# Druthyn/rtiow

Hardware: AMD Instinct MI355X
Metric: Msamples/sec (pixels×spp) on book-1 final scene; per-pixel RMSE vs CPU (higher is better)
Workload: dtype f64

## Files before the change

__graft_entry__.py:

```python
import os
import subprocess
import sys

ROOT = os.path.dirname(os.path.abspath(__file__))
if ROOT not in sys.path:
    sys.path.insert(0, ROOT)

HIPCC_FLAGS = [
    "-O3", "-std=c++17", "--offload-arch=gfx950",
    "-ffp-contract=off",
    "-fhip-fp32-correctly-rounded-divide-sqrt",
    "-mllvm", "-amdgpu-mfma-vgpr-form",
    "-fPIC", "-shared",
]


def build_hip_library(crosscheck=False):
    out = os.path.join(ROOT, "tools", "librtiow_hip_xcheck.so") if crosscheck else os.path.join(ROOT, "rtiow_amd", "librtiow_hip.so")
    srcs = [os.path.join(ROOT, "rtiow_amd", "csrc", name) for name in ("rt_api.hip", "rt_frames.hip")]
    import bench
    cmd = ["hipcc", *HIPCC_FLAGS, *(["-DRTIOW_CROSSCHECK_MODES"] if crosscheck else []),
           f'-DRT_SOURCE_SHA="{bench.kernel_source_sha()}"',
           "-I", os.path.join(ROOT, "include"), "-I", os.path.join(ROOT, "rtiow_amd", "csrc"), "-o", out, *srcs]
    subprocess.run(cmd, check=True, cwd=ROOT)
    return out


def build_host_cli(sanitize=False):
    out = os.path.join(ROOT, "host", "rtiow_render_san" if sanitize else "rtiow_render")
    rocm = os.environ.get("ROCM_PATH", "/opt/rocm")
    opt = ["-O1", "-g", "-fno-omit-frame-pointer", "-fsanitize=address,undefined", "-fno-sanitize-recover=all"] if sanitize else ["-O2"]
    cmd = ["g++", *opt, "-std=c++17", "-ffp-contract=off", "-Wall", "-Wextra", "-Wno-unused-parameter",
           "-I", os.path.join(ROOT, "include"), "-I", os.path.join(ROOT, "host"), "-isystem", os.path.join(rocm, "include"),
           "-o", out, os.path.join(ROOT, "host", "rtiow_render.cpp"),
           "-L", os.path.join(ROOT, "rtiow_amd"), "-lrtiow_hip", "-L", os.path.join(rocm, "lib"), "-lamdhip64", "-lrccl",
           "-pthread", "-Wl,-rpath,$ORIGIN/../rtiow_amd", "-Wl,-rpath," + os.path.join(rocm, "lib")]
    subprocess.run(cmd, check=True, cwd=ROOT)
    return out


def build() -> None:
    build_hip_library()
    build_hip_library(crosscheck=True)
    build_host_cli()
    subprocess.run(["make", "-s", "-C", os.path.join(ROOT, "oracle"), "liboracle.so"], check=True)
    import rtiow_amd
    from rtiow_amd import _ffi
    lib = _ffi.load()
    assert lib.rt_backend_name() == b"hip-gfx950"
    assert not _ffi.has_crosscheck_modes()
    assert rtiow_amd.SPHERE_DTYPE.itemsize == 72


def smoke() -> None:
    import numpy as np
    import oracle
    import rtiow_amd as rt

    w, h, spp = 96, 54, 4
    flat = rt.random_scene(1).flatten()
    cam = rt.book1_camera(w, h)
    with rt.Renderer(0) as r:
        r.upload_scene(flat)
        sums, fix, st = r.render(cam, rt.make_params(w, h, spp, seed=1))
        rgba = r.resolve_rgba8(fix, spp, flip=True)
    want_fix, want_sum, ost = oracle.render_b(oracle.camera_from_host(cam), flat, oracle.make_params(w, h, spp, seed=1))
    assert np.array_equal(fix, want_fix), "GPU exact sums differ from the CPU oracle"
    assert np.array_equal(sums, want_sum)
    assert st["rays_traced"] == ost["rays_traced"] and st["samples"] == w * h * spp
    assert np.array_equal(rgba, oracle.resolve_b(want_fix, spp, flip=True))
    with rt.Renderer(0) as r:
        r.upload_scene(flat)
        one_call, _ = r.render_rgba8(cam, rt.make_params(w, h, spp, seed=1), flip=True)
    assert np.array_equal(one_call, rgba), "rt_render_rgba8 differs from rt_render + rt_resolve_rgba8"
    print(f"smoke ok: {w}x{h}x{spp} bit-exact vs oracle; {st['rays_traced']} rays, "
          f"kernel {st['kernel_ms']:.3f} ms on {st['grid_blocks']} blocks")


if __name__ == "__main__":
    build()
    if len(sys.argv) > 1 and sys.argv[1] == "smoke":
        smoke()
```

rtiow_amd/csrc/rt_api.hip:

```cpp
#include <hip/hip_runtime.h>

#include <algorithm>
#include <cmath>
#include <cstdarg>
#include <cstdio>
#include <cstdlib>
#include <cstring>
#include <vector>

#include "rt_host.hpp"

namespace {

thread_local char g_err[512] = "";

int env_int(const char *name, int dflt)
{
    const char *v = getenv(name);
    if (!v || !*v) return dflt;
    return atoi(v);
}

}

int rt_host::fail(int code, const char *fmt, ...)
{
    va_list ap;
    va_start(ap, fmt);
    vsnprintf(g_err, sizeof(g_err), fmt, ap);
    va_end(ap);
    return code;
}

using namespace rt_host;

int rt_host::validate_params(const rt_params *p)
{
    if (!p) return fail(RT_ERR_INVALID_ARGUMENT, "params is NULL");
    if (p->width < 2 || p->height < 2)
        return fail(RT_ERR_INVALID_ARGUMENT, "width and height must be >= 2 (u,v divide by W-1,H-1; main.rs:131-132)");
    if (p->width > 65535 || p->height > 65535)
        return fail(RT_ERR_INVALID_ARGUMENT, "width and height must be <= 65535");
    if ((long long)p->width * p->height > 0x7fffffffLL)
        return fail(RT_ERR_INVALID_ARGUMENT, "width*height does not fit the 32-bit Philox pixel counter");
    if (p->spp < 0 || p->sample_begin < 0 || (long long)p->spp + p->sample_begin > 0x7fffffffLL)
        return fail(RT_ERR_INVALID_ARGUMENT, "spp/sample_begin out of range");
    if (p->max_depth < 0) return fail(RT_ERR_INVALID_ARGUMENT, "max_depth must be >= 0");
    if (!(p->t_min > 0.0)) return fail(RT_ERR_INVALID_ARGUMENT, "t_min must be > 0 (reference: 1e-4, main.rs:44)");
    if (p->tile_rows < 1) return fail(RT_ERR_INVALID_ARGUMENT, "tile_rows must be >= 1");
    if (p->shard_count < 1 || p->shard_index < 0 || p->shard_index >= p->shard_count)
        return fail(RT_ERR_INVALID_ARGUMENT, "need 0 <= shard_index < shard_count");
    if (p->flags & ~RT_FLAG_KNOWN)
        return fail(RT_ERR_INVALID_ARGUMENT, "unknown flags 0x%x (this library knows 0x%x)", p->flags & ~RT_FLAG_KNOWN, RT_FLAG_KNOWN);
    return RT_OK;
}

namespace {

int shard_rows(const rt_params *p)
{
    const long long T = p->tile_rows, H = p->height;
    const long long ntiles = (H + T - 1) / T;
    long long rows = 0;
    for (long long t = p->shard_index; t < ntiles; t += p->shard_count) {
        const long long lo = t * T;
        rows += (lo + T <= H) ? T : (H - lo);
    }
    return (int)rows;
}

}

int rt_host::ensure(void **ptr, size_t *have, size_t need)
{
    if (*have >= need && *ptr) return RT_OK;
    if (*ptr) { (void)hipFree(*ptr); *ptr = nullptr; *have = 0; }
    RT_HIP(hipMalloc(ptr, need ? need : 16));
    *have = need;
    return RT_OK;
}

namespace {

float filter_kprime(const rt_sphere &s, double KU)
{
    const double kappa = KU / (1.0 - KU);
    const double r2 = s.radius * s.radius;
    const double c2 = s.center[0] * s.center[0] + s.center[1] * s.center[1] + s.center[2] * s.center[2];
    if (!(r2 > 1e-30) || !(c2 + r2 < 1e30)) return -INFINITY;
    const double exact = c2 * (1.0 - kappa) - r2 * (1.0 + 2.0 * kappa);
    float kp = (float)(exact - std::fabs(exact) * 1e-12);
    if ((double)kp > exact) kp = std::nextafterf(kp, -INFINITY);
    return kp;
}

uint32_t host_bf16_rne(float x)
{
    uint32_t u; memcpy(&u, &x, 4);
    return (u + 0x7FFFu + ((u >> 16) & 1u)) >> 16;
}
void host_split_bf16x3(float x, uint32_t p[3])
{
    auto back = [](uint32_t b) { uint32_t u = b << 16; float f; memcpy(&f, &u, 4); return f; };
    p[0] = host_bf16_rne(x);
    const float r1 = x - back(p[0]);
    p[1] = host_bf16_rne(r1);
    const float r2 = r1 - back(p[1]);
    p[2] = host_bf16_rne(r2);
}

float tube_radius_floor(const rt_sphere *spheres, int n, const char *skip)
{
    std::vector<double> r;
    for (int i = 0; i < n; ++i)
        if (!(skip && skip[i]) && std::fabs(spheres[i].radius) > 1e-15 && std::fabs(spheres[i].radius) < 1e15)
            r.push_back(std::fabs(spheres[i].radius));
    if (r.empty()) return 1.0f;
    std::nth_element(r.begin(), r.begin() + r.size() / 4, r.end());
    return (float)r[r.size() / 4];
}
float tube_bound(const rt_sphere &s, float rho)
{
    const double r = std::fabs(s.radius);
    const double c2 = s.center[0] * s.center[0] + s.center[1] * s.center[1] + s.center[2] * s.center[2];
    if (!(r * r > 1e-30) || !(c2 + r * r < 1e30)) return INFINITY;
    const double R = r * (1.0 + (double)rt::kTubeBasisErr) + (double)rt::kTubeCenterErr * std::sqrt(c2);
    float f = (float)(R * (1.0 + 1e-12));
    if ((double)f < R) f = std::nextafterf(f, INFINITY);
    return f > rho ? f : rho;
}
uint32_t tube_sigma_bits(float bound)
{
    if (!(bound < INFINITY)) return 0u;
    const float f = (float)(2.0 * (1.0 - 1.0 / 64.0) / (double)bound);
    uint32_t u; memcpy(&u, &f, 4);
    return u >> 16;
}
void tube_tile(const rt_sphere *const s[32], float rho, uint4 out_b[64], float out_r[32])
{
    for (int c = 0; c < 32; ++c) {
        uint32_t w[8] = {0, 0, 0, 0, 0, 0, 0, 0};
        out_r[c] = -1.0f;
        if (s[c]) {
            out_r[c] = tube_bound(*s[c], rho);
            const uint32_t sg = tube_sigma_bits(out_r[c]);
            uint32_t sgu = sg << 16; float sigma; memcpy(&sigma, &sgu, 4);
            if (sg != 0u) {
                for (int i = 0; i < 3; ++i) {
                    const double ci = s[c]->center[i] * (double)sigma;
                    const uint32_t y1 = host_bf16_rne((float)ci);
                    uint32_t u1 = y1 << 16; float f1; memcpy(&f1, &u1, 4);
                    const uint32_t y2 = host_bf16_rne((float)(ci - (double)f1));
                    w[2 * i + 0] = y1 | (y2 << 16);
                    w[2 * i + 1] = y1 | (y2 << 16);
                }
            }
            w[6] = sg | (sg << 16);
            w[7] = sg;
        } else {
            w[7] = 0x4080u << 16;
        }
        out_b[c] = make_uint4(w[0], w[1], w[2], w[3]);
        out_b[32 + c] = make_uint4(w[4], w[5], w[6], w[7]);
    }
}

void free_scene(rt_context *ctx)
{
    (void)hipFree(ctx->d_filt); (void)hipFree(ctx->d_geo); (void)hipFree(ctx->d_mat);
    (void)hipFree(ctx->d_btube); (void)hipFree(ctx->d_geo_slot); (void)hipFree(ctx->d_slot_orig);
    ctx->d_filt = nullptr; ctx->d_geo = ctx->d_mat = nullptr; ctx->d_btube = nullptr; ctx->d_geo_slot = nullptr; ctx->d_slot_orig = nullptr;
#ifdef RTIOW_CROSSCHECK_MODES
    ctx->x.release();
#endif
    ctx->n_spheres = -1;
}

template <typename T>
int upload_table(T **dst, const T *src, size_t count)
{
    RT_HIP(hipMalloc((void **)dst, (count ? count : 1) * sizeof(T)));
    if (count) RT_HIP(hipMemcpy(*dst, src, count * sizeof(T), hipMemcpyHostToDevice));
    return RT_OK;
}

}

void rt_host::set_scene_params(const rt_context *ctx, rt::KParams &kp)
{
    kp.filt = ctx->d_filt; kp.geo = ctx->d_geo; kp.mat = ctx->d_mat;
    kp.n_tiles = ctx->n_tiles;
#ifdef RTIOW_CROSSCHECK_MODES
    kp.x.bmat = ctx->x.d_bmat; kp.x.kpt = ctx->x.d_kpt;
    kp.x.bmat16 = ctx->x.d_bmat16; kp.x.kpt16 = ctx->x.d_kpt16; kp.x.bmatL = ctx->x.d_bmatL;
#endif
    kp.btube = ctx->d_btube; kp.tube_rho = ctx->tube_rho;
    kp.geo_slot = ctx->d_geo_slot; kp.slot_orig = ctx->d_slot_orig;
    kp.n_global = ctx->n_global; kp.grid_dim = ctx->grid_dim;
    kp.grid_rows = 0ull;
    for (int k = 0; ctx->grid_dim > 0 && (k + 1) * ctx->grid_dim <= 64; ++k) kp.grid_rows |= 1ull << (k * ctx->grid_dim);
    for (int k = 0; k < 8; ++k) kp.grid[k] = ctx->grid[k];
    kp.scene_scale = ctx->scene_scale;
    kp.n_always = ctx->n_always;
    for (int e = 0; e < 8; ++e) kp.always_idx[e] = ctx->always_idx[e];
}

int rt_host::next_launch_slot(rt_context *ctx, hipStream_t stream, rt::KParams &kp)
{
    ctx->cur = (ctx->cur + 1) % rt_context::kSlots;
    ctx->d_queue = ctx->q_slots[ctx->cur]; ctx->d_stats = ctx->s_slots[ctx->cur];
    ctx->ev0 = ctx->e0_slots[ctx->cur]; ctx->ev1 = ctx->e1_slots[ctx->cur];
    if (ctx->slot_used[ctx->cur]) RT_HIP(hipStreamWaitEvent(stream, ctx->ev1, 0));
    ctx->slot_used[ctx->cur] = true;
    kp.queue = ctx->d_queue; kp.stats = ctx->d_stats;
    return RT_OK;
}

namespace {

int validate_pixel_list(const rt_context *ctx, const rt_camera *cam, const rt_params *p, int64_t n_pixels)
{
    int rc = validate_params(p);
    if (rc) return rc;
    if (p->flags & (RT_FLAG_UNIFORM53 | RT_FLAG_DIAG_STATS | RT_FLAG_NO_FILTER))
        return fail(RT_ERR_INVALID_ARGUMENT, "pixel-list renders run the shipped kernel only: RT_FLAG_UNIFORM53, RT_FLAG_DIAG_STATS and "
                    "RT_FLAG_NO_FILTER are not available on them (flags 0x%x)", p->flags);
    if (p->shard_count != 1)
        return fail(RT_ERR_INVALID_ARGUMENT, "pixel-list renders are not sharded: shard_count must be 1 (is %d)", p->shard_count);
    if (n_pixels < 0 || n_pixels > 0x7fffffffLL)
        return fail(RT_ERR_INVALID_ARGUMENT, "n_pixels %lld out of range [0, 2^31)", (long long)n_pixels);
    if (!ctx || !cam) return fail(RT_ERR_INVALID_ARGUMENT, "ctx/cam is NULL");
    if (ctx->scan_mode != 5)
        return fail(RT_ERR_INVALID_ARGUMENT, "pixel-list renders need the shipped scan mode 5; this context was created under RTIOW_SCAN_MODE=%d", ctx->scan_mode);
    return RT_OK;
}

int validate_adaptive(const rt_adaptive *a)
{
    if (!a) return fail(RT_ERR_INVALID_ARGUMENT, "rt_adaptive is NULL");
    if (a->step < 1) return fail(RT_ERR_INVALID_ARGUMENT, "rt_adaptive.step must be >= 1 (is %d)", a->step);
    if (a->reserved != 0) return fail(RT_ERR_INVALID_ARGUMENT, "rt_adaptive.reserved must be 0");
    if (!(a->threshold >= 0.0)) return fail(RT_ERR_INVALID_ARGUMENT, "rt_adaptive.threshold must be >= 0 (and not a NaN)");
    if (!(a->dark_floor > 0.0) || !(a->dark_floor < INFINITY))
        return fail(RT_ERR_INVALID_ARGUMENT, "rt_adaptive.dark_floor must be > 0 and finite (with a zero floor a black pixel's error is 0/0)");
    return RT_OK;
}

constexpr int kAdaptiveMaxSpp = 32766;

int validate_select(const void *fix, const void *half, const void *count, int32_t width, int32_t height, int32_t n, const rt_adaptive *a,
                    const void *list_out, const void *n_out)
{
    if (!fix || !half || !count || !list_out || !n_out) return fail(RT_ERR_INVALID_ARGUMENT, "rt_select_pixels: a buffer is NULL");
    if (width < 1 || height < 1 || (long long)width * height > 0x7fffffffLL)
        return fail(RT_ERR_INVALID_ARGUMENT, "rt_select_pixels: bad width/height");
    if (n < 2 || n > kAdaptiveMaxSpp || (n & 1))
        return fail(RT_ERR_INVALID_ARGUMENT, "rt_select_pixels: n = %d samples must be even (two halves) and in [2, %d]", n, kAdaptiveMaxSpp);
    return validate_adaptive(a);
}

constexpr size_t kMaxColumns = (size_t)1 << 26;
constexpr int kMaxGridDim = 63;

struct TileLayout {
    int grid_dim = 0, n_global = 0;
    float grid[8] = {};
    float scale = 0.0f;
    std::vector<int> slot_of;
};

std::vector<int> always_exact_list(const rt_sphere *spheres, int n)
{
    std::vector<int> out;
    if (n <= 0) return out;
    std::vector<double> radii(n);
    for (int i = 0; i < n; ++i) radii[i] = std::fabs(spheres[i].radius);
    std::vector<double> sorted = radii;
    std::nth_element(sorted.begin(), sorted.begin() + n / 2, sorted.end());
    const double big = 8.0 * sorted[n / 2];
    std::vector<int> order;
    for (int i = 0; i < n; ++i) if (radii[i] > big) order.push_back(i);
    std::sort(order.begin(), order.end(), [&](int x, int y) { return radii[x] > radii[y]; });
    for (size_t k = 0; k < order.size() && k < 8; ++k) out.push_back(order[k]);
    return out;
}

TileLayout tile_layout(const rt_sphere *spheres, int n, const char *never)
{
    TileLayout L;
    std::vector<int> filtered;
    for (int i = 0; i < n; ++i) if (!never[i]) filtered.push_back(i);
    std::vector<int> &slot_of = L.slot_of;
    L.grid_dim = 0; L.n_global = 0;
    if (filtered.size() > 64 && !env_int("RTIOW_NO_GRID", 0)) {
        std::vector<double> rr;
        for (int i : filtered) rr.push_back(std::fabs(spheres[i].radius));
        std::nth_element(rr.begin(), rr.begin() + rr.size() / 2, rr.end());
        const double med = rr[rr.size() / 2];
        double x0 = INFINITY, x1 = -INFINITY, z0 = INFINITY, z1 = -INFINITY;
        for (int i : filtered) {
            if (std::fabs(spheres[i].radius) > 3.0 * med) continue;
            x0 = std::min(x0, spheres[i].center[0]); x1 = std::max(x1, spheres[i].center[0]);
            z0 = std::min(z0, spheres[i].center[2]); z1 = std::max(z1, spheres[i].center[2]);
        }
        const double extent = std::max(x1 - x0, z1 - z0);
        const bool one_cell = extent == 0.0;
        const bool grid_ok = one_cell || (extent > 0.0 && extent < 1e15);
        if (grid_ok) {
        std::vector<std::vector<int>> cells;
        std::vector<int> global;
        double cell = 1.0;
        auto assign = [&](int G, bool keep) -> int {
            cell = one_cell ? 1.0 : extent / G;
            std::vector<int> count((size_t)G * G, 0);
            if (keep) { cells.assign((size_t)G * G, {}); global.clear(); }
            size_t n_glob = 0;
            for (int i : filtered) {
                const double r = std::fabs(spheres[i].radius);
                bool to_cell = !(r > 3.0 * med || r > 0.25 * cell);
                size_t c = 0;
                if (to_cell) {
                    int ix = (int)std::floor((spheres[i].center[0] - x0) / cell), iz = (int)std::floor((spheres[i].center[2] - z0) / cell);
                    ix = std::max(0, std::min(ix, G - 1)); iz = std::max(0, std::min(iz, G - 1));
                    c = (size_t)iz * G + ix;
                    to_cell = count[c] < 32;
                }
                if (to_cell) { ++count[c]; if (keep) cells[c].push_back(i); }
                else { ++n_glob; if (keep) global.push_back(i); }
            }
            return (int)((n_glob + 31) / 32);
        };
        int G = one_cell ? 1 : env_int("RTIOW_GRID_DIM", 0);
        if (G <= 0) {
            double best = INFINITY;
            for (int g = 1; g <= kMaxGridDim; ++g) {
                if ((double)g * g > (double)filtered.size()) break;
                const int ng = assign(g, false);
                if (ng > 48) continue;
                const double cost = ng + 1.4 * g;
                if (cost < best) { best = cost; G = g; }
            }
        }
        G = std::max(1, std::min(G, kMaxGridDim));
        (void)assign(G, true);
        double ylo = INFINITY, yhi = -INFINITY, pad = 0.0;
        for (const std::vector<int> &c : cells)
            for (int i : c) {
                const double r = std::fabs(spheres[i].radius);
                ylo = std::min(ylo, spheres[i].center[1] - r); yhi = std::max(yhi, spheres[i].center[1] + r);
                pad = std::max(pad, r);
            }
        const int n_global = (int)((global.size() + 31) / 32);
        const float inv_cell = (float)(1.0 / cell);
        if (std::isnormal(inv_cell) && (size_t)(n_global + G * G) * 32 <= (size_t)kMaxColumns && n_global <= 48 && ylo <= yhi) {
            L.grid_dim = G; L.n_global = n_global;
            slot_of.assign((size_t)(n_global + G * G) * 32, -1);
            for (size_t k = 0; k < global.size(); ++k) slot_of[k] = global[k];
            for (size_t c = 0; c < cells.size(); ++c)
                for (size_t k = 0; k < cells[c].size(); ++k) slot_of[((size_t)n_global + c) * 32 + k] = cells[c][k];
            auto down = [](double v) { float f = (float)v; if ((double)f > v) f = std::nextafterf(f, -INFINITY); return f; };
            auto up = [](double v) { float f = (float)v; if ((double)f < v) f = std::nextafterf(f, INFINITY); return f; };
            L.grid[0] = down(x0); L.grid[1] = down(z0);
            L.grid[2] = inv_cell;
            L.grid[3] = up(x0 + G * cell); L.grid[4] = up(z0 + G * cell);
            L.grid[5] = down(ylo); L.grid[6] = up(yhi); L.grid[7] = up(pad);
            const double gs = std::max(std::fabs(x0), std::fabs(x0 + G * cell)) + pad + std::max(std::fabs(ylo), std::fabs(yhi)) +
                              std::max(std::fabs(z0), std::fabs(z0 + G * cell)) + pad;
            L.scale = (float)gs * 1.0001f;
        }
        }
    }
    if (L.grid_dim == 0) {
        slot_of.assign((size_t)((filtered.empty() ? 0 : filtered.back() + 1) + 31) / 32 * 32, -1);
        for (int i : filtered) slot_of[i] = i;
    }
    return L;
}

#ifdef RTIOW_CROSSCHECK_MODES
#include "xcheck/rt_xcheck_host.inc"
#endif

}

extern "C" {

const char *rt_last_error(void) { return g_err; }
const char *rt_backend_name(void) { return "hip-gfx950"; }
int32_t rt_abi_version(void) { return RTIOW_HIP_ABI_VERSION; }
#ifndef RT_SOURCE_SHA
#define RT_SOURCE_SHA "unknown"
#endif
const char *rt_build_source_sha(void) { return RT_SOURCE_SHA; }

int rt_create(int32_t device_id, rt_context **out)
{
    if (!out) return fail(RT_ERR_INVALID_ARGUMENT, "out is NULL");
    *out = nullptr;
    int count = 0;
    hipError_t e = hipGetDeviceCount(&count);
    if (e != hipSuccess || count <= 0)
        return fail(RT_ERR_NO_DEVICE, "no HIP device visible (%s); librtiow_hip has no CPU fallback",
                    e == hipSuccess ? "count = 0" : hipGetErrorString(e));
    if (device_id < 0 || device_id >= count)
        return fail(RT_ERR_INVALID_ARGUMENT, "device_id %d out of range [0,%d)", device_id, count);
    RT_HIP(hipSetDevice(device_id));
    hipDeviceProp_t prop;
    RT_HIP(hipGetDeviceProperties(&prop, device_id));
    if (strncmp(prop.gcnArchName, "gfx950", 6) != 0)
        return fail(RT_ERR_NO_DEVICE, "device %d is %s; this library carries gfx950 (MI355X) code only",
                    device_id, prop.gcnArchName);
    rt_context *ctx = new (std::nothrow) rt_context();
    if (!ctx) return fail(RT_ERR_OUT_OF_MEMORY, "host allocation failed");
    ctx->device = device_id;
    ctx->cu_count = prop.multiProcessorCount;
    ctx->blocks_per_cu = env_int("RTIOW_BLOCKS_PER_CU", 0);
    ctx->ring_min_spp = env_int("RTIOW_RING_MIN_SPP", 0);
    ctx->scan_mode = env_int("RTIOW_SCAN_MODE", 5);
#ifdef RTIOW_CROSSCHECK_MODES
    if (ctx->scan_mode < 1 || ctx->scan_mode > 5) ctx->scan_mode = 5;
#else
    if (ctx->scan_mode != 1 && ctx->scan_mode != 5) {
        const int asked = ctx->scan_mode;
        rt_destroy(ctx);
        return fail(RT_ERR_INVALID_ARGUMENT, "RTIOW_SCAN_MODE=%d: this build carries scan modes 1 and 5 (modes 2-4 need "
                    "a -DRTIOW_CROSSCHECK_MODES build)", asked);
    }
#endif
    hipError_t e1 = hipSuccess, e2 = hipSuccess, e3 = hipSuccess, e4 = hipSuccess;
    for (int k = 0; k < rt_context::kSlots; ++k) {
        hipError_t a = hipMalloc((void **)&ctx->q_slots[k], 64), b = hipMalloc((void **)&ctx->s_slots[k], 1024);
        hipError_t c = hipEventCreate(&ctx->e0_slots[k]), d = hipEventCreate(&ctx->e1_slots[k]);
        if (a != hipSuccess) e1 = a;
        if (b != hipSuccess) e2 = b;
        if (c != hipSuccess) e3 = c;
        if (d != hipSuccess) e4 = d;
    }
    ctx->d_queue = ctx->q_slots[0]; ctx->d_stats = ctx->s_slots[0]; ctx->ev0 = ctx->e0_slots[0]; ctx->ev1 = ctx->e1_slots[0];
    hipError_t e5 = hipStreamCreateWithFlags(&ctx->own_stream, hipStreamNonBlocking);
    if (e1 != hipSuccess || e2 != hipSuccess || e3 != hipSuccess || e4 != hipSuccess || e5 != hipSuccess) {
        rt_destroy(ctx);
        return fail(RT_ERR_HIP, "context setup failed on device %d", device_id);
    }
    *out = ctx;
    return RT_OK;
}

int rt_destroy(rt_context *ctx)
{
    if (!ctx) return RT_OK;
    (void)hipSetDevice(ctx->device);
    if (ctx->own_stream) (void)hipStreamSynchronize(ctx->own_stream);
    free_scene(ctx);
    for (int k = 0; k < rt_context::kSlots; ++k) {
        (void)hipFree(ctx->q_slots[k]); (void)hipFree(ctx->s_slots[k]);
        if (ctx->e0_slots[k]) (void)hipEventDestroy(ctx->e0_slots[k]);
        if (ctx->e1_slots[k]) (void)hipEventDestroy(ctx->e1_slots[k]);
    }
    (void)hipFree(ctx->d_stage_fix); (void)hipFree(ctx->d_stage_sum); (void)hipFree(ctx->d_stage_rgba);
    (void)hipFree(ctx->d_sel); (void)hipFree(ctx->d_adapt); (void)hipFree(ctx->d_stage_list); (void)hipFree(ctx->d_stage_cams);
    if (ctx->own_stream) (void)hipStreamDestroy(ctx->own_stream);
    delete ctx;
    return RT_OK;
}

int rt_upload_scene(rt_context *ctx, const rt_sphere *spheres, int32_t n)
{
    if (!ctx) return fail(RT_ERR_INVALID_ARGUMENT, "ctx is NULL");
    if (n < 0 || (n > 0 && !spheres)) return fail(RT_ERR_INVALID_ARGUMENT, "bad sphere list");
    if (n > RT_MAX_SPHERES) return fail(RT_ERR_INVALID_ARGUMENT, "at most %d spheres (RT_MAX_SPHERES)", RT_MAX_SPHERES);
    if (ctx->scan_mode == 1 && n > 65535) return fail(RT_ERR_INVALID_ARGUMENT, "RTIOW_SCAN_MODE=1 (the cross-check filter) takes at most 65535 spheres");
    for (int i = 0; i < n; ++i) {
        const rt_sphere &s = spheres[i];
        if (s.kind < RT_LAMBERTIAN || s.kind > RT_DIALECTRIC)
            return fail(RT_ERR_INVALID_ARGUMENT, "sphere %d: unknown material kind %d", i, s.kind);
        const double mags[4] = { s.center[0], s.center[1], s.center[2], s.radius };
        for (double v : mags)
            if (!(std::fabs(v) < 1e15))
                return fail(RT_ERR_INVALID_ARGUMENT, "sphere %d: coordinates/radius must be finite and below 1e15", i);
        if (s.radius == 0.0) return fail(RT_ERR_INVALID_ARGUMENT, "sphere %d: radius must not be zero", i);
    }
    RT_HIP(hipSetDevice(ctx->device));
    RT_HIP(hipDeviceSynchronize());
    free_scene(ctx);
    const size_t cnt = (size_t)(n > 0 ? n : 1);
    std::vector<double> geo(cnt * 4, 0.0), mat(cnt * rt::kMatStride, 0.0);
    for (int i = 0; i < n; ++i) {
        const rt_sphere &s = spheres[i];
        const double r2 = s.radius * s.radius;
        geo[4 * i + 0] = s.center[0]; geo[4 * i + 1] = s.center[1]; geo[4 * i + 2] = s.center[2];
        geo[4 * i + 3] = r2;
        double *m = &mat[(size_t)rt::kMatStride * i];
        m[0] = 1.0 / s.radius;
        m[1] = s.param;
        m[2] = s.albedo[0]; m[3] = s.albedo[1]; m[4] = s.albedo[2];
        m[5] = (double)s.kind;
        if (s.kind == RT_DIALECTRIC) {
            m[6] = 1.0 / s.param;
            double r0 = (1.0 - m[6]) / (1.0 + m[6]); m[7] = r0 * r0;
            r0 = (1.0 - s.param) / (1.0 + s.param); m[8] = r0 * r0;
            m[2] = 1.0; m[3] = 1.0; m[4] = 1.0;
        }
    }
    ctx->n_always = 0;
    for (int i : always_exact_list(spheres, n)) ctx->always_idx[ctx->n_always++] = i;
    const int n_tiles = 2 * ((n + 31) / 32);
    ctx->n_tiles = n_tiles;
    int rc = RT_OK;
    if (ctx->scan_mode == 5) {
        std::vector<char> never(n > 0 ? n : 1, 0);
        for (int e = 0; e < ctx->n_always; ++e) never[ctx->always_idx[e]] = 1;
        ctx->tube_rho = tube_radius_floor(spheres, n, never.data());
        const TileLayout L = tile_layout(spheres, n, never.data());
        const std::vector<int> &slot_of = L.slot_of;
        ctx->grid_dim = L.grid_dim; ctx->n_global = L.n_global;
        for (int k = 0; k < 8; ++k) ctx->grid[k] = L.grid[k];
        ctx->scene_scale = L.scale;
        const int n_tiles32 = (int)(slot_of.size() / 32);
        ctx->n_tiles = 2 * n_tiles32;
        const size_t ttc = (size_t)n_tiles32 + 1;
        std::vector<uint4> btube(ttc * 64);
        std::vector<float> rtube(ttc * 32);
        std::vector<double> geo_slot(ttc * 32 * 4, 0.0);
        std::vector<uint32_t> slot_orig(ttc * 32, 0xFFFFFFFFu);
        for (size_t t = 0; t < ttc; ++t) {
            const rt_sphere *col[32];
            for (int c = 0; c < 32; ++c) {
                const size_t slot = 32 * t + c;
                const int i = slot < slot_of.size() ? slot_of[slot] : -1;
                col[c] = i >= 0 ? &spheres[i] : nullptr;
                if (i >= 0) {
                    slot_orig[slot] = (uint32_t)i;
                    for (int k = 0; k < 4; ++k) geo_slot[4 * slot + k] = geo[4 * (size_t)i + k];
                }
            }
            tube_tile(col, ctx->tube_rho, &btube[t * 64], &rtube[t * 32]);
        }
        if (!rc) rc = upload_table(&ctx->d_btube, btube.data(), btube.size());
        if (!rc) rc = upload_table(&ctx->d_geo_slot, geo_slot.data(), geo_slot.size());
        if (!rc) rc = upload_table(&ctx->d_slot_orig, slot_orig.data(), slot_orig.size());
    }
    std::vector<float> filt(cnt * 4, 0.0f);
    if (ctx->scan_mode >= 1 && ctx->scan_mode <= 3) {
        for (int i = 0; i < n; ++i) {
            const rt_sphere &s = spheres[i];
            filt[4 * i + 0] = (float)s.center[0]; filt[4 * i + 1] = (float)s.center[1];
            filt[4 * i + 2] = (float)s.center[2]; filt[4 * i + 3] = filter_kprime(s, (double)rt::kFilterKU);
        }
        if (ctx->scan_mode == 1 && !rc) rc = upload_table(&ctx->d_filt, filt.data(), filt.size());
    }
#ifdef RTIOW_CROSSCHECK_MODES
    if (!rc) rc = xcheck_upload_tables(ctx, spheres, n, n_tiles, filt);
#endif
    if (!rc) rc = upload_table(&ctx->d_geo, geo.data(), geo.size());
    if (!rc) rc = upload_table(&ctx->d_mat, mat.data(), mat.size());
    if (rc) {
        free_scene(ctx);
        return rc;
    }
    ctx->n_spheres = n;
    return RT_OK;
}

int rt_shard_rows(const rt_params *p, int32_t *out_rows)
{
    if (!out_rows) return fail(RT_ERR_INVALID_ARGUMENT, "out_rows is NULL");
    int rc = validate_params(p);
    if (rc) return rc;
    *out_rows = shard_rows(p);
    return RT_OK;
}

int rt_shard_row_index(const rt_params *p, int32_t compact_row, int32_t *out_j)
{
    if (!out_j) return fail(RT_ERR_INVALID_ARGUMENT, "out_j is NULL");
    int rc = validate_params(p);
    if (rc) return rc;
    if (compact_row < 0 || compact_row >= shard_rows(p))
        return fail(RT_ERR_INVALID_ARGUMENT, "compact_row out of range");
    const int lt = compact_row / p->tile_rows;
    *out_j = (lt * p->shard_count + p->shard_index) * p->tile_rows + (compact_row - lt * p->tile_rows);
    return RT_OK;
}

int rt_render_device(rt_context *ctx, const rt_camera *cam, const rt_params *p, void *d_fix, void *stream_v)
{
    if (!ctx || !cam) return fail(RT_ERR_INVALID_ARGUMENT, "ctx/cam is NULL");
    int rc = validate_params(p);
    if (rc) return rc;
    if (ctx->n_spheres < 0) return fail(RT_ERR_NO_SCENE, "rt_upload_scene has not been called");
    const int rows = shard_rows(p);
    if (rows > 0 && !d_fix) return fail(RT_ERR_INVALID_ARGUMENT, "d_fix is NULL");
    RT_HIP(hipSetDevice(ctx->device));
    hipStream_t stream = (hipStream_t)stream_v;

    const long long npix = (long long)rows * p->width;
    const unsigned long long total_items = (unsigned long long)npix * (unsigned long long)p->spp;
    const int mode_now = (p->flags & RT_FLAG_NO_FILTER) ? 0 : ctx->scan_mode;
    const char *lb_env = getenv("RTIOW_LARGE_BLOCK_MIN_ITEMS");
    const unsigned long long lb_min = (lb_env && *lb_env) ? strtoull(lb_env, nullptr, 0)
                                    : (p->flags & RT_FLAG_OVERLAPPED) ? 0ull : rt::kLargeMinItems;
    const bool small_grid_scene = ctx->grid_dim > 0 && ctx->n_global + ctx->grid_dim * ctx->grid_dim <= 64;
    const bool shipped_kernel = mode_now == 5 && !(p->flags & RT_FLAG_DIAG_STATS);
    const bool large_candidate = shipped_kernel && !small_grid_scene && p->spp >= rt::kLargeMinSpp && total_items >= lb_min && p->spp >= ctx->ring_min_spp;
    const bool wide_ring = shipped_kernel && !large_candidate;
    const unsigned ring_slots = wide_ring ? 2u * (unsigned)rt::kRingSlots : (unsigned)rt::kRingSlots;
    unsigned small_block = 0;
    for (unsigned items = rt::kItemBlock; items >= 64u && p->spp >= 1; items -= 64u)
        if ((items - 1u + (unsigned)p->spp - 1u) / (unsigned)p->spp + 1u <= ring_slots) { small_block = items; break; }
    const bool use_ring = small_block != 0u && p->spp >= ctx->ring_min_spp;
    const bool large_blocks = mode_now == 5 && !(p->flags & RT_FLAG_DIAG_STATS) && use_ring && small_block == (unsigned)rt::kItemBlock &&
                              p->spp >= (small_grid_scene ? rt::kLargeMinSppSmallGrid : rt::kLargeMinSpp) && total_items >= lb_min;
    const unsigned item_block = large_blocks ? rt::kItemBlockLarge : use_ring ? small_block : rt::kItemBlock;
    const unsigned long long n_blocks = (total_items + item_block - 1) / item_block;
    if (n_blocks > 0x7fffffffULL)
        return fail(RT_ERR_INVALID_ARGUMENT, "rows*width*spp = %llu pixel-samples in one launch: at most 2^31 blocks of %d "
                    "(split the samples over several launches with sample_begin and RT_FLAG_ACCUMULATE)", total_items, (int)item_block);
    rt::KParams kp;
    memset(&kp, 0, sizeof(kp));
    static_assert(sizeof(rt::KCamera) == sizeof(rt_camera), "camera layouts must match");
    memcpy(&kp.cam, cam, sizeof(rt_camera));
    kp.width = p->width; kp.height = p->height;
    kp.spp = p->spp; kp.sample_begin = p->sample_begin; kp.max_depth = p->max_depth;
    kp.t_min = p->t_min;
    kp.k0 = (uint32_t)p->seed; kp.k1 = (uint32_t)(p->seed >> 32);
    kp.tile_rows = p->tile_rows; kp.shard_index = p->shard_index; kp.shard_count = p->shard_count;
    kp.rows = rows; kp.n_spheres = ctx->n_spheres;
    kp.npix = (uint32_t)npix; kp.total_items = total_items; kp.n_blocks = (uint32_t)n_blocks;
    kp.inv_spp = p->spp > 0 ? 1.0 / (double)p->spp : 0.0;
    kp.inv_width = 1.0 / (double)p->width;
    auto magic_for = [](long long d) -> uint32_t {
        return (d <= 1 || d >= 32768) ? 0u : (uint32_t)(0x100000000ULL / (unsigned long long)d + 1ULL);
    };
    kp.magic_spp = magic_for(p->spp); kp.magic_width = magic_for(p->width); kp.magic_tile = magic_for(p->tile_rows);
    kp.use_ring = use_ring ? 1 : 0;
    kp.block_items = item_block;
    set_scene_params(ctx, kp);
    kp.fix = (unsigned long long *)d_fix;
    rc = next_launch_slot(ctx, stream, kp);
    if (rc) return rc;

    if (!(p->flags & RT_FLAG_ACCUMULATE) && npix > 0)
        RT_HIP(hipMemsetAsync(d_fix, 0, (size_t)npix * 3 * sizeof(unsigned long long), stream));
    RT_HIP(hipMemsetAsync(ctx->d_queue, 0, 64, stream));
    RT_HIP(hipMemsetAsync(ctx->d_stats, 0, 1024, stream));

    memset(&ctx->last, 0, sizeof(ctx->last));
    ctx->last.n_spheres = ctx->n_spheres;
    ctx->last.block_threads = rt::kBlock;
    ctx->zero_depth_samples = 0;
    if (p->max_depth == 0 || kp.total_items == 0) {
        RT_HIP(hipEventRecord(ctx->ev0, stream));
        RT_HIP(hipEventRecord(ctx->ev1, stream));
        ctx->zero_depth_samples = (unsigned long long)npix * (unsigned long long)p->spp;
        ctx->launched = true;
        return RT_OK;
    }

    int grid = 0;
    const bool diag = (p->flags & RT_FLAG_DIAG_STATS) != 0;
    const int mode = (p->flags & RT_FLAG_NO_FILTER) ? 0 : ctx->scan_mode;
    ctx->last.scan_mode = mode;
    ctx->last.kernel_variant = 0;
    const bool small_grid = small_grid_scene;
    if (p->flags & RT_FLAG_UNIFORM53) {
        if (diag || (mode != 0 && mode != 5))
            return fail(RT_ERR_INVALID_ARGUMENT, "RT_FLAG_UNIFORM53 runs with scan mode 5 (the default) or RT_FLAG_NO_FILTER, without RT_FLAG_DIAG_STATS");
        if (mode == 0) rc = launch_render<0, false, false, true>(ctx, kp, stream, &grid);
        else if (small_grid) rc = large_blocks ? launch_render<5, false, true, true, rt::kItemBlockLarge>(ctx, kp, stream, &grid)
                                              : launch_render<5, false, true, true>(ctx, kp, stream, &grid);
        else rc = large_blocks ? launch_render<5, false, false, true, rt::kItemBlockLarge>(ctx, kp, stream, &grid)
                               : launch_render<5, false, false, true>(ctx, kp, stream, &grid);
        if (rc) return rc;
        ctx->last.kernel_variant = 2 | ((mode == 5 && small_grid) ? 1 : 0) | (mode == 5 && large_blocks ? 4 : 0);
        ctx->launched = true;
        ctx->last.grid_blocks = grid;
        return RT_OK;
    }
    switch (mode * 2 + (diag ? 1 : 0)) {
    case 0: rc = launch_render<0, false>(ctx, kp, stream, &grid); break;
    case 1: rc = launch_render<0, true>(ctx, kp, stream, &grid); break;
    case 2: rc = launch_render<1, false>(ctx, kp, stream, &grid); break;
    case 3: rc = launch_render<1, true>(ctx, kp, stream, &grid); break;
#ifdef RTIOW_CROSSCHECK_MODES
    case 4: rc = launch_render<2, false>(ctx, kp, stream, &grid); break;
    case 5: rc = launch_render<2, true>(ctx, kp, stream, &grid); break;
    case 6: rc = launch_render<3, false>(ctx, kp, stream, &grid); break;
    case 7: rc = launch_render<3, true>(ctx, kp, stream, &grid); break;
    case 8: rc = launch_render<4, false>(ctx, kp, stream, &grid); break;
    case 9: rc = launch_render<4, true>(ctx, kp, stream, &grid); break;
#endif
    case 10:
        if (small_grid) {
            rc = large_blocks ? launch_render<5, false, true, false, rt::kItemBlockLarge>(ctx, kp, stream, &grid)
                              : launch_render<5, false, true>(ctx, kp, stream, &grid);
            ctx->last.kernel_variant = 1;
        } else rc = large_blocks ? launch_render<5, false, false, false, rt::kItemBlockLarge>(ctx, kp, stream, &grid)
                                 : launch_render<5, false>(ctx, kp, stream, &grid);
        if (large_blocks) ctx->last.kernel_variant |= 4;
        break;
    default: rc = launch_render<5, true>(ctx, kp, stream, &grid); break;
    }
    if (rc) return rc;
    ctx->launched = true;
    ctx->last.grid_blocks = grid;
    return RT_OK;
}

int rt_last_stats(rt_context *ctx, rt_stats *stats)
{
    if (!ctx || !stats) return fail(RT_ERR_INVALID_ARGUMENT, "ctx/stats is NULL");
    if (!ctx->launched) return fail(RT_ERR_INVALID_ARGUMENT, "no launch to report on");
    RT_HIP(hipSetDevice(ctx->device));
    RT_HIP(hipEventSynchronize(ctx->ev1));
    float ms = 0.0f;
    RT_HIP(hipEventElapsedTime(&ms, ctx->ev0, ctx->ev1));
    unsigned long long h[80];
    RT_HIP(hipMemcpy(h, ctx->d_stats, sizeof(h), hipMemcpyDeviceToHost));
    for (int k = 0; k < 64; ++k) ctx->last.live_per_bounce[k] = h[16 + k];
    ctx->last.rays_traced = h[0];
    ctx->last.samples = h[1] + ctx->zero_depth_samples;
    ctx->last.candidates = h[2];
    ctx->last.exact_roots = h[3];
    ctx->last.direct_samples = h[4];
    ctx->last.sphere_tests = h[0] * (unsigned long long)(ctx->last.n_spheres > 0 ? ctx->last.n_spheres : 0);
    ctx->last.kernel_ms = ms;
    *stats = ctx->last;
    return RT_OK;
}

#if defined(RT_PHASE_STAMPS) || defined(RT_BLOCK_COUNTS) || defined(RT_EXIT_TIMES) || defined(RT_LDS_CONFLICTS)
extern "C" int rt_debug_phase_cycles(rt_context *ctx, unsigned long long out[8])
{
    RT_HIP(hipSetDevice(ctx->device));
    RT_HIP(hipEventSynchronize(ctx->ev1));
    RT_HIP(hipMemcpy(out, ctx->d_stats + 8, 64, hipMemcpyDeviceToHost));
    return RT_OK;
}
extern "C" int rt_debug_phase_cycles16(rt_context *ctx, unsigned long long out[16])
{
    RT_HIP(hipSetDevice(ctx->device));
    RT_HIP(hipEventSynchronize(ctx->ev1));
    RT_HIP(hipMemcpy(out, ctx->d_stats + 8, 64, hipMemcpyDeviceToHost));
    RT_HIP(hipMemcpy(out + 8, ctx->d_stats + 80, 64, hipMemcpyDeviceToHost));
    return RT_OK;
}
#endif

int rt_fix_to_f32_device(rt_context *ctx, const void *d_fix, int64_t count, void *d_out_f32, void *stream_v)
{
    if (!ctx) return fail(RT_ERR_INVALID_ARGUMENT, "ctx is NULL");
    if (count < 0 || (count > 0 && (!d_fix || !d_out_f32))) return fail(RT_ERR_INVALID_ARGUMENT, "bad buffers");
    if (count == 0) return RT_OK;
    RT_HIP(hipSetDevice(ctx->device));
    long long blocks = (count + 255) / 256;
    if (blocks > 8192) blocks = 8192;
    hipLaunchKernelGGL(rt::fix_to_f32_kernel, dim3((unsigned)blocks), dim3(256), 0, (hipStream_t)stream_v,
                       (const unsigned long long *)d_fix, (float *)d_out_f32, (long long)count);
    RT_HIP(hipGetLastError());
    return RT_OK;
}

int rt_resolve_rgba8_device(rt_context *ctx, const void *d_fix, int32_t width, int32_t rows,
                            int64_t spp, int32_t flip, void *d_rgba, void *stream_v)
{
    if (!ctx) return fail(RT_ERR_INVALID_ARGUMENT, "ctx is NULL");
    if (width < 1 || rows < 0 || spp < 1) return fail(RT_ERR_INVALID_ARGUMENT, "bad width/rows/spp");
    if (rows == 0) return RT_OK;
    if (!d_fix || !d_rgba) return fail(RT_ERR_INVALID_ARGUMENT, "bad buffers");
    RT_HIP(hipSetDevice(ctx->device));
    const long long npix = (long long)width * rows;
    long long blocks = (npix + 255) / 256;
    if (blocks > 8192) blocks = 8192;
    const double scale = 1.0 / (double)spp;
    hipLaunchKernelGGL(rt::resolve_rgba8_kernel, dim3((unsigned)blocks), dim3(256), 0, (hipStream_t)stream_v,
                       (const unsigned long long *)d_fix, (uint8_t *)d_rgba, (int)width, (int)rows, scale, (int)flip);
    RT_HIP(hipGetLastError());
    return RT_OK;
}

int rt_render(rt_context *ctx, const rt_camera *cam, const rt_params *p,
              float *out_sum, uint64_t *out_fix, rt_stats *stats)
{
    if (!ctx) return fail(RT_ERR_INVALID_ARGUMENT, "ctx is NULL");
    int rc = validate_params(p);
    if (rc) return rc;
    const int rows = shard_rows(p);
    const size_t count = (size_t)rows * p->width * 3;
    if (count > 0 && !out_sum && !out_fix) return fail(RT_ERR_INVALID_ARGUMENT, "no output buffer");
    RT_HIP(hipSetDevice(ctx->device));
    rc = ensure(&ctx->d_stage_fix, &ctx->stage_fix_bytes, count * sizeof(uint64_t));
    if (rc) return rc;
    rc = ensure(&ctx->d_stage_sum, &ctx->stage_sum_bytes, count * sizeof(float));
    if (rc) return rc;
    rt_params q = *p;
    q.flags &= ~RT_FLAG_ACCUMULATE;
    rc = rt_render_device(ctx, cam, &q, ctx->d_stage_fix, ctx->own_stream);
    if (rc) return rc;
    if (out_sum) {
        rc = rt_fix_to_f32_device(ctx, ctx->d_stage_fix, (int64_t)count, ctx->d_stage_sum, ctx->own_stream);
        if (rc) return rc;
        RT_HIP(hipMemcpyAsync(out_sum, ctx->d_stage_sum, count * sizeof(float), hipMemcpyDeviceToHost, ctx->own_stream));
    }
    if (out_fix)
        RT_HIP(hipMemcpyAsync(out_fix, ctx->d_stage_fix, count * sizeof(uint64_t), hipMemcpyDeviceToHost, ctx->own_stream));
    RT_HIP(hipStreamSynchronize(ctx->own_stream));
    if (stats) return rt_last_stats(ctx, stats);
    return RT_OK;
}

int rt_resolve_rgba8(rt_context *ctx, const uint64_t *fix, int32_t width, int32_t rows,
                     int64_t spp, int32_t flip, uint8_t *out_rgba)
{
    if (!ctx) return fail(RT_ERR_INVALID_ARGUMENT, "ctx is NULL");
    if (width < 1 || rows < 0 || spp < 1) return fail(RT_ERR_INVALID_ARGUMENT, "bad width/rows/spp");
    if (rows == 0) return RT_OK;
    if (!fix || !out_rgba) return fail(RT_ERR_INVALID_ARGUMENT, "bad buffers");
    RT_HIP(hipSetDevice(ctx->device));
    const size_t npix = (size_t)width * rows;
    int rc = ensure(&ctx->d_stage_fix, &ctx->stage_fix_bytes, npix * 3 * sizeof(uint64_t));
    if (rc) return rc;
    rc = ensure(&ctx->d_stage_rgba, &ctx->stage_rgba_bytes, npix * 4);
    if (rc) return rc;
    RT_HIP(hipMemcpyAsync(ctx->d_stage_fix, fix, npix * 3 * sizeof(uint64_t), hipMemcpyHostToDevice, ctx->own_stream));
    rc = rt_resolve_rgba8_device(ctx, ctx->d_stage_fix, width, rows, spp, flip, ctx->d_stage_rgba, ctx->own_stream);
    if (rc) return rc;
    RT_HIP(hipMemcpyAsync(out_rgba, ctx->d_stage_rgba, npix * 4, hipMemcpyDeviceToHost, ctx->own_stream));
    RT_HIP(hipStreamSynchronize(ctx->own_stream));
    return RT_OK;
}

int rt_render_rgba8(rt_context *ctx, const rt_camera *cam, const rt_params *p, int32_t flip,
                    uint8_t *out_rgba, rt_stats *stats)
{
    if (!ctx) return fail(RT_ERR_INVALID_ARGUMENT, "ctx is NULL");
    int rc = validate_params(p);
    if (rc) return rc;
    if (p->spp < 1) return fail(RT_ERR_INVALID_ARGUMENT, "rt_render_rgba8 needs spp >= 1 (to_rgba divides by the sample count, vec3.rs:409)");
    const int rows = shard_rows(p);
    const size_t npix = (size_t)rows * p->width;
    if (npix > 0 && !out_rgba) return fail(RT_ERR_INVALID_ARGUMENT, "out_rgba is NULL");
    RT_HIP(hipSetDevice(ctx->device));
    rc = ensure(&ctx->d_stage_fix, &ctx->stage_fix_bytes, npix * 3 * sizeof(uint64_t));
    if (rc) return rc;
    rc = ensure(&ctx->d_stage_rgba, &ctx->stage_rgba_bytes, npix * 4);
    if (rc) return rc;
    rt_params q = *p;
    q.flags &= ~RT_FLAG_ACCUMULATE;
    rc = rt_render_device(ctx, cam, &q, ctx->d_stage_fix, ctx->own_stream);
    if (rc) return rc;
    if (npix > 0) {
        rc = rt_resolve_rgba8_device(ctx, ctx->d_stage_fix, p->width, rows, (int64_t)p->spp, flip, ctx->d_stage_rgba, ctx->own_stream);
        if (rc) return rc;
        RT_HIP(hipMemcpyAsync(out_rgba, ctx->d_stage_rgba, npix * 4, hipMemcpyDeviceToHost, ctx->own_stream));
        RT_HIP(hipStreamSynchronize(ctx->own_stream));
    } else {
        RT_HIP(hipStreamSynchronize(ctx->own_stream));
    }
    if (stats) return rt_last_stats(ctx, stats);
    return RT_OK;
}

int rt_render_pixels_device(rt_context *ctx, const rt_camera *cam, const rt_params *p, const uint32_t *d_pixels,
                            int64_t n_pixels, void *d_fix, void *stream_v)
{
    int rc = validate_pixel_list(ctx, cam, p, n_pixels);
    if (rc) return rc;
    if (ctx->n_spheres < 0) return fail(RT_ERR_NO_SCENE, "rt_upload_scene has not been called");
    if (n_pixels == 0) return RT_OK;
    if (!d_pixels || !d_fix) return fail(RT_ERR_INVALID_ARGUMENT, "d_pixels/d_fix is NULL");
    const unsigned long long total_items = (unsigned long long)n_pixels * (unsigned long long)p->spp;
    unsigned small_block = 0;
    for (unsigned items = rt::kItemBlock; items >= 64u && p->spp >= 1; items -= 64u)
        if ((items - 1u + (unsigned)p->spp - 1u) / (unsigned)p->spp + 1u <= 2u * (unsigned)rt::kRingSlots) { small_block = items; break; }
    const bool use_ring = small_block != 0u && p->spp >= ctx->ring_min_spp;
    const unsigned item_block = use_ring ? small_block : rt::kItemBlock;
    const unsigned long long n_blocks = (total_items + item_block - 1) / item_block;
    if (n_blocks > 0x7fffffffULL)
        return fail(RT_ERR_INVALID_ARGUMENT, "n_pixels*spp = %llu pixel-samples in one launch: at most 2^31 blocks of %d", total_items, (int)item_block);
    RT_HIP(hipSetDevice(ctx->device));
    hipStream_t stream = (hipStream_t)stream_v;

    rt::KParams kp;
    memset(&kp, 0, sizeof(kp));
    memcpy(&kp.cam, cam, sizeof(rt_camera));
    kp.width = p->width; kp.height = p->height;
    kp.spp = p->spp; kp.sample_begin = p->sample_begin; kp.max_depth = p->max_depth;
    kp.t_min = p->t_min;
    kp.k0 = (uint32_t)p->seed; kp.k1 = (uint32_t)(p->seed >> 32);
    kp.tile_rows = 1; kp.shard_index = 0; kp.shard_count = 1;
    kp.rows = 1; kp.n_spheres = ctx->n_spheres;
    kp.npix = (uint32_t)n_pixels; kp.total_items = total_items; kp.n_blocks = (uint32_t)n_blocks;
    kp.inv_spp = p->spp > 0 ? 1.0 / (double)p->spp : 0.0;
    kp.inv_width = 1.0 / (double)p->width;
    kp.magic_spp = (p->spp <= 1 || p->spp >= 32768) ? 0u : (uint32_t)(0x100000000ULL / (unsigned long long)p->spp + 1ULL);
    kp.use_ring = use_ring ? 1 : 0;
    kp.block_items = item_block;
    set_scene_params(ctx, kp);
    kp.fix = (unsigned long long *)d_fix;
    kp.pix_list = d_pixels;
    rc = next_launch_slot(ctx, stream, kp);
    if (rc) return rc;

    if (!(p->flags & RT_FLAG_ACCUMULATE))
        RT_HIP(hipMemsetAsync(d_fix, 0, (size_t)n_pixels * 3 * sizeof(unsigned long long), stream));
    RT_HIP(hipMemsetAsync(ctx->d_queue, 0, 64, stream));
    RT_HIP(hipMemsetAsync(ctx->d_stats, 0, 1024, stream));
    memset(&ctx->last, 0, sizeof(ctx->last));
    ctx->last.n_spheres = ctx->n_spheres;
    ctx->last.block_threads = rt::kBlock;
    ctx->zero_depth_samples = 0;
    if (p->max_depth == 0 || total_items == 0) {
        RT_HIP(hipEventRecord(ctx->ev0, stream));
        RT_HIP(hipEventRecord(ctx->ev1, stream));
        ctx->zero_depth_samples = total_items;
        ctx->launched = true;
        return RT_OK;
    }
    int grid = 0;
    const bool small_grid = ctx->grid_dim > 0 && ctx->n_global + ctx->grid_dim * ctx->grid_dim <= 64;
    ctx->last.scan_mode = 5;
    ctx->last.kernel_variant = 8 | (small_grid ? 1 : 0);
    rc = small_grid ? launch_render<5, false, true, false, rt::kItemBlockList>(ctx, kp, stream, &grid)
                    : launch_render<5, false, false, false, rt::kItemBlockList>(ctx, kp, stream, &grid);
    if (rc) return rc;
    ctx->launched = true;
    ctx->last.grid_blocks = grid;
    return RT_OK;
}

int rt_render_pixels(rt_context *ctx, const rt_camera *cam, const rt_params *p, const uint32_t *pixels, int64_t n_pixels,
                     uint64_t *out_fix, rt_stats *stats)
{
    int rc = validate_pixel_list(ctx, cam, p, n_pixels);
    if (rc) return rc;
    if (ctx->n_spheres < 0) return fail(RT_ERR_NO_SCENE, "rt_upload_scene has not been called");
    if (n_pixels == 0) return RT_OK;
    if (!pixels || !out_fix) return fail(RT_ERR_INVALID_ARGUMENT, "pixels/out_fix is NULL");
    const long long npix_frame = (long long)p->width * p->height;
    for (int64_t k = 0; k < n_pixels; ++k)
        if ((long long)pixels[k] >= npix_frame)
            return fail(RT_ERR_INVALID_ARGUMENT, "pixels[%lld] = %u is not a pixel of a %d x %d frame", (long long)k, pixels[k], p->width, p->height);
    RT_HIP(hipSetDevice(ctx->device));
    const size_t count = (size_t)n_pixels * 3;
    rc = ensure(&ctx->d_stage_fix, &ctx->stage_fix_bytes, count * sizeof(uint64_t));
    if (rc) return rc;
    rc = ensure(&ctx->d_stage_list, &ctx->stage_list_bytes, (size_t)n_pixels * sizeof(uint32_t));
    if (rc) return rc;
    RT_HIP(hipMemcpyAsync(ctx->d_stage_list, pixels, (size_t)n_pixels * sizeof(uint32_t), hipMemcpyHostToDevice, ctx->own_stream));
    rt_params q = *p;
    q.flags &= ~RT_FLAG_ACCUMULATE;
    rc = rt_render_pixels_device(ctx, cam, &q, (const uint32_t *)ctx->d_stage_list, n_pixels, ctx->d_stage_fix, ctx->own_stream);
    if (rc) return rc;
    RT_HIP(hipMemcpyAsync(out_fix, ctx->d_stage_fix, count * sizeof(uint64_t), hipMemcpyDeviceToHost, ctx->own_stream));
    RT_HIP(hipStreamSynchronize(ctx->own_stream));
    if (stats) return rt_last_stats(ctx, stats);
    return RT_OK;
}

int rt_select_pixels_host(const uint64_t *fix, const uint64_t *half, const uint32_t *count, int32_t width, int32_t height,
                          int32_t n, const rt_adaptive *a, uint32_t *list_out, int64_t *n_out)
{
    int rc = validate_select(fix, half, count, width, height, n, a, list_out, n_out);
    if (rc) return rc;
    const size_t npix = (size_t)width * height;
    std::vector<char> noisy(npix);
    const double sc = 1.0 / ((double)n * 4294967296.0);
    for (size_t p = 0; p < npix; ++p)
        noisy[p] = count[p] == (uint32_t)n &&
                   rt::select_noisy((const unsigned long long *)fix + p * 3, (const unsigned long long *)half + p * 3, sc, a->threshold, a->dark_floor);
    int64_t m = 0;
    for (int j = 0; j < height; ++j)
        for (int i = 0; i < width; ++i) {
            const size_t p = (size_t)j * width + i;
            if (count[p] != (uint32_t)n) continue;
            bool act = false;
            for (int jj = std::max(j - 1, 0); jj <= std::min(j + 1, height - 1); ++jj)
                for (int ii = std::max(i - 1, 0); ii <= std::min(i + 1, width - 1); ++ii) act = act || noisy[(size_t)jj * width + ii];
            if (act) list_out[m++] = (uint32_t)p;
        }
    *n_out = m;
    return RT_OK;
}

int rt_select_pixels_device(rt_context *ctx, const void *d_fix, const void *d_half, const void *d_count, int32_t width,
                            int32_t height, int32_t n, const rt_adaptive *a, void *d_list_out, void *d_n_out, void *stream_v)
{
    if (!ctx) return fail(RT_ERR_INVALID_ARGUMENT, "ctx is NULL");
    int rc = validate_select(d_fix, d_half, d_count, width, height, n, a, d_list_out, d_n_out);
    if (rc) return rc;
    RT_HIP(hipSetDevice(ctx->device));
    hipStream_t stream = (hipStream_t)stream_v;
    const uint32_t npix = (uint32_t)((long long)width * height);
    const uint32_t blocks = (npix + rt::kSelBlock - 1) / rt::kSelBlock;
    const size_t flags_bytes = ((size_t)npix + 255) / 256 * 256;
    rc = ensure(&ctx->d_sel, &ctx->sel_bytes, 2 * flags_bytes + (size_t)blocks * sizeof(uint32_t));
    if (rc) return rc;
    uint8_t *noisy = (uint8_t *)ctx->d_sel, *active = noisy + flags_bytes;
    uint32_t *block_count = (uint32_t *)(active + flags_bytes);
    const double sc = 1.0 / ((double)n * 4294967296.0);
    hipLaunchKernelGGL(rt::select_noisy_kernel, dim3(blocks), dim3(rt::kSelBlock), 0, stream, (const unsigned long long *)d_fix,
                       (const unsigned long long *)d_half, (const uint32_t *)d_count, npix, (uint32_t)n, sc, a->threshold, a->dark_floor, noisy);
    hipLaunchKernelGGL(rt::select_active_kernel, dim3(blocks), dim3(rt::kSelBlock), 0, stream, (const uint8_t *)noisy,
                       (const uint32_t *)d_count, (int)width, (int)height, (uint32_t)n, active, block_count);
    hipLaunchKernelGGL(rt::select_scan_kernel, dim3(1), dim3(1024), 0, stream, block_count, blocks, (uint32_t *)d_n_out);
    hipLaunchKernelGGL(rt::select_write_kernel, dim3(blocks), dim3(rt::kSelBlock), 0, stream, (const uint8_t *)active,
                       (const uint32_t *)block_count, npix, (uint32_t *)d_list_out);
    RT_HIP(hipGetLastError());
    return RT_OK;
}

int rt_render_adaptive(rt_context *ctx, const rt_camera *cam, const rt_params *p, const rt_adaptive *a,
                       uint64_t *out_fix, uint64_t *out_half, uint32_t *out_count, rt_stats *stats)
{
    int rc = validate_params(p);
    if (rc) return rc;
    rc = validate_adaptive(a);
    if (rc) return rc;
    if (p->sample_begin != 0) return fail(RT_ERR_INVALID_ARGUMENT, "rt_render_adaptive numbers its own passes: sample_begin must be 0 (is %d)", p->sample_begin);
    if (p->spp < 2 * (long long)a->step || p->spp % (2 * (long long)a->step) != 0 || p->spp > kAdaptiveMaxSpp)
        return fail(RT_ERR_INVALID_ARGUMENT, "rt_render_adaptive: spp = %d (the most samples a pixel may get) must be a multiple of 2 * step = %lld "
                    "and <= %d", p->spp, 2 * (long long)a->step, kAdaptiveMaxSpp);
    rc = validate_pixel_list(ctx, cam, p, 0);
    if (rc) return rc;
    if (!out_fix || !out_count) return fail(RT_ERR_INVALID_ARGUMENT, "out_fix/out_count is NULL");
    if (ctx->n_spheres < 0) return fail(RT_ERR_NO_SCENE, "rt_upload_scene has not been called");
    RT_HIP(hipSetDevice(ctx->device));
    hipStream_t st = ctx->own_stream;
    const size_t npix = (size_t)p->width * p->height;
    const size_t sums = npix * 3 * sizeof(uint64_t);
    rc = ensure(&ctx->d_adapt, &ctx->adapt_bytes, 3 * sums + 2 * npix * sizeof(uint32_t) + 64);
    if (rc) return rc;
    char *base = (char *)ctx->d_adapt;
    void *d_fix = base, *d_half = base + sums, *d_pass = base + 2 * sums;
    uint32_t *d_count = (uint32_t *)(base + 3 * sums), *d_list = d_count + npix;
    unsigned long long *d_total = (unsigned long long *)(d_list + npix);
    uint32_t *d_n = (uint32_t *)(d_total + 5);
    RT_HIP(hipMemsetAsync(d_total, 0, 64, st));

    const uint32_t step = (uint32_t)a->step;
    float kernel_ms = 0.0f;
    unsigned long long zero_depth = 0;
    rt_stats shape{};
    int round_slots[2] = {0, 0};
    auto after_pass = [&](int k) -> int {
        hipLaunchKernelGGL(rt::stats_accumulate_kernel, dim3(1), dim3(64), 0, st, (const unsigned long long *)ctx->d_stats, d_total);
        RT_HIP(hipGetLastError());
        zero_depth += ctx->zero_depth_samples;
        round_slots[k] = ctx->cur;
        shape = ctx->last;
        return RT_OK;
    };
    auto round_time = [&]() -> int {
        for (int k = 0; k < 2; ++k) {
            float ms = 0.0f;
            RT_HIP(hipEventElapsedTime(&ms, ctx->e0_slots[round_slots[k]], ctx->e1_slots[round_slots[k]]));
            kernel_ms += ms;
        }
        return RT_OK;
    };
    rt_params q = *p;
    q.spp = (int32_t)step;
    q.sample_begin = 0; q.flags = p->flags & ~RT_FLAG_ACCUMULATE;
    rc = rt_render_device(ctx, cam, &q, d_fix, st);
    if (rc) return rc;
    if ((rc = after_pass(0))) return rc;
    RT_HIP(hipMemcpyAsync(d_half, d_fix, sums, hipMemcpyDeviceToDevice, st));
    q.sample_begin = (int32_t)step; q.flags = p->flags | RT_FLAG_ACCUMULATE;
    rc = rt_render_device(ctx, cam, &q, d_fix, st);
    if (rc) return rc;
    if ((rc = after_pass(1))) return rc;
    hipLaunchKernelGGL(rt::fill_u32_kernel, dim3((unsigned)((npix + 255) / 256)), dim3(256), 0, st, d_count, 2u * step, (uint32_t)npix);
    RT_HIP(hipGetLastError());
    q.flags = p->flags & ~RT_FLAG_ACCUMULATE;
    for (uint32_t n = 2u * step; ; n += 2u * step) {
        uint32_t n_list = 0;
        if (n < (uint32_t)p->spp) {
            rc = rt_select_pixels_device(ctx, d_fix, d_half, d_count, p->width, p->height, (int32_t)n, a, d_list, d_n, st);
            if (rc) return rc;
            RT_HIP(hipMemcpyAsync(&n_list, d_n, sizeof(uint32_t), hipMemcpyDeviceToHost, st));
        }
        RT_HIP(hipStreamSynchronize(st));
        if ((rc = round_time())) return rc;
        if (n_list == 0u) break;
        for (int k = 0; k < 2; ++k) {
            q.sample_begin = (int32_t)(n + (uint32_t)k * step);
            rc = rt_render_pixels_device(ctx, cam, &q, d_list, (int64_t)n_list, d_pass, st);
            if (rc) return rc;
            if ((rc = after_pass(k))) return rc;
            hipLaunchKernelGGL(rt::add_back_kernel, dim3((n_list + 255u) / 256u), dim3(256), 0, st, (const uint32_t *)d_list, n_list,
                               (const unsigned long long *)d_pass, (unsigned long long *)d_fix,
                               k == 0 ? (unsigned long long *)d_half : (unsigned long long *)nullptr, d_count, step);
            RT_HIP(hipGetLastError());
        }
    }
    unsigned long long total[5];
    RT_HIP(hipMemcpyAsync(out_fix, d_fix, sums, hipMemcpyDeviceToHost, st));
    if (out_half) RT_HIP(hipMemcpyAsync(out_half, d_half, sums, hipMemcpyDeviceToHost, st));
    RT_HIP(hipMemcpyAsync(out_count, d_count, npix * sizeof(uint32_t), hipMemcpyDeviceToHost, st));
    RT_HIP(hipMemcpyAsync(total, d_total, sizeof(total), hipMemcpyDeviceToHost, st));
    RT_HIP(hipStreamSynchronize(st));
    if (stats) {
        memset(stats, 0, sizeof(*stats));
        stats->n_spheres = shape.n_spheres; stats->grid_blocks = shape.grid_blocks; stats->block_threads = shape.block_threads;
        stats->scan_mode = shape.scan_mode; stats->kernel_variant = shape.kernel_variant;
        stats->rays_traced = total[0];
        stats->samples = total[1] + zero_depth;
        stats->direct_samples = total[4];
        stats->sphere_tests = total[0] * (unsigned long long)(shape.n_spheres > 0 ? shape.n_spheres : 0);
        stats->kernel_ms = kernel_ms;
    }
    return RT_OK;
}

int rt_resolve_rgba8_counts_device(rt_context *ctx, const void *d_fix, const void *d_count, int32_t width, int32_t rows,
                                   int32_t flip, void *d_rgba, void *stream_v)
{
    if (!ctx) return fail(RT_ERR_INVALID_ARGUMENT, "ctx is NULL");
    if (width < 1 || rows < 0) return fail(RT_ERR_INVALID_ARGUMENT, "bad width/rows");
    if (rows == 0) return RT_OK;
    if (!d_fix || !d_count || !d_rgba) return fail(RT_ERR_INVALID_ARGUMENT, "bad buffers");
    RT_HIP(hipSetDevice(ctx->device));
    const long long npix = (long long)width * rows;
    long long blocks = (npix + 255) / 256;
    if (blocks > 8192) blocks = 8192;
    hipLaunchKernelGGL(rt::resolve_rgba8_counts_kernel, dim3((unsigned)blocks), dim3(256), 0, (hipStream_t)stream_v,
                       (const unsigned long long *)d_fix, (const uint32_t *)d_count, (uint8_t *)d_rgba, (int)width, (int)rows, (int)flip);
    RT_HIP(hipGetLastError());
    return RT_OK;
}

int rt_resolve_rgba8_counts(rt_context *ctx, const uint64_t *fix, const uint32_t *count, int32_t width, int32_t rows,
                            int32_t flip, uint8_t *out_rgba)
{
    if (!ctx) return fail(RT_ERR_INVALID_ARGUMENT, "ctx is NULL");
    if (width < 1 || rows < 0) return fail(RT_ERR_INVALID_ARGUMENT, "bad width/rows");
    if (rows == 0) return RT_OK;
    if (!fix || !count || !out_rgba) return fail(RT_ERR_INVALID_ARGUMENT, "bad buffers");
    RT_HIP(hipSetDevice(ctx->device));
    const size_t npix = (size_t)width * rows;
    int rc = ensure(&ctx->d_stage_fix, &ctx->stage_fix_bytes, npix * 3 * sizeof(uint64_t));
    if (rc) return rc;
    rc = ensure(&ctx->d_stage_rgba, &ctx->stage_rgba_bytes, npix * 4);
    if (rc) return rc;
    rc = ensure(&ctx->d_stage_list, &ctx->stage_list_bytes, npix * sizeof(uint32_t));
    if (rc) return rc;
    RT_HIP(hipMemcpyAsync(ctx->d_stage_fix, fix, npix * 3 * sizeof(uint64_t), hipMemcpyHostToDevice, ctx->own_stream));
    RT_HIP(hipMemcpyAsync(ctx->d_stage_list, count, npix * sizeof(uint32_t), hipMemcpyHostToDevice, ctx->own_stream));
    rc = rt_resolve_rgba8_counts_device(ctx, ctx->d_stage_fix, ctx->d_stage_list, width, rows, flip, ctx->d_stage_rgba, ctx->own_stream);
    if (rc) return rc;
    RT_HIP(hipMemcpyAsync(out_rgba, ctx->d_stage_rgba, npix * 4, hipMemcpyDeviceToHost, ctx->own_stream));
    RT_HIP(hipStreamSynchronize(ctx->own_stream));
    return RT_OK;
}

int rt_f64_div_sqrt_device(rt_context *ctx, const double *a, const double *b, int32_t n,
                           double *out_div, double *out_sqrt)
{
    if (!ctx || !a || !b || !out_div || !out_sqrt || n < 0) return fail(RT_ERR_INVALID_ARGUMENT, "bad argument");
    if (n == 0) return RT_OK;
    RT_HIP(hipSetDevice(ctx->device));
    const size_t bytes = (size_t)n * sizeof(double);
    int rc = ensure(&ctx->d_stage_fix, &ctx->stage_fix_bytes, 4 * bytes);
    if (rc) return rc;
    double *da = (double *)ctx->d_stage_fix, *db = da + n, *dq = db + n, *dr = dq + n;
    RT_HIP(hipMemcpyAsync(da, a, bytes, hipMemcpyHostToDevice, ctx->own_stream));
    RT_HIP(hipMemcpyAsync(db, b, bytes, hipMemcpyHostToDevice, ctx->own_stream));
    hipLaunchKernelGGL(rt::f64_div_sqrt_kernel, dim3((unsigned)((n + 255) / 256)), dim3(256), 0, ctx->own_stream,
                       (const double *)da, (const double *)db, (int)n, dq, dr);
    RT_HIP(hipGetLastError());
    RT_HIP(hipMemcpyAsync(out_div, dq, bytes, hipMemcpyDeviceToHost, ctx->own_stream));
    RT_HIP(hipMemcpyAsync(out_sqrt, dr, bytes, hipMemcpyDeviceToHost, ctx->own_stream));
    RT_HIP(hipStreamSynchronize(ctx->own_stream));
    return RT_OK;
}

int rt_quantize_device(rt_context *ctx, const double *x, int32_t n, uint64_t *out)
{
    if (!ctx || !x || !out || n < 0) return fail(RT_ERR_INVALID_ARGUMENT, "bad argument");
    if (n == 0) return RT_OK;
    RT_HIP(hipSetDevice(ctx->device));
    const size_t bytes = (size_t)n * sizeof(double);
    int rc = ensure(&ctx->d_stage_fix, &ctx->stage_fix_bytes, 2 * bytes);
    if (rc) return rc;
    double *dx = (double *)ctx->d_stage_fix;
    unsigned long long *dq = (unsigned long long *)(dx + n);
    RT_HIP(hipMemcpyAsync(dx, x, bytes, hipMemcpyHostToDevice, ctx->own_stream));
    hipLaunchKernelGGL(rt::quantize_kernel, dim3((unsigned)((n + 255) / 256)), dim3(256), 0, ctx->own_stream, (const double *)dx, (int)n, dq);
    RT_HIP(hipGetLastError());
    RT_HIP(hipMemcpyAsync(out, dq, bytes, hipMemcpyDeviceToHost, ctx->own_stream));
    RT_HIP(hipStreamSynchronize(ctx->own_stream));
    return RT_OK;
}

int rt_unit_accept_device(rt_context *ctx, const uint32_t *words, int32_t n, uint32_t *out_accept, double *out_uniforms)
{
    if (!ctx || !words || !out_accept || !out_uniforms || n < 0) return fail(RT_ERR_INVALID_ARGUMENT, "bad argument");
    if (n == 0) return RT_OK;
    RT_HIP(hipSetDevice(ctx->device));
    const size_t wb = (size_t)n * 3 * sizeof(uint32_t), ab = (size_t)n * sizeof(uint32_t), ub = (size_t)n * 4 * sizeof(double);
    int rc = ensure(&ctx->d_stage_fix, &ctx->stage_fix_bytes, ub + wb + ab);
    if (rc) return rc;
    double *du = (double *)ctx->d_stage_fix;
    uint32_t *dw = (uint32_t *)(du + 4 * (size_t)n), *da = dw + 3 * (size_t)n;
    RT_HIP(hipMemcpyAsync(dw, words, wb, hipMemcpyHostToDevice, ctx->own_stream));
    hipLaunchKernelGGL(rt::unit_accept_kernel, dim3((unsigned)((n + 255) / 256)), dim3(256), 0, ctx->own_stream, (const uint32_t *)dw, (int)n, da, du);
    RT_HIP(hipGetLastError());
    RT_HIP(hipMemcpyAsync(out_accept, da, ab, hipMemcpyDeviceToHost, ctx->own_stream));
    RT_HIP(hipMemcpyAsync(out_uniforms, du, ub, hipMemcpyDeviceToHost, ctx->own_stream));
    RT_HIP(hipStreamSynchronize(ctx->own_stream));
    return RT_OK;
}

#ifdef RTIOW_CROSSCHECK_MODES
#include "xcheck/rt_xcheck_hooks.inc"
#endif

int rt_tube_tile_host(const rt_sphere *spheres32, uint32_t *out_words, float *out_bound, float *out_rho)
{
    if (!spheres32 || !out_words || !out_bound || !out_rho) return fail(RT_ERR_INVALID_ARGUMENT, "NULL argument");
    const float rho = tube_radius_floor(spheres32, 32, nullptr);
    *out_rho = rho;
    const rt_sphere *col[32];
    for (int c = 0; c < 32; ++c) col[c] = &spheres32[c];
    uint4 tile[64];
    tube_tile(col, rho, tile, out_bound);
    memcpy(out_words, tile, sizeof(tile));
    return RT_OK;
}

int rt_filter_tube_device(rt_context *ctx, const double *o, const double *d, const rt_sphere *spheres32,
                          float *out_h, float *out_rows, float *out_bound, float *out_rho)
{
    if (!ctx || !o || !d || !spheres32 || !out_h || !out_rows || !out_bound || !out_rho)
        return fail(RT_ERR_INVALID_ARGUMENT, "NULL argument");
    RT_HIP(hipSetDevice(ctx->device));
    const float rho = tube_radius_floor(spheres32, 32, nullptr);
    *out_rho = rho;
    const rt_sphere *col[32];
    for (int c = 0; c < 32; ++c) col[c] = &spheres32[c];
    uint4 tile[64];
    tube_tile(col, rho, tile, out_bound);
    const size_t in_b = 3072 + sizeof(tile), out_b = (64 * 32 * 2 + 64 * 9) * 4;
    int rc = ensure(&ctx->d_stage_fix, &ctx->stage_fix_bytes, in_b + out_b);
    if (rc) return rc;
    char *base = (char *)ctx->d_stage_fix;
    double *d_o = (double *)base, *d_d = d_o + 192;
    uint4 *d_tile = (uint4 *)(base + 3072);
    float *d_h = (float *)(base + in_b), *d_rows = d_h + 64 * 32 * 2;
    RT_HIP(hipMemcpyAsync(d_o, o, 1536, hipMemcpyHostToDevice, ctx->own_stream));
    RT_HIP(hipMemcpyAsync(d_d, d, 1536, hipMemcpyHostToDevice, ctx->own_stream));
    RT_HIP(hipMemcpyAsync(d_tile, tile, sizeof(tile), hipMemcpyHostToDevice, ctx->own_stream));
    hipLaunchKernelGGL(rt::tube_products_kernel, dim3(1), dim3(64), 0, ctx->own_stream,
                       (const double *)d_o, (const double *)d_d, (const uint4 *)d_tile, rho, d_h, d_rows);
    RT_HIP(hipGetLastError());
    RT_HIP(hipMemcpyAsync(out_h, d_h, 64 * 32 * 2 * 4, hipMemcpyDeviceToHost, ctx->own_stream));
    RT_HIP(hipMemcpyAsync(out_rows, d_rows, 64 * 9 * 4, hipMemcpyDeviceToHost, ctx->own_stream));
    RT_HIP(hipStreamSynchronize(ctx->own_stream));
    return RT_OK;
}

int rt_tile_layout_host(const rt_sphere *spheres, int32_t n, int32_t out_dims[2], float out_grid[8], int32_t *out_slot_of, int32_t cap)
{
    if (!spheres || n < 0 || n > RT_MAX_SPHERES || !out_dims || !out_grid || (!out_slot_of && cap > 0)) return fail(RT_ERR_INVALID_ARGUMENT, "rt_tile_layout_host: bad argument");
    std::vector<char> never(n > 0 ? n : 1, 0);
    for (int i : always_exact_list(spheres, n)) never[i] = 1;
    const TileLayout L = tile_layout(spheres, n, never.data());
    out_dims[0] = L.grid_dim; out_dims[1] = L.n_global;
    for (int k = 0; k < 8; ++k) out_grid[k] = L.grid[k];
    if ((size_t)cap < L.slot_of.size()) return fail(RT_ERR_INVALID_ARGUMENT, "rt_tile_layout_host: out_slot_of too small");
    for (size_t k = 0; k < L.slot_of.size(); ++k) out_slot_of[k] = L.slot_of[k];
    return (int)L.slot_of.size();
}

int rt_philox_device(rt_context *ctx, const uint32_t ctr[4], const uint32_t key[2], uint32_t out[4])
{
    if (!ctx || !ctr || !key || !out) return fail(RT_ERR_INVALID_ARGUMENT, "NULL argument");
    RT_HIP(hipSetDevice(ctx->device));
    int rc = ensure(&ctx->d_stage_rgba, &ctx->stage_rgba_bytes, 64);
    if (rc) return rc;
    hipLaunchKernelGGL(rt::philox_kat_kernel, dim3(1), dim3(1), 0, ctx->own_stream,
                       ctr[0], ctr[1], ctr[2], ctr[3], key[0], key[1], (uint32_t *)ctx->d_stage_rgba);
    RT_HIP(hipGetLastError());
    RT_HIP(hipMemcpyAsync(out, ctx->d_stage_rgba, 16, hipMemcpyDeviceToHost, ctx->own_stream));
    RT_HIP(hipStreamSynchronize(ctx->own_stream));
    return RT_OK;
}

}
```

rtiow_amd/csrc/rt_diag.hpp:

```cpp
#pragma once
#include <hip/hip_runtime.h>
#include <stdint.h>

#if (defined(RT_PHASE_STAMPS) + defined(RT_BLOCK_COUNTS) + defined(RT_EXIT_TIMES) + defined(RT_LDS_CONFLICTS)) > 1
#error "one diagnostic build at a time: RT_PHASE_STAMPS, RT_BLOCK_COUNTS, RT_EXIT_TIMES or RT_LDS_CONFLICTS"
#endif

#define RT_DIAG_NOTHING do { } while (0)

#define RT_DIAG_DECLARE() RT_DIAG_NOTHING
#define RT_DIAG_FLUSH() RT_DIAG_NOTHING
#define RT_STAMP(k) RT_DIAG_NOTHING
#define RT_COUNT(k) RT_DIAG_NOTHING
#define RT_COUNT_N(k, n) RT_DIAG_NOTHING
#define RT_COUNT_MAIN(k) RT_DIAG_NOTHING
#define RT_COUNT_ROWS_TRIP(k) RT_DIAG_NOTHING
#define RT_COUNT_ENUM_TRIP(m) RT_DIAG_NOTHING
#define RT_COUNT_REDRAW_LANES(ok) RT_DIAG_NOTHING
#define RT_LDS(site, BYTES, ATOMIC, LOAD64, ptr, active) RT_DIAG_NOTHING
#define RT_LDS_N(site, n, BYTES, ATOMIC, LOAD64, byte_addr, active) RT_DIAG_NOTHING
#define RT_LDS_QUEUE_READS(take, entry) RT_DIAG_NOTHING
#define RT_LDS_POOL_TIE(has_root, r, key) RT_DIAG_NOTHING
#define RT_LDS_ENUM_READS(has, word, summary, seg0) RT_DIAG_NOTHING
#define RT_LDS_RING_ADDS(ringed, my_blk) RT_DIAG_NOTHING

#if defined(RT_PHASE_STAMPS)
#undef RT_DIAG_DECLARE
#undef RT_DIAG_FLUSH
#undef RT_STAMP
#define RT_DIAG_DECLARE() unsigned long long ph[16] = {0, 0, 0, 0, 0, 0, 0, 0, 0, 0, 0, 0, 0, 0, 0, 0}, tprev = __builtin_amdgcn_s_memtime()
#define RT_STAMP(k) do { __builtin_amdgcn_s_waitcnt(0); const unsigned long long tn_ = __builtin_amdgcn_s_memtime(); \
                         __builtin_amdgcn_s_waitcnt(0); ph[k] += tn_ - tprev; tprev = tn_; } while (0)
#define RT_DIAG_FLUSH() do { if (lane == 0) { \
        for (int k_ = 0; k_ < 8; ++k_) atomicAdd(P.stats + 8 + k_, ph[k_]); \
        for (int k_ = 8; k_ < 16; ++k_) atomicAdd(P.stats + 80 + (k_ - 8), ph[k_]); } } while (0)
#endif

#if defined(RT_EXIT_TIMES)
#undef RT_DIAG_DECLARE
#undef RT_DIAG_FLUSH
#define RT_DIAG_DECLARE() const unsigned long long t_wave_start = __builtin_amdgcn_s_memrealtime()
#define RT_DIAG_FLUSH() do { if (lane == 0) { \
        const unsigned long long te_ = __builtin_amdgcn_s_memrealtime(); \
        atomicMax(P.stats + 8, te_); atomicMax(P.stats + 9, ~te_); atomicAdd(P.stats + 10, te_); \
        atomicMax(P.stats + 11, ~t_wave_start); atomicAdd(P.stats + 12, 1ull); } } while (0)
#endif

#if defined(RT_BLOCK_COUNTS)
#undef RT_DIAG_DECLARE
#undef RT_DIAG_FLUSH
#undef RT_COUNT
#undef RT_COUNT_N
#define RT_DIAG_DECLARE() __shared__ unsigned int s_cnt[kBlock / 64][8]; if ((tid & 63) < 8) s_cnt[tid >> 6][tid & 7] = 0u
#define RT_COUNT(k) do { if ((int)(tid & 63) == (int)__builtin_ctzll(__ballot(true))) s_cnt[tid >> 6][k] += 1u; } while (0)
#define RT_COUNT_N(k, n) do { if ((int)(tid & 63) == (int)__builtin_ctzll(__ballot(true))) s_cnt[tid >> 6][k] += (unsigned)(n); } while (0)
#define RT_DIAG_FLUSH() do { if (lane == 0) for (int k_ = 0; k_ < 8; ++k_) atomicAdd(P.stats + 8 + k_, (unsigned long long)s_cnt[tid >> 6][k_]); } while (0)
#if defined(RT_COUNT_ROWS)
#undef RT_COUNT_ROWS_TRIP
#define RT_COUNT_ROWS_TRIP(k) RT_COUNT(k)
#elif defined(RT_COUNT_ENUM)
#undef RT_COUNT_ENUM_TRIP
#define RT_COUNT_ENUM_TRIP(m) do { RT_COUNT(1); RT_COUNT_N(6, __popcll(m)); } while (0)
#elif defined(RT_COUNT_REDRAW)
#undef RT_COUNT_REDRAW_LANES
#define RT_COUNT_REDRAW_LANES(ok) do { const unsigned n1_ = (unsigned)__popcll(__ballot(true)), n6_ = (unsigned)__popcll(__ballot(!(ok))); \
                                       RT_COUNT_N(1, n1_); RT_COUNT_N(6, n6_); } while (0)
#else
#undef RT_COUNT_MAIN
#define RT_COUNT_MAIN(k) RT_COUNT(k)
#endif
#endif

#if defined(RT_LDS_CONFLICTS)
namespace rt {
template <int BYTES, bool ATOMIC, bool LOAD64 = false>
__device__ __noinline__ uint32_t lds_extra_cycles(uint32_t byte_addr, bool active)
{
    constexpr int G = (BYTES == 8 && !LOAD64) ? 16 : 32;
    const int lane = threadIdx.x & 63;
    const unsigned long long m = __ballot(active);
    const uint32_t unit = byte_addr / (uint32_t)BYTES;
    const uint32_t bank = unit % (uint32_t)G;
    bool first = active;
    for (int k = 0; k < 64; ++k) {
        const uint32_t uk = (uint32_t)__builtin_amdgcn_readlane((int)unit, k);
        if (((m >> k) & 1ull) && k < lane && k / G == lane / G && uk == unit) first = false;
    }
    const unsigned long long counted = ATOMIC ? m : __ballot(first);
    uint32_t cnt = 0;
    for (int k = 0; k < 64; ++k) {
        const uint32_t bk = (uint32_t)__builtin_amdgcn_readlane((int)bank, k);
        if (((counted >> k) & 1ull) && k / G == lane / G && bk == bank) cnt++;
    }
    if (!active) cnt = 0;
    uint32_t extra = 0;
    for (int g = 0; g < 64 / G; ++g) {
        uint32_t mx = 0;
        for (int k = g * G; k < (g + 1) * G; ++k) mx = max(mx, (uint32_t)__builtin_amdgcn_readlane((int)cnt, k));
        extra += mx > 1u ? mx - 1u : 0u;
    }
    return extra;
}
}
#undef RT_DIAG_DECLARE
#undef RT_DIAG_FLUSH
#undef RT_LDS
#undef RT_LDS_N
#undef RT_LDS_QUEUE_READS
#undef RT_LDS_POOL_TIE
#undef RT_LDS_ENUM_READS
#undef RT_LDS_RING_ADDS
#define RT_DIAG_DECLARE() unsigned long long lds_x[8] = {0, 0, 0, 0, 0, 0, 0, 0}
#define RT_DIAG_FLUSH() do { if (lane == 0) for (int k_ = 0; k_ < 8; ++k_) atomicAdd(P.stats + 8 + k_, lds_x[k_]); } while (0)
#define RT_LDS(site, BYTES, ATOMIC, LOAD64, ptr, active) do { lds_x[site] += rt::lds_extra_cycles<BYTES, ATOMIC, LOAD64>( \
        (uint32_t)(uintptr_t)(const void __attribute__((address_space(3))) *)(ptr), (active)); } while (0)
#define RT_LDS_N(site, n, BYTES, ATOMIC, LOAD64, byte_addr, active) do { lds_x[site] += (unsigned long long)(n) * \
        rt::lds_extra_cycles<BYTES, ATOMIC, LOAD64>((uint32_t)(byte_addr), (active)); } while (0)
#define RT_LDS_QUEUE_READS(take, entry) do { const bool take_ = (take); const uint32_t e_ = take_ ? (entry) : 0u; \
        RT_LDS(6, 8, false, true, &quv_w[e_], take_); RT_LDS(6, 8, false, true, &quv_w[64 + e_], take_); \
        for (int c_ = 0; c_ < 5; ++c_) RT_LDS(6, 4, false, false, &qid_w[c_ * 64 + e_], take_); } while (0)
#define RT_LDS_POOL_TIE(has_root, r, key) do { const bool eq_ = (has_root) && best_w[r] == (key); RT_LDS(3, 4, true, false, &bidx_w[r], eq_); } while (0)
#define RT_LDS_ENUM_READS(has, word, summary, seg0) do { if constexpr (TUBE) { \
        const bool need_ = (has) && (word) == 0u; \
        const int w_ = need_ ? __builtin_ctz(summary) : 0; \
        RT_LDS(5, 4, false, false, &bits_w[w_ * 64 + lane], need_); \
        if (SMALLGRID || !list_all) RT_LDS(5, 4, false, false, &bits_w[(kSeg / 2) * 64 + (seg0) + w_], need_); } } while (0)
#define RT_LDS_RING_ADDS(ringed, my_blk) do { if (__ballot(ringed) != 0ull) { \
        unsigned long long *acc_d = ring_w + (((my_blk) >> 4) & (uint32_t)(kRingDepth - 1)) * (kRingSlots * 3) + ((my_blk) & 15u) * 3u; \
        RT_LDS(1, 8, true, false, acc_d + 0, ringed); RT_LDS(1, 8, true, false, acc_d + 1, ringed); RT_LDS(1, 8, true, false, acc_d + 2, ringed); } } while (0)
#endif
```

rtiow_amd/csrc/rt_frames.hip:

```cpp
#include <hip/hip_runtime.h>

#include <cstring>

#define RT_RENDER_KERNEL_ONLY
#include "rt_host.hpp"

using namespace rt_host;

namespace {

unsigned frames_block_items(int spp, int ring_min_spp, bool *use_ring)
{
    unsigned small_block = 0;
    for (unsigned items = rt::kItemBlock; items >= 64u && spp >= 1; items -= 64u)
        if ((items - 1u + (unsigned)spp - 1u) / (unsigned)spp + 1u <= 2u * (unsigned)rt::kRingSlots) { small_block = items; break; }
    *use_ring = small_block != 0u && spp >= ring_min_spp;
    return *use_ring ? small_block : (unsigned)rt::kItemBlock;
}

int validate_frames(const rt_context *ctx, int32_t n_frames, int32_t sample_stride, const rt_params *p)
{
    int rc = validate_params(p);
    if (rc) return rc;
    if (p->flags & (RT_FLAG_UNIFORM53 | RT_FLAG_DIAG_STATS | RT_FLAG_NO_FILTER))
        return fail(RT_ERR_INVALID_ARGUMENT, "frame batches run the shipped kernel only: RT_FLAG_UNIFORM53, RT_FLAG_DIAG_STATS and "
                    "RT_FLAG_NO_FILTER are not available on them (flags 0x%x)", p->flags);
    if (p->shard_count != 1)
        return fail(RT_ERR_INVALID_ARGUMENT, "frame batches are not sharded: shard_count must be 1 (is %d)", p->shard_count);
    if (n_frames < 0) return fail(RT_ERR_INVALID_ARGUMENT, "n_frames must be >= 0 (is %d)", n_frames);
    if (sample_stride < 0) return fail(RT_ERR_INVALID_ARGUMENT, "sample_stride must be >= 0 (is %d)", sample_stride);
    const long long frame_pix = (long long)p->width * p->height;
    if ((long long)n_frames * frame_pix > 0x80000000LL)
        return fail(RT_ERR_INVALID_ARGUMENT, "n_frames*width*height = %lld pixels in one batch: at most 2^31", (long long)n_frames * frame_pix);
    if (n_frames > 0 && (long long)p->sample_begin + (long long)(n_frames - 1) * sample_stride + p->spp > 0x7fffffffLL)
        return fail(RT_ERR_INVALID_ARGUMENT, "sample_begin + (n_frames-1)*sample_stride + spp = %lld: the last frame's sample indices must stay "
                    "below 2^31", (long long)p->sample_begin + (long long)(n_frames - 1) * sample_stride + p->spp);
    bool use_ring = false;
    const unsigned item_block = frames_block_items(p->spp, ctx ? ctx->ring_min_spp : 0, &use_ring);
    const unsigned long long frame_blocks = ((unsigned long long)frame_pix * (unsigned long long)p->spp + item_block - 1) / item_block;
    if (frame_blocks * (unsigned long long)n_frames > 0x7fffffffULL)
        return fail(RT_ERR_INVALID_ARGUMENT, "n_frames*ceil(width*height*spp / %u) = %llu work blocks in one batch: at most 2^31 - 1 "
                    "(split the batch, or the samples with sample_begin and RT_FLAG_ACCUMULATE)", item_block, frame_blocks * (unsigned long long)n_frames);
    if (!ctx) return fail(RT_ERR_INVALID_ARGUMENT, "ctx is NULL");
    if (ctx->scan_mode != 5)
        return fail(RT_ERR_INVALID_ARGUMENT, "frame batches need the shipped scan mode 5; this context was created under RTIOW_SCAN_MODE=%d", ctx->scan_mode);
    return RT_OK;
}

}

extern "C" {

int rt_render_frames_device(rt_context *ctx, const rt_camera *d_cams, int32_t n_frames, int32_t sample_stride,
                            const rt_params *p, void *d_fix, void *stream_v)
{
    int rc = validate_frames(ctx, n_frames, sample_stride, p);
    if (rc) return rc;
    if (ctx->n_spheres < 0) return fail(RT_ERR_NO_SCENE, "rt_upload_scene has not been called");
    if (n_frames == 0) return RT_OK;
    if (!d_cams || !d_fix) return fail(RT_ERR_INVALID_ARGUMENT, "d_cams/d_fix is NULL");
    const unsigned long long frame_pix = (unsigned long long)p->width * (unsigned long long)p->height;
    const unsigned long long frame_items = frame_pix * (unsigned long long)p->spp;
    const unsigned long long total_items = frame_items * (unsigned long long)n_frames;
    bool use_ring = false;
    const unsigned item_block = frames_block_items(p->spp, ctx->ring_min_spp, &use_ring);
    const unsigned long long frame_blocks = (frame_items + item_block - 1) / item_block;
    const unsigned long long n_blocks = frame_blocks * (unsigned long long)n_frames;
    RT_HIP(hipSetDevice(ctx->device));
    hipStream_t stream = (hipStream_t)stream_v;

    rt::KParams kp;
    memset(&kp, 0, sizeof(kp));
    static_assert(sizeof(rt::KCamera) == sizeof(rt_camera) && sizeof(rt_camera) == 19 * sizeof(double), "camera layouts must match");
    kp.width = p->width; kp.height = p->height;
    kp.spp = p->spp; kp.sample_begin = p->sample_begin; kp.max_depth = p->max_depth;
    kp.t_min = p->t_min;
    kp.k0 = (uint32_t)p->seed; kp.k1 = (uint32_t)(p->seed >> 32);
    kp.tile_rows = 1; kp.shard_index = 0; kp.shard_count = 1;
    kp.rows = p->height; kp.n_spheres = ctx->n_spheres;
    kp.npix = (uint32_t)(frame_pix * (unsigned long long)n_frames);
    kp.total_items = total_items; kp.n_blocks = (uint32_t)n_blocks;
    kp.inv_spp = p->spp > 0 ? 1.0 / (double)p->spp : 0.0;
    kp.inv_width = 1.0 / (double)p->width;
    auto magic_for = [](long long d) -> uint32_t {
        return (d <= 1 || d >= 32768) ? 0u : (uint32_t)(0x100000000ULL / (unsigned long long)d + 1ULL);
    };
    kp.magic_spp = magic_for(p->spp); kp.magic_width = magic_for(p->width);
    kp.use_ring = use_ring ? 1 : 0;
    kp.block_items = item_block;
    set_scene_params(ctx, kp);
    kp.fix = (unsigned long long *)d_fix;
    kp.cams = reinterpret_cast<const rt::KCamera *>(d_cams);
    kp.frame_items = frame_items;
    kp.frame_blocks = (uint32_t)frame_blocks;
    kp.inv_frame_blocks = frame_blocks > 0 ? 1.0 / (double)frame_blocks : 0.0;
    kp.frame_pix = (uint32_t)frame_pix;
    kp.sample_stride = sample_stride;
    rc = next_launch_slot(ctx, stream, kp);
    if (rc) return rc;

    if (!(p->flags & RT_FLAG_ACCUMULATE))
        RT_HIP(hipMemsetAsync(d_fix, 0, (size_t)(frame_pix * (unsigned long long)n_frames) * 3 * sizeof(unsigned long long), stream));
    RT_HIP(hipMemsetAsync(ctx->d_queue, 0, 64, stream));
    RT_HIP(hipMemsetAsync(ctx->d_stats, 0, 1024, stream));
    memset(&ctx->last, 0, sizeof(ctx->last));
    ctx->last.n_spheres = ctx->n_spheres;
    ctx->last.block_threads = rt::kBlock;
    ctx->zero_depth_samples = 0;
    if (p->max_depth == 0 || total_items == 0) {
        RT_HIP(hipEventRecord(ctx->ev0, stream));
        RT_HIP(hipEventRecord(ctx->ev1, stream));
        ctx->zero_depth_samples = total_items;
        ctx->last.scan_mode = 5;
        ctx->launched = true;
        return RT_OK;
    }
    int grid = 0;
    const bool small_grid = ctx->grid_dim > 0 && ctx->n_global + ctx->grid_dim * ctx->grid_dim <= 64;
    ctx->last.scan_mode = 5;
    ctx->last.kernel_variant = 16 | (small_grid ? 1 : 0);
    rc = small_grid ? launch_render<5, false, true, false, rt::kItemBlockFrames>(ctx, kp, stream, &grid)
                    : launch_render<5, false, false, false, rt::kItemBlockFrames>(ctx, kp, stream, &grid);
    if (rc) return rc;
    ctx->launched = true;
    ctx->last.grid_blocks = grid;
    return RT_OK;
}

int rt_render_frames(rt_context *ctx, const rt_camera *cams, int32_t n_frames, int32_t sample_stride,
                     const rt_params *p, uint64_t *out_fix, rt_stats *stats)
{
    int rc = validate_frames(ctx, n_frames, sample_stride, p);
    if (rc) return rc;
    if (ctx->n_spheres < 0) return fail(RT_ERR_NO_SCENE, "rt_upload_scene has not been called");
    if (n_frames == 0) return RT_OK;
    if (!cams || !out_fix) return fail(RT_ERR_INVALID_ARGUMENT, "cams/out_fix is NULL");
    RT_HIP(hipSetDevice(ctx->device));
    const size_t count = (size_t)n_frames * p->width * p->height * 3;
    rc = ensure(&ctx->d_stage_fix, &ctx->stage_fix_bytes, count * sizeof(uint64_t));
    if (rc) return rc;
    rc = ensure(&ctx->d_stage_cams, &ctx->stage_cams_bytes, (size_t)n_frames * sizeof(rt_camera));
    if (rc) return rc;
    RT_HIP(hipMemcpyAsync(ctx->d_stage_cams, cams, (size_t)n_frames * sizeof(rt_camera), hipMemcpyHostToDevice, ctx->own_stream));
    rt_params q = *p;
    q.flags &= ~RT_FLAG_ACCUMULATE;
    rc = rt_render_frames_device(ctx, (const rt_camera *)ctx->d_stage_cams, n_frames, sample_stride, &q, ctx->d_stage_fix, ctx->own_stream);
    if (rc) return rc;
    RT_HIP(hipMemcpyAsync(out_fix, ctx->d_stage_fix, count * sizeof(uint64_t), hipMemcpyDeviceToHost, ctx->own_stream));
    RT_HIP(hipStreamSynchronize(ctx->own_stream));
    if (stats) return rt_last_stats(ctx, stats);
    return RT_OK;
}

int rt_render_frames_rgba8(rt_context *ctx, const rt_camera *cams, int32_t n_frames, int32_t sample_stride,
                           const rt_params *p, int32_t flip, uint8_t *out_rgba, rt_stats *stats)
{
    int rc = validate_frames(ctx, n_frames, sample_stride, p);
    if (rc) return rc;
    if (p->spp < 1) return fail(RT_ERR_INVALID_ARGUMENT, "rt_render_frames_rgba8 needs spp >= 1 (to_rgba divides by the sample count, vec3.rs:409)");
    if (ctx->n_spheres < 0) return fail(RT_ERR_NO_SCENE, "rt_upload_scene has not been called");
    if (n_frames == 0) return RT_OK;
    if (!cams || !out_rgba) return fail(RT_ERR_INVALID_ARGUMENT, "cams/out_rgba is NULL");
    RT_HIP(hipSetDevice(ctx->device));
    const size_t frame_pix = (size_t)p->width * p->height;
    const size_t npix = frame_pix * (size_t)n_frames;
    rc = ensure(&ctx->d_stage_fix, &ctx->stage_fix_bytes, npix * 3 * sizeof(uint64_t));
    if (rc) return rc;
    rc = ensure(&ctx->d_stage_rgba, &ctx->stage_rgba_bytes, npix * 4);
    if (rc) return rc;
    rc = ensure(&ctx->d_stage_cams, &ctx->stage_cams_bytes, (size_t)n_frames * sizeof(rt_camera));
    if (rc) return rc;
    RT_HIP(hipMemcpyAsync(ctx->d_stage_cams, cams, (size_t)n_frames * sizeof(rt_camera), hipMemcpyHostToDevice, ctx->own_stream));
    rt_params q = *p;
    q.flags &= ~RT_FLAG_ACCUMULATE;
    rc = rt_render_frames_device(ctx, (const rt_camera *)ctx->d_stage_cams, n_frames, sample_stride, &q, ctx->d_stage_fix, ctx->own_stream);
    if (rc) return rc;
    if (!flip && (long long)n_frames * p->height <= 0x7fffffffLL) {
        rc = rt_resolve_rgba8_device(ctx, ctx->d_stage_fix, p->width, n_frames * p->height, (int64_t)p->spp, 0, ctx->d_stage_rgba, ctx->own_stream);
        if (rc) return rc;
    } else {
        for (int32_t f = 0; f < n_frames; ++f) {
            rc = rt_resolve_rgba8_device(ctx, (const uint64_t *)ctx->d_stage_fix + (size_t)f * frame_pix * 3, p->width, p->height, (int64_t)p->spp,
                                         flip, (uint8_t *)ctx->d_stage_rgba + (size_t)f * frame_pix * 4, ctx->own_stream);
            if (rc) return rc;
        }
    }
    RT_HIP(hipMemcpyAsync(out_rgba, ctx->d_stage_rgba, npix * 4, hipMemcpyDeviceToHost, ctx->own_stream));
    RT_HIP(hipStreamSynchronize(ctx->own_stream));
    if (stats) return rt_last_stats(ctx, stats);
    return RT_OK;
}

}
```

rtiow_amd/csrc/rt_host.hpp:

```cpp
#pragma once
#include <hip/hip_runtime.h>

#include "rtiow_hip.h"
#include "rt_kernels.hpp"
#ifdef RTIOW_CROSSCHECK_MODES
#include "xcheck/rt_xcheck_host_ctx.hpp"
#endif

namespace rt_host {
int fail(int code, const char *fmt, ...);
}

#define RT_HIP(call)                                                                          \
    do {                                                                                      \
        hipError_t e_ = (call);                                                               \
        if (e_ != hipSuccess)                                                                 \
            return rt_host::fail(e_ == hipErrorOutOfMemory ? RT_ERR_OUT_OF_MEMORY : RT_ERR_HIP,        \
                        "%s failed: %s (%s:%d)", #call, hipGetErrorString(e_), __FILE__, __LINE__); \
    } while (0)

struct rt_context {
    int device = 0;
    int cu_count = 0;
    float *d_filt = nullptr;
    double *d_geo = nullptr;
    double *d_mat = nullptr;
    uint4 *d_btube = nullptr;
    float tube_rho = 1.0f;
    double *d_geo_slot = nullptr;
    uint32_t *d_slot_orig = nullptr;
    int n_global = 0;
    int grid_dim = 0;
    float grid[8] = {};
    float scene_scale = 0.0f;
#ifdef RTIOW_CROSSCHECK_MODES
    XcheckScene x;
#endif
    int n_tiles = 0;
    int n_always = 0;
    int always_idx[8] = {0, 0, 0, 0, 0, 0, 0, 0};
    int scan_mode = 5;
    int n_spheres = -1;
    static constexpr int kSlots = 2;
    unsigned int *q_slots[kSlots] = {nullptr, nullptr};
    unsigned long long *s_slots[kSlots] = {nullptr, nullptr};
    hipEvent_t e0_slots[kSlots] = {nullptr, nullptr}, e1_slots[kSlots] = {nullptr, nullptr};
    bool slot_used[kSlots] = {false, false};
    int cur = 0;
    unsigned int *d_queue = nullptr;
    unsigned long long *d_stats = nullptr;
    hipEvent_t ev0 = nullptr, ev1 = nullptr;
    hipStream_t own_stream = nullptr;
    bool launched = false;
    unsigned long long zero_depth_samples = 0;
    rt_stats last{};
    void *d_stage_fix = nullptr; size_t stage_fix_bytes = 0;
    void *d_stage_sum = nullptr; size_t stage_sum_bytes = 0;
    void *d_stage_rgba = nullptr; size_t stage_rgba_bytes = 0;
    int blocks_per_cu = 0;
    void *d_sel = nullptr; size_t sel_bytes = 0;
    void *d_adapt = nullptr; size_t adapt_bytes = 0;
    void *d_stage_list = nullptr; size_t stage_list_bytes = 0;
    void *d_stage_cams = nullptr; size_t stage_cams_bytes = 0;
    int ring_min_spp = 0;
};

namespace rt_host {

int validate_params(const rt_params *p);
int ensure(void **ptr, size_t *have, size_t need);
void set_scene_params(const rt_context *ctx, rt::KParams &kp);
int next_launch_slot(rt_context *ctx, hipStream_t stream, rt::KParams &kp);

template <int MODE, bool DIAG, bool SMALLGRID = false, bool U53 = false, int ITEMS = rt::kItemBlock>
int launch_render(rt_context *ctx, const rt::KParams &kp, hipStream_t stream, int *grid_out)
{
    int per_cu = ctx->blocks_per_cu;
    if (per_cu <= 0) {
        int occ = 0;
        RT_HIP(hipOccupancyMaxActiveBlocksPerMultiprocessor(&occ, rt::render_kernel<MODE, DIAG, SMALLGRID, U53, ITEMS>, rt::kBlock, 0));
        per_cu = occ < 1 ? 1 : (occ > 8 ? 8 : occ);
    }
    long long grid = (long long)ctx->cu_count * per_cu;
    const long long need = (long long)((kp.total_items + rt::kBlock - 1) / rt::kBlock);
    if (grid > need) grid = need;
    if (grid < 1) grid = 1;
    *grid_out = (int)grid;
    RT_HIP(hipEventRecord(ctx->ev0, stream));
    hipLaunchKernelGGL((rt::render_kernel<MODE, DIAG, SMALLGRID, U53, ITEMS>), dim3((unsigned)grid), dim3(rt::kBlock), 0, stream, kp);
    RT_HIP(hipGetLastError());
    RT_HIP(hipEventRecord(ctx->ev1, stream));
    return RT_OK;
}

}
```

rtiow_amd/csrc/rt_kernels.hpp:

```cpp
#pragma once
#include "rt_device.hpp"
#include "rt_diag.hpp"
#ifdef RTIOW_CROSSCHECK_MODES
#include "xcheck/rt_xcheck_params.hpp"
#endif
#include <type_traits>

#ifndef RT_GROUP_SKIP
#define RT_GROUP_SKIP 1
#endif

namespace rt {

struct KCamera {
    double origin[3], llc[3], horizontal[3], vertical[3], u[3], v[3];
    double lens_radius;
};

struct KParams {
    KCamera cam;
    double t_min;
    int32_t width, height;
    int32_t spp, sample_begin, max_depth;
    uint32_t k0, k1;
    int32_t tile_rows, shard_index, shard_count;
    int32_t rows;
    int32_t n_spheres;
    int32_t use_ring;
    uint32_t npix;
    uint32_t n_blocks;
    unsigned long long total_items;
    double inv_spp;
    double inv_width;
    uint32_t magic_spp, magic_width, magic_tile;
    uint32_t block_items;
    const float *filt;
#ifdef RTIOW_CROSSCHECK_MODES
    KXcheckTables x;
#endif
    const uint4 *btube;
    float tube_rho;
    float scene_scale;
    const double *geo_slot;
    const uint32_t *slot_orig;
    float grid[8];
    int32_t grid_dim;
    unsigned long long grid_rows;
    int32_t n_global;
    int32_t n_tiles;
    int32_t n_always;
    int32_t always_idx[8];
    const double *geo;
    const double *mat;
    unsigned long long *fix;
    unsigned int *queue;
    unsigned long long *stats;
    const uint32_t *pix_list;
    const KCamera *cams;
    unsigned long long frame_items;
    double inv_frame_blocks;
    uint32_t frame_blocks;
    uint32_t frame_pix;
    int32_t sample_stride;
};

constexpr int RT_KIND_LAMBERTIAN = 0, RT_KIND_METAL = 1, RT_KIND_DIALECTRIC = 2;
constexpr int kBlock = 256;
constexpr int kCandCap = 24;
constexpr int kScanUnroll = 8;
constexpr int kItemBlock = 256;
constexpr int kItemBlockLarge = 1024;
constexpr int kItemBlockList = -kItemBlock;
constexpr int kItemBlockFrames = -2 * kItemBlock;
static_assert(kItemBlockLarge + 32768 < 65536, "udiv_small: numerators x < d + kItemBlockLarge with d < 2^15 keep x * d < 2^32");
constexpr int kLargeMinSpp = 147;
constexpr int kLargeMinSppSmallGrid = 69;
constexpr unsigned long long kLargeMinItems = 200000000ull;
constexpr int kRingSlots = 8;
constexpr int kRingDepth = 4;
constexpr int kMatStride = 10;
constexpr int kListCap = 126;
constexpr int kSegTilesTube = 28;
constexpr int kSegTiles = 36;

__device__ __forceinline__ D3 ld3(const double *p) { return mk(p[0], p[1], p[2]); }

__device__ __forceinline__ uint32_t udiv_small(uint32_t x, uint32_t d, uint32_t magic)
{
    const uint32_t big = x >= d ? 1u : 0u;
    const uint32_t q = __umulhi(x, magic);
    return d == 1u ? x : (d >= 32768u ? big : q);
}



constexpr int kRowPad = 80;

typedef float f32x4 __attribute__((ext_vector_type(4)));

template <int MODE, bool DIAG, bool SMALLGRID = false, bool U53 = false, int ITEMS = 256>
__global__ __launch_bounds__(kBlock, (MODE == 5 && !DIAG) ? 4 : (MODE >= 2) ? 3 : 5) void render_kernel(const KParams P)
{
    constexpr bool PIXLIST = ITEMS == kItemBlockList;
    constexpr bool FRAMES = ITEMS == kItemBlockFrames;
    static_assert(ITEMS > 0 || PIXLIST || FRAMES, "ITEMS: a block size, kItemBlockList or kItemBlockFrames");
    static_assert(!(PIXLIST || FRAMES) || (MODE == 5 && !DIAG && !U53), "pixel lists and frame batches: the shipped kernel, 32-bit uniforms, blocks of 256");
    constexpr bool kWideRing = SMALLGRID || (MODE == 5 && !DIAG && (ITEMS == kItemBlock || ITEMS == kItemBlockList || ITEMS == kItemBlockFrames));
    constexpr int kRingDepth = kWideRing ? 2 : 4;
    constexpr int kRingSlots = kWideRing ? 16 : 8;
    static_assert(kRingDepth * kRingSlots == rt::kRingDepth * rt::kRingSlots, "same LDS either way");
    __shared__ uint16_t cand[MODE == 1 ? kCandCap : 1][MODE == 1 ? kBlock : 1];
    constexpr bool MATRIX = (MODE >= 2);
    constexpr bool LIFTED = (MODE == 4);
    constexpr bool TUBE = (MODE == 5);
    constexpr bool RAYOP = (MODE == 2 || MODE == 3);
    __shared__ float s_rayop[RAYOP ? kBlock / 64 : 1][RAYOP ? 8 : 1][RAYOP ? kRowPad : 1];
    constexpr int kSeg = TUBE ? kSegTilesTube : kSegTiles;
    static_assert(TUBE || (kSeg / 2) * 64 * sizeof(unsigned int) >= 32 * kStageStride * sizeof(uint4), "operand staging fits the bitmap");
    static_assert(!TUBE || ((kSeg / 2) * 64 + kListCap + 2) * sizeof(unsigned int) == 64 * 4 * sizeof(uint4), "tube: staging = bitmap + tile list");
    constexpr int kBitWords = TUBE ? (kSeg / 2) * 64 + kListCap + 2 : (kSeg / 2) * 64;
    __shared__ __attribute__((aligned(16))) unsigned int s_bits[MATRIX ? kBlock / 64 : 1][MATRIX ? kBitWords : 1];
    __shared__ unsigned int s_sum[(MATRIX && !TUBE) ? kBlock : 1];
    __shared__ double s_quv[kBlock / 64][2][64];
    __shared__ unsigned int s_qid[kBlock / 64][5][64];
    __shared__ unsigned int s_pool[MATRIX ? kBlock / 64 : 1][MATRIX ? 128 : 1];
    __shared__ unsigned long long s_best[MATRIX ? kBlock : 1];
    __shared__ unsigned int s_bidx[MATRIX ? kBlock : 1];
    __shared__ unsigned long long s_ring[kBlock / 64][kRingDepth][kRingSlots * 3];
    __shared__ unsigned int s_rpix[kBlock / 64][kRingDepth];
    __shared__ unsigned int s_live[DIAG ? kBlock / 64 : 1][DIAG ? 64 : 1];
    __shared__ double s_thr[3][kBlock];

    const int tid = threadIdx.x;
    const int lane = tid & 63;
    {
        unsigned long long *z = &s_ring[tid >> 6][0][0];
        for (int k = lane; k < kRingDepth * kRingSlots * 3; k += 64) z[k] = 0ull;
        if (lane < kRingDepth) s_rpix[tid >> 6][lane] = 0u;
    }
    if (DIAG) s_live[tid >> 6][tid & 63] = 0u;
    auto rank_below = [](unsigned long long m) -> uint32_t {
        return __builtin_amdgcn_mbcnt_hi((uint32_t)(m >> 32), __builtin_amdgcn_mbcnt_lo((uint32_t)m, 0u));
    };

    const float __attribute__((address_space(4))) *filt =
        (const float __attribute__((address_space(4))) *)(uintptr_t)P.filt;
    const double *__restrict__ geo = P.geo;
    const double *__restrict__ mat = P.mat;
    const int n = P.n_spheres;
    const double t_min = P.t_min;
    const double wm1 = (double)(P.width - 1);
    const double hm1 = (double)(P.height - 1);

    bool dead = false, alive = false;
    uint32_t pix_local = 0, pix_global = 0;
    int s = 0;
    uint32_t my_frame = 0;
    uint32_t my_blk = 0;
    D3 o = mk(0, 0, 0), d = mk(0, 0, 1);
    int depth = 0;
    uint32_t ev = 0;
    uint32_t n_rays = 0, n_samples = 0, n_direct = 0;
    unsigned long long tot_cand = 0, tot_roots = 0;
    uint32_t blk_next = 0, blk_end = 0, blk_seq = 0xFFFFFFFFu, blk_pix0 = 0, blk_s0 = 0, blk_rr0 = 0, blk_i0 = 0;
    uint32_t blk_frame = 0, blk_sbase = (uint32_t)P.sample_begin;
    bool queue_empty = false;
    uint32_t q_head = 0, q_count = 0;
    double *quv_w = &s_quv[tid >> 6][0][0];
    unsigned int *qid_w = &s_qid[tid >> 6][0][0];
    unsigned long long *ring_w = &s_ring[tid >> 6][0][0];
    unsigned int *rpix_w = &s_rpix[tid >> 6][0];
    uint32_t rem0 = 0, rem1 = 0, rem2 = 0, rem3 = 0;
    static_assert(kRingDepth == 4 || kRingDepth == 2, "the block counters are written out for a ring of 4 or 2");
    auto flush_ring = [&](uint32_t e) {
        if (lane < kRingSlots * 3) {
            const unsigned long long v = ring_w[e * (kRingSlots * 3) + lane];
            if (v != 0ull) {
                atomicAdd(P.fix + (size_t)rpix_w[e] * 3u + (size_t)lane, v);
                ring_w[e * (kRingSlots * 3) + lane] = 0ull;
            }
        }
        __builtin_amdgcn_wave_barrier();
    };

    RT_DIAG_DECLARE();
    for (;;) {
        __builtin_amdgcn_s_setprio(1);
        RT_COUNT(0);
        bool fresh = false;
        double cam_u = 0.0, cam_v = 0.0;
        uint32_t lens_wx = 0u, lens_wy = 0u;
        for (;;) {
            const bool want = !alive && !dead && !fresh;
            const unsigned long long m = __ballot(want);
            if (m == 0ull) break;
            if (q_count == 0u) {
                RT_STAMP(0);
                if (blk_next == blk_end) {
                    uint32_t nb = 0xFFFFFFFFu;
                    if (!queue_empty) {
                        const int leader = (int)__builtin_ctzll(m);
                        if (lane == leader) nb = atomicAdd(P.queue, 1u);
                        nb = (uint32_t)__builtin_amdgcn_readfirstlane((int)__shfl(nb, leader));
                    }
                    if (nb >= P.n_blocks) {
                        queue_empty = true;
                        if (want) dead = true;
                        break;
                    }
                    uint32_t nb_f = nb;
                    if constexpr (FRAMES) {
                        uint32_t fr = (uint32_t)((double)nb * P.inv_frame_blocks);
                        long long br = (long long)nb - (long long)fr * (long long)P.frame_blocks;
                        if (br < 0) { fr -= 1u; br += (long long)P.frame_blocks; }
                        else if (br >= (long long)P.frame_blocks) { fr += 1u; br -= (long long)P.frame_blocks; }
                        blk_frame = (uint32_t)__builtin_amdgcn_readfirstlane((int)fr);
                        nb_f = (uint32_t)__builtin_amdgcn_readfirstlane((int)(uint32_t)br);
                        blk_sbase = (uint32_t)P.sample_begin + blk_frame * (uint32_t)P.sample_stride;
                    }
                    const unsigned long long W0 = (unsigned long long)nb_f * (unsigned long long)P.block_items;
                    const unsigned long long left = (FRAMES ? P.frame_items : P.total_items) - W0;
                    const uint32_t n_items = left < (unsigned long long)P.block_items ? (uint32_t)left : P.block_items;
                    uint32_t p0 = (uint32_t)((double)W0 * P.inv_spp);
                    long long rem = (long long)(W0 - (unsigned long long)p0 * (unsigned long long)(uint32_t)P.spp);
                    if (rem < 0) { p0 -= 1u; rem += (long long)P.spp; }
                    else if (rem >= (long long)P.spp) { p0 += 1u; rem -= (long long)P.spp; }
                    blk_pix0 = (uint32_t)__builtin_amdgcn_readfirstlane((int)p0);
                    blk_s0 = (uint32_t)__builtin_amdgcn_readfirstlane((int)(uint32_t)rem);
                    if constexpr (!PIXLIST) {
                    uint32_t rr0 = (uint32_t)((double)blk_pix0 * P.inv_width);
                    int i0 = (int)(blk_pix0 - rr0 * (uint32_t)P.width);
                    if (i0 < 0) { rr0 -= 1u; i0 += P.width; } else if (i0 >= P.width) { rr0 += 1u; i0 -= P.width; }
                    blk_rr0 = (uint32_t)__builtin_amdgcn_readfirstlane((int)rr0);
                    blk_i0 = (uint32_t)__builtin_amdgcn_readfirstlane(i0);
                    }
                    if constexpr (FRAMES) blk_pix0 += blk_frame * P.frame_pix;
                    blk_next = 0u; blk_end = (uint32_t)__builtin_amdgcn_readfirstlane((int)n_items);
                    blk_seq += 1u;
                    if (P.use_ring) {
                        if constexpr (kRingDepth == 4) {
                            if (rem3 != 0u) flush_ring(blk_seq & (uint32_t)(kRingDepth - 1));
                            rem3 = rem2; rem2 = rem1; rem1 = rem0; rem0 = blk_end;
                        } else {
                            if (rem1 != 0u) flush_ring(blk_seq & (uint32_t)(kRingDepth - 1));
                            rem1 = rem0; rem0 = blk_end;
                        }
                        if (lane == 0) rpix_w[blk_seq & (uint32_t)(kRingDepth - 1)] = blk_pix0;
                        __builtin_amdgcn_wave_barrier();
                    }
                }
                const uint32_t n_gen = min(64u, blk_end - blk_next);
                RT_COUNT_MAIN(1);
                if ((uint32_t)lane < n_gen) {
                    const uint32_t s_rel = blk_s0 + blk_next + (uint32_t)lane;
                    const uint32_t dq = udiv_small(s_rel, (uint32_t)P.spp, P.magic_spp);
                    uint32_t i, j, g_pix;
                    if constexpr (PIXLIST) {
                        g_pix = P.pix_list[blk_pix0 + dq];
                        uint32_t jq = (uint32_t)((double)g_pix * P.inv_width);
                        int ir = (int)(g_pix - jq * (uint32_t)P.width);
                        if (ir < 0) { jq -= 1u; ir += P.width; } else if (ir >= P.width) { jq += 1u; ir -= P.width; }
                        i = (uint32_t)ir; j = jq;
                    } else if constexpr (FRAMES) {
                        const uint32_t col = blk_i0 + dq;
                        const uint32_t rq = udiv_small(col, (uint32_t)P.width, P.magic_width);
                        i = col - rq * (uint32_t)P.width;
                        j = blk_rr0 + rq;
                        g_pix = j * (uint32_t)P.width + i;
                    } else {
                    const uint32_t col = blk_i0 + dq;
                    const uint32_t rq = udiv_small(col, (uint32_t)P.width, P.magic_width);
                    i = col - rq * (uint32_t)P.width;
                    const uint32_t rr = blk_rr0 + rq;
                    const uint32_t lt = udiv_small(rr, (uint32_t)P.tile_rows, P.magic_tile);
                    j = (lt * (uint32_t)P.shard_count + (uint32_t)P.shard_index) * (uint32_t)P.tile_rows
                                       + (rr - lt * (uint32_t)P.tile_rows);
                    g_pix = j * (uint32_t)P.width + i;
                    }
                    const uint32_t g_s = (FRAMES ? blk_sbase : (uint32_t)P.sample_begin) + (s_rel - dq * (uint32_t)P.spp);
                    U4 w = philox4x32_10(g_pix, g_s, 0u, 0u, P.k0, P.k1);
                    uint32_t g_ev = 1u;
                    const double u = ((double)i + (U53 ? u01_53(w.x, w.y) : u01(w.x))) / wm1;
                    const double v = ((double)j + (U53 ? u01_53(w.z, w.w) : u01(w.y))) / hm1;
                    uint32_t wx = w.z, wy = w.w;
                    if constexpr (U53) {
                        double lx, ly;
                        do {
                            w = philox4x32_10(g_pix, g_s, g_ev, 0u, P.k0, P.k1);
                            g_ev++;
                            lx = u11_53(w.x, w.y); ly = u11_53(w.z, w.w);
                        } while (!(lx * lx + ly * ly < 1.0));
                    } else
                    while (!unit_disk_accepts(wx, wy)) {
                        w = philox4x32_10(g_pix, g_s, g_ev, 0u, P.k0, P.k1);
                        g_ev++;
                        wx = w.x; wy = w.y;
                        if (!unit_disk_accepts(wx, wy)) { wx = w.z; wy = w.w; }
                    }
                    quv_w[0 * 64 + lane] = u;
                    quv_w[1 * 64 + lane] = v;
                    qid_w[0 * 64 + lane] = wx;
                    qid_w[1 * 64 + lane] = wy;
                    qid_w[2 * 64 + lane] = g_pix;
                    qid_w[3 * 64 + lane] = g_s;
                    qid_w[4 * 64 + lane] = (g_ev << 8) | dq;
                }
                blk_next += n_gen;
                q_head = 0u; q_count = n_gen;
                __builtin_amdgcn_wave_barrier();
                RT_STAMP(8);
            }
            const uint32_t r = rank_below(m);
            RT_LDS_QUEUE_READS(want && r < q_count, q_head + r);
            if (want && r < q_count) {
                const uint32_t e = q_head + r;
                cam_u = quv_w[0 * 64 + e]; cam_v = quv_w[1 * 64 + e];
                lens_wx = qid_w[0 * 64 + e]; lens_wy = qid_w[1 * 64 + e];
                pix_global = qid_w[2 * 64 + e];
                s = (int)qid_w[3 * 64 + e];
                const uint32_t meta = qid_w[4 * 64 + e];
                ev = meta >> 8;
                pix_local = blk_pix0 + (meta & 255u);
                my_blk = (blk_seq << 4) | (meta & 15u);
                if constexpr (FRAMES) my_frame = blk_frame;
                fresh = true;
            }
            const uint32_t cnt = (uint32_t)__popcll(m);
            const uint32_t took = cnt < q_count ? cnt : q_count;
            q_head += took; q_count -= took;
        }
        RT_STAMP(0);
        if (fresh) {
            double lx = u11(lens_wx), ly = u11(lens_wy);
            if constexpr (U53) {
                const U4 lb = philox4x32_10(pix_global, (uint32_t)s, ev - 1u, 0u, P.k0, P.k1);
                lx = u11_53(lb.x, lb.y); ly = u11_53(lb.z, lb.w);
            }
            if constexpr (!FRAMES) {
            const D3 cam_origin = ld3(P.cam.origin);
            const D3 rd = mk(lx, ly, 0.0) * P.cam.lens_radius;
            const D3 offset = ld3(P.cam.u) * rd.x + ld3(P.cam.v) * rd.y;
            o = cam_origin + offset;
            d = (((ld3(P.cam.llc) + ld3(P.cam.horizontal) * cam_u) + ld3(P.cam.vertical) * cam_v) - cam_origin) - offset;
            }
            s_thr[0][tid] = 1.0; s_thr[1][tid] = 1.0; s_thr[2][tid] = 1.0;
            depth = P.max_depth;
            alive = true;
        }
        if constexpr (FRAMES) {
            for (unsigned long long todo = __ballot(fresh); todo != 0ull;) {
                const uint32_t f = (uint32_t)__builtin_amdgcn_readlane((int)my_frame, (int)__builtin_ctzll(todo));
                const bool mine = fresh && my_frame == f;
                const unsigned long long ca = (unsigned long long)(uintptr_t)P.cams + (unsigned long long)f * sizeof(KCamera);
                const double __attribute__((address_space(4))) *c = (const double __attribute__((address_space(4))) *)(uintptr_t)(
                    (unsigned long long)(uint32_t)__builtin_amdgcn_readfirstlane((int)(uint32_t)ca) |
                    ((unsigned long long)(uint32_t)__builtin_amdgcn_readfirstlane((int)(uint32_t)(ca >> 32)) << 32));
                double cc[sizeof(KCamera) / sizeof(double)];
                for (int k = 0; k < (int)(sizeof(KCamera) / sizeof(double)); ++k) cc[k] = c[k];
                if (mine) {
                    const D3 cam_origin = mk(cc[0], cc[1], cc[2]);
                    const D3 rd = mk(u11(lens_wx), u11(lens_wy), 0.0) * cc[18];
                    const D3 offset = mk(cc[12], cc[13], cc[14]) * rd.x + mk(cc[15], cc[16], cc[17]) * rd.y;
                    o = cam_origin + offset;
                    d = (((mk(cc[3], cc[4], cc[5]) + mk(cc[6], cc[7], cc[8]) * cam_u) + mk(cc[9], cc[10], cc[11]) * cam_v) - cam_origin) - offset;
                }
                todo &= ~__ballot(mine);
            }
        }

        RT_STAMP(9);
        const unsigned long long alive_mask = __ballot(alive);
        if (alive_mask == 0ull) break;
        n_rays += (uint32_t)__popcll(alive_mask);
        if (DIAG && alive) atomicAdd(&s_live[tid >> 6][min(P.max_depth - depth, 63)], 1u);

        double closest = __builtin_inf();
        int hit = -1;
        uint32_t n_cand = 0, n_roots = 0;
        const double a = length_squared(d);
        auto exact_test_g = [&](int idx, const double4 g, auto ordered) {
            const D3 oc = o - mk(g.x, g.y, g.z);
            const double half_b = dot(oc, d);
            const double c = length_squared(oc) - g.w;
            const double disc = half_b * half_b - a * c;
            if (disc < 0.0) return;
            if constexpr (decltype(ordered)::value) {
                if (DIAG && !(half_b > 0.0 && c > 0.0)) n_roots++;
                const double sq = __builtin_sqrt(disc);
                double r = (-half_b - sq) / a;
                if (r < t_min || closest < r) {
                    r = (-half_b + sq) / a;
                    if (r < t_min || closest < r) return;
                }
                closest = r;
                hit = idx;
                return;
            }
            if (half_b > 0.0 && c > 0.0) return;
            if (DIAG) n_roots++;
            const double sqrtd = __builtin_sqrt(disc);
            double root = (-half_b - sqrtd) / a;
            if (root < t_min) {
                root = (-half_b + sqrtd) / a;
                if (root < t_min) return;
            }
            if (root < closest || (root == closest && idx > hit)) {
                closest = root;
                hit = idx;
            }
        };
        auto exact_test = [&](int idx, auto ordered) {
            exact_test_g(idx, *reinterpret_cast<const double4 *>(geo + 4 * (size_t)idx), ordered);
        };
        auto test_list = [&](int cnt) {
            for (int k = 0; __any(k < cnt); ++k) {
                if (k < cnt) { if (DIAG) n_cand++; exact_test((int)cand[k][tid], std::true_type{}); }
            }
        };

        if (MATRIX) {
            const int wave = tid >> 6;
            const int col = lane & 15, quad = lane >> 4;
            const f32x4 zero = {0.0f, 0.0f, 0.0f, 0.0f};
            unsigned int *bits_w = &s_bits[wave][0];
            unsigned int *sum_w = &s_sum[TUBE ? 0 : wave * 64];
#ifdef RTIOW_CROSSCHECK_MODES
#include "xcheck/rt_xcheck_looks.inc"
#endif
            auto f64_key = [](double x) -> unsigned long long { return (unsigned long long)__double_as_longlong(x); };
            auto key_f64 = [](unsigned long long k) -> double { return __longlong_as_double((long long)k); };
            auto from_lane_f64 = [](int byte_addr, double x) -> double {
                const long long b = __double_as_longlong(x);
                const int lo = __builtin_amdgcn_ds_bpermute(byte_addr, (int)(b & 0xFFFFFFFFll));
                const int hi = __builtin_amdgcn_ds_bpermute(byte_addr, (int)(b >> 32));
                return __longlong_as_double(((long long)hi << 32) | (long long)(unsigned int)lo);
            };
            unsigned int *pool_w = &s_pool[wave][0];
            unsigned long long *best_w = &s_best[wave * 64];
            unsigned int *bidx_w = &s_bidx[wave * 64];
            constexpr bool SEED = TUBE && !SMALLGRID;
            if constexpr (!SEED) {
                best_w[lane] = 0x7FF0000000000000ull;
                bidx_w[lane] = 0u;
            }
            uint32_t pool_n = 0, pool_done = 0;
            auto pool_round = [&]() {
                RT_STAMP(10);
                RT_COUNT(5);
                const uint32_t e_i = pool_done + (uint32_t)lane;
                const bool act = e_i < pool_n;
                const uint32_t e = act ? pool_w[e_i & 127u] : (uint32_t)lane;
                const int r = (int)(e & 63u), slot = (int)(e >> 6);
                const int idx = TUBE ? (int)P.slot_orig[slot] : slot;
                const double *__restrict__ pgeo = TUBE ? P.geo_slot : geo;
                const int src = r << 2;
                const D3 ro = mk(from_lane_f64(src, o.x), from_lane_f64(src, o.y), from_lane_f64(src, o.z));
                const D3 rd = mk(from_lane_f64(src, d.x), from_lane_f64(src, d.y), from_lane_f64(src, d.z));
                bool has_root = false;
                unsigned long long key = 0ull;
                if (act) {
                    if (DIAG) n_cand++;
                    const double4 g = *reinterpret_cast<const double4 *>(pgeo + 4 * (size_t)slot);
                    const double ra = length_squared(rd);
                    const D3 oc = ro - mk(g.x, g.y, g.z);
                    const double half_b = dot(oc, rd);
                    const double c = length_squared(oc) - g.w;
                    const double disc = half_b * half_b - ra * c;
                    if (!(disc < 0.0) && !(half_b > 0.0 && c > 0.0)) {
                        if (DIAG) n_roots++;
                        const double sqrtd = __builtin_sqrt(disc);
                        double root = (-half_b - sqrtd) / ra;
                        if (root < t_min) root = (-half_b + sqrtd) / ra;
                        if (!(root < t_min)) {
                            key = f64_key(root);
                            has_root = true;
                        }
                    }
                }
                unsigned long long old = 0ull;
                RT_LDS_N(4, 12, 4, false, false, src, true);
                RT_LDS(2, 8, true, false, &best_w[r], has_root);
                if (has_root) old = atomicMin(&best_w[r], key);
                __builtin_amdgcn_wave_barrier();
                RT_LDS(3, 4, false, false, &bidx_w[r], has_root && old > key);
                if (has_root && old > key) bidx_w[r] = 0u;
                __builtin_amdgcn_wave_barrier();
                RT_LDS(7, 8, false, true, &best_w[r], has_root);
                RT_LDS_POOL_TIE(has_root, r, key);
                if (has_root && best_w[r] == key) atomicMax(&bidx_w[r], (unsigned)idx + 1u);
                __builtin_amdgcn_wave_barrier();
                pool_done = min(pool_done + 64u, pool_n);
                RT_STAMP(2);
            };
            bool list_all = true;
            auto enumerate = [&](int seg0, int nwords_tube = 0) {
                unsigned summary = 0u, word = 0u;
                if constexpr (TUBE) {
                    for (int w = 0; w < nwords_tube; ++w) summary |= min(bits_w[w * 64 + lane], 1u) << w;
                    if (!alive) summary = 0u;
                } else {
                    summary = alive ? s_sum[tid] : 0u;
                }
                int wbase = 0;
                for (;;) {
                    const bool has = (summary | word) != 0u;
                    const unsigned long long m = __ballot(has);
                    if (m == 0ull) break;
                    RT_COUNT_ENUM_TRIP(m);
                    RT_LDS_ENUM_READS(has, word, summary, seg0);
                    if (has) {
                        if (word == 0u) {
                            const int w = __builtin_ctz(summary);
                            summary &= summary - 1u;
                            word = bits_w[w * 64 + lane];
                            if constexpr (TUBE)
                                wbase = 32 * (!SMALLGRID && list_all ? seg0 + w : (int)(bits_w[(kSeg / 2) * 64 + seg0 + w] & 0x0FFFFFFFu));
                            else
                                wbase = 16 * seg0 + 32 * w;
                        }
                        const int bpos = __builtin_ctz(word);
                        word &= word - 1u;
                        const uint32_t pos = pool_n + rank_below(m);
                        pool_w[pos & 127u] = ((uint32_t)(wbase + bpos) << 6) | (uint32_t)lane;
                    }
                    pool_n += (uint32_t)__popcll(m);
                    if (pool_n - pool_done >= 64u) pool_round();
                }
            };
            auto finish_pool = [&]() {
                RT_STAMP(10);
                while (pool_done < pool_n) pool_round();
                const unsigned int hb = bidx_w[lane];
                if constexpr (SEED) {
                    if (alive) { hit = (int)hb - 1; closest = key_f64(best_w[lane]); }
                } else
                if (alive && hb != 0u) {
                    const double root = key_f64(best_w[lane]);
                    const int idx = (int)hb - 1;
                    if (root < closest || (root == closest && idx > hit)) { closest = root; hit = idx; }
                }
            };
            const int nt = P.n_tiles;

            if constexpr (TUBE) {
                const double4 g_first = *reinterpret_cast<const double4 *>(geo + 4 * (size_t)(P.n_always > 0 ? P.always_idx[0] : 0));
                const bool scan = alive;
                const unsigned long long scan_mask = __ballot(scan);
                if (scan_mask != 0ull) {
                float ray_of[3], ray_df[3], ray_o1;
                ray_f32(o, d, ray_of, ray_df, ray_o1);
                TubeRay T = make_tube<false>(ray_of, ray_df, ray_o1, P.tube_rho);
                if (!scan) T.sane = true;
                if (__builtin_expect(__ballot(!scan || !T.sane) != 0ull, 0)) {
                    if (!scan || !T.sane) tube_rows_keep_nothing(T);
                }
                bf16x8 A[4];
                {
                    uint32_t w[2][8];
                    tube_a_words(T, w);
                    tube_stage_operands(reinterpret_cast<uint4 *>(bits_w), lane, w, A);
                }
                if (alive)
                    for (int e = 0; e < P.n_always; ++e) {
                        if (DIAG) n_cand++;
                        if (e == 0) exact_test_g(P.always_idx[0], g_first, std::false_type{});
                        else exact_test(P.always_idx[e], std::false_type{});
                    }
                if (scan && !T.sane) {
                    closest = __builtin_inf(); hit = -1;
                    for (int i = 0; i < n; ++i) { if (DIAG) n_cand++; exact_test(i, std::true_type{}); }
                }
                if constexpr (SEED) {
                    best_w[lane] = f64_key(closest);
                    bidx_w[lane] = (unsigned)(hit + 1);
                }
                typedef float f32x16 __attribute__((ext_vector_type(16)));
                const int ntt = nt >> 1;
                const __amdgpu_buffer_rsrc_t brs = __builtin_amdgcn_make_buffer_rsrc(
                    const_cast<uint4 *>(P.btube), 0, (ntt + 1) * 1024, 0x00020000);
                const int voff = lane * 16;
                auto load_b = [&](int t32) -> bf16x8 {
                    return __builtin_bit_cast(bf16x8, __builtin_amdgcn_raw_buffer_load_b128(brs, voff, t32 * 1024, 0));
                };
                const int col32 = lane & 31, hh = lane >> 5;
                const f32x16 zero16 = {0, 0, 0, 0, 0, 0, 0, 0, 0, 0, 0, 0, 0, 0, 0, 0};
                auto keeps = [](uint32_t x) -> bool { return __builtin_fabsf(__uint_as_float(x)) < kTubeKeepBelow; };
                auto look_tube = [&](int G, const f32x16 &acc, int wrel) {
                    uint32_t X[2];
#pragma unroll
                    for (int bb = 0; bb < 2; ++bb) {
                        X[bb] = __float_as_uint(acc[8 * bb]) | __float_as_uint(acc[8 * bb + 4]);
#pragma unroll
                        for (int j = 1; j < 4; ++j)
                            X[bb] = __builtin_amdgcn_bitop3_b32(X[bb], __float_as_uint(acc[8 * bb + j]), __float_as_uint(acc[8 * bb + 4 + j]), 0xE0);
                    }
                    const unsigned long long kh[2] = {__ballot(keeps(X[0])), __ballot(keeps(X[1]))};
                    if (__builtin_expect((kh[0] | kh[1]) != 0ull, 0)) {
                        RT_COUNT(3);
                        int colv = col32;
                        asm volatile("" : "+v"(colv));
                        const unsigned bit = 1u << colv;
                        int rbase = wrel * 64 + 4 * hh;
                        unsigned int *row = bits_w + rbase;
#pragma unroll
                        for (int bb = 0; bb < 2; ++bb) {
                            if (kh[bb] != 0ull) {
                                RT_COUNT(4);
#pragma unroll
                                for (int j = 0; j < 4; ++j) {
                                    RT_LDS(0, 4, true, false, &row[16 * G + 8 * bb + j],
                                           keeps(__float_as_uint(acc[8 * bb + j]) | __float_as_uint(acc[8 * bb + 4 + j])));
                                    if (keeps(__float_as_uint(acc[8 * bb + j]) | __float_as_uint(acc[8 * bb + 4 + j])))
                                        atomicOr(&row[16 * G + 8 * bb + j], bit);
                                }
                            }
                        }
                    }
                };
                int n_list = ntt;
                unsigned int *tl = bits_w + (kSeg / 2) * 64;
                auto wave_or = [](int v) -> int {
                    v |= __builtin_amdgcn_update_dpp(0, v, 0x111, 0xF, 0xF, true);
                    v |= __builtin_amdgcn_update_dpp(0, v, 0x112, 0xF, 0xF, true);
                    v |= __builtin_amdgcn_update_dpp(0, v, 0x114, 0xF, 0xF, true);
                    v |= __builtin_amdgcn_update_dpp(0, v, 0x118, 0xF, 0xF, true);
                    v |= __builtin_amdgcn_update_dpp(0, v, 0x142, 0xA, 0xF, false);
                    v |= __builtin_amdgcn_update_dpp(0, v, 0x143, 0xC, 0xF, false);
                    return __builtin_amdgcn_readlane(v, 63);
                };
                auto rows_or = [](int v) -> int {
                    v |= __builtin_amdgcn_update_dpp(0, v, 0x111, 0xF, 0xF, true);
                    v |= __builtin_amdgcn_update_dpp(0, v, 0x112, 0xF, 0xF, true);
                    v |= __builtin_amdgcn_update_dpp(0, v, 0x114, 0xF, 0xF, true);
                    v |= __builtin_amdgcn_update_dpp(0, v, 0x118, 0xF, 0xF, true);
                    return v;
                };
                auto wave_scan_add = [](int v) -> int {
                    v += __builtin_amdgcn_update_dpp(0, v, 0x111, 0xF, 0xF, true);
                    v += __builtin_amdgcn_update_dpp(0, v, 0x112, 0xF, 0xF, true);
                    v += __builtin_amdgcn_update_dpp(0, v, 0x114, 0xF, 0xF, true);
                    v += __builtin_amdgcn_update_dpp(0, v, 0x118, 0xF, 0xF, true);
                    v += __builtin_amdgcn_update_dpp(0, v, 0x142, 0xA, 0xF, false);
                    v += __builtin_amdgcn_update_dpp(0, v, 0x143, 0xC, 0xF, false);
                    return v;
                };
                if (SMALLGRID || P.grid_dim > 0) {
                    int ix0 = 0, nx = 0, iz0 = 0, nz = 0, cnt = 0;
                    GridSeg seg;
                    RT_STAMP(5);
                    if (scan && T.sane) cnt = grid_cells(ray_of, ray_df, ray_o1, P.grid, P.grid_dim, P.scene_scale, ix0, nx, iz0, nz, SMALLGRID ? nullptr : &seg);
                    RT_STAMP(7);
                    const int gcells = P.grid_dim * P.grid_dim;
                    if (SMALLGRID || P.n_global + gcells <= 64) {
                        unsigned long long m = cnt < 0 ? ~0ull : 0ull;
                        if (cnt > 0) {
                            const unsigned long long run = (unsigned long long)(((1u << nx) - 1u) << ix0);
                            const unsigned long long rows = P.grid_rows & (~0ull >> (64 - nz * P.grid_dim));
                            m = (run * rows) << (iz0 * P.grid_dim);
                        }
#if RT_GROUP_SKIP
                        const int vlo = rows_or((int)(unsigned)m), vhi = rows_or((int)(unsigned)(m >> 32));
                        unsigned mlo = 0u, mhi = 0u, gm = 0u;
#pragma unroll
                        for (int g = 0; g < 4; ++g) {
                            const unsigned lo = (unsigned)__builtin_amdgcn_readlane(vlo, 16 * g + 15), hi = (unsigned)__builtin_amdgcn_readlane(vhi, 16 * g + 15);
                            mlo |= lo; mhi |= hi;
                            if (__builtin_amdgcn_inverse_ballot_w64(((unsigned long long)hi << 32) | lo)) gm |= 1u << g;
                        }
                        const unsigned kAll = 0xF0000000u;
#else
                        const unsigned mlo = (unsigned)wave_or((int)(unsigned)m), mhi = (unsigned)wave_or((int)(unsigned)(m >> 32));
                        const unsigned gm = 0u, kAll = 0u;
#endif
                        const unsigned long long cells = (((unsigned long long)mhi << 32) | mlo) & (~0ull >> (64 - gcells));
                        const int rank = (int)__builtin_amdgcn_mbcnt_hi(mhi, __builtin_amdgcn_mbcnt_lo(mlo, 0u));
                        tl[lane] = (unsigned)(lane < P.n_global ? lane : ntt) | kAll;
                        if (lane < 2) tl[64 + lane] = (unsigned)ntt | kAll;
                        __builtin_amdgcn_wave_barrier();
                        if ((cells >> lane) & 1ull) tl[P.n_global + rank] = (unsigned)(P.n_global + lane) | (gm << 28);
                        __builtin_amdgcn_wave_barrier();
                        list_all = false;
                        n_list = P.n_global + __builtin_popcountll(cells);
                    } else if (!SMALLGRID && __ballot(cnt < 0) == 0ull) {
                        if (cnt == 0) nz = 0;
                        auto build_list = [&](auto zero) {
                            typedef decltype(zero) W;
                            constexpr int kGroups = RT_GROUP_SKIP ? 4 : 1;
                            W *tm = reinterpret_cast<W *>(bits_w);
#pragma unroll
                            for (int g = 0; g < kGroups; ++g) tm[g * 64 + lane] = (W)0;
                            int lg_ = lane;
                            asm volatile("" : "+v"(lg_));
                            W *tm_g = tm + (RT_GROUP_SKIP ? (lg_ >> 4) * 64 : 0);
                            __builtin_amdgcn_wave_barrier();
                            for (int k = 0; __any(k < nz); ++k) {
                                RT_COUNT_ROWS_TRIP(1);
                                if (k < nz) {
                                    int rx0, rnx;
                                    grid_row_run(seg, ix0, ix0 + nx - 1, (float)(iz0 + k), rx0, rnx);
                                    atomicOr(&tm_g[iz0 + k], (W)((W)(~(W)0 >> (8 * (int)sizeof(W) - rnx)) << rx0));
                                }
                            }
                            __builtin_amdgcn_wave_barrier();
                            W wg[kGroups];
                            W mw = (W)0;
#pragma unroll
                            for (int g = 0; g < kGroups; ++g) { wg[g] = tm[g * 64 + lane]; mw |= wg[g]; }
                            const int mine = sizeof(W) == 8 ? __builtin_popcountll(mw) : __builtin_popcount((unsigned)mw);
                            const int upto = wave_scan_add(mine);
                            const int tn = P.n_global + __builtin_amdgcn_readlane(upto, 63);
                            if (tn <= kListCap) {
                                const unsigned kAll = RT_GROUP_SKIP ? 0xF0000000u : 0u;
                                if (lane < P.n_global) tl[lane] = (unsigned)lane | kAll;
                                int pos = P.n_global + upto - mine;
                                const int row0 = P.n_global + lane * P.grid_dim;
                                while (__any(mw != (W)0)) {
                                    RT_COUNT_ROWS_TRIP(6);
                                    if (mw != (W)0) {
                                        const int bpos = sizeof(W) == 8 ? __builtin_ctzll(mw) : __builtin_ctz((unsigned)mw);
                                        unsigned gm = 0u;
#pragma unroll
                                        for (int g = 0; g < (RT_GROUP_SKIP ? 4 : 0); ++g) gm |= (unsigned)((wg[g] >> bpos) & (W)1) << g;
                                        tl[pos++] = (unsigned)(row0 + bpos) | (gm << 28);
                                        mw &= mw - (W)1;
                                    }
                                }
                                int ntt_ = ntt;
                                asm volatile("" : "+s"(ntt_));
                                if (lane < 2) tl[tn + lane] = (unsigned)ntt_ | kAll;
                                __builtin_amdgcn_wave_barrier();
                                list_all = false;
                                n_list = tn;
                            }
                        };
                        if (P.grid_dim <= 32) build_list(0u); else build_list(0ull);
                    }
                }
                RT_STAMP(3);
                RT_STAMP(5);
                for (int t0 = 0; t0 < n_list; t0 += kSeg / 2) {
                    __builtin_amdgcn_s_setprio(3);
                    const int nwords = min(kSeg / 2, n_list - t0);
                    for (int w = 0; w < nwords; ++w) bits_w[w * 64 + lane] = 0u;
                    const int listv = !SMALLGRID && list_all ? (min(t0 + lane, ntt) | (RT_GROUP_SKIP ? (int)0xF0000000u : 0))
                                                             : (int)tl[min(t0 + lane, kListCap + 1)];
                    auto tile_at = [&](int j) -> int { return __builtin_amdgcn_readlane(listv, j) & 0x0FFFFFFF; };
                    auto groups_at = [&](int j) -> unsigned { return (unsigned)__builtin_amdgcn_readlane(listv, j) >> 28; };
                    __builtin_amdgcn_wave_barrier();
                    auto do_tile = [&](int w, const bf16x8 &b, unsigned groups) {
                        RT_COUNT(7);
                        RT_COUNT_N(2, __builtin_popcount(groups));
#if RT_GROUP_SKIP
                        if (groups != 0xFu) {
#pragma unroll
                            for (int G = 0; G < 4; ++G)
                                if ((groups >> G) & 1u) {
                                    f32x16 acc = __builtin_amdgcn_mfma_f32_32x32x16_bf16(A[G], b, zero16, 0, 0, 0);
                                    look_tube(G, acc, w);
                                }
                            return;
                        }
#endif
                        f32x16 acc0 = __builtin_amdgcn_mfma_f32_32x32x16_bf16(A[0], b, zero16, 0, 0, 0);
                        f32x16 acc1 = __builtin_amdgcn_mfma_f32_32x32x16_bf16(A[1], b, zero16, 0, 0, 0);
                        asm volatile("" : "+v"(acc1));
                        look_tube(0, acc0, w);
                        acc0 = __builtin_amdgcn_mfma_f32_32x32x16_bf16(A[2], b, zero16, 0, 0, 0);
                        asm volatile("" : "+v"(acc0));
                        look_tube(1, acc1, w);
                        acc1 = __builtin_amdgcn_mfma_f32_32x32x16_bf16(A[3], b, zero16, 0, 0, 0);
                        asm volatile("" : "+v"(acc1));
                        look_tube(2, acc0, w);
                        look_tube(3, acc1, w);
                    };
                    {
                        bf16x8 bp = load_b(tile_at(0)), bq;
                        int w = 0;
                        for (; w + 1 < nwords; w += 2) {
                            bq = load_b(tile_at(w + 1));
                            do_tile(w, bp, groups_at(w));
                            bp = load_b(tile_at(w + 2));
                            do_tile(w + 1, bq, groups_at(w + 1));
                        }
                        if (w < nwords) do_tile(w, bp, groups_at(w));
                    }
                    __builtin_amdgcn_wave_barrier();
                    RT_STAMP(6);
                    __builtin_amdgcn_s_setprio(2);
                    enumerate(t0, nwords);
                }
                __builtin_amdgcn_s_setprio(1);
                finish_pool();
                __builtin_amdgcn_s_setprio(0);
                }
            }
#ifdef RTIOW_CROSSCHECK_MODES
#include "xcheck/rt_xcheck_scan.inc"
#endif
        }
        RT_STAMP(2);
        if (alive && !MATRIX) {
            if (MODE == 0) {
                for (int i = 0; i < n; ++i) { if (DIAG) n_cand++; exact_test(i, std::true_type{}); }
            } else {
                const RayFilter f = make_filter(o, d);
                int cnt = 0;
                auto drain = [&]() { test_list(cnt); cnt = 0; };
                auto test = [&](float cx, float cy, float cz, float kp, int i) {
                    const bool keep = filter_keeps(f, cx, cy, cz, kp);
                    if (__builtin_expect(__ballot(keep) != 0ull, 0)) {
                        if (keep) {
                            cand[cnt][tid] = (uint16_t)i;
                            cnt++;
                        }
                    }
                };
                constexpr int BW = 4 * kScanUnroll;
                const int nb = n / kScanUnroll;
                for (int bidx = 0; bidx < nb; ++bidx) {
                    const float __attribute__((address_space(4))) *q = filt + (size_t)BW * (size_t)bidx;
                    float rec[BW];
#pragma unroll
                    for (int k = 0; k < BW; ++k) rec[k] = q[k];
#pragma unroll
                    for (int k = 0; k < kScanUnroll; ++k)
                        test(rec[4 * k + 0], rec[4 * k + 1], rec[4 * k + 2], rec[4 * k + 3], bidx * kScanUnroll + k);
                    if (__any(cnt > kCandCap - kScanUnroll)) drain();
                }
                for (int i = nb * kScanUnroll; i < n; ++i) {
                    const float __attribute__((address_space(4))) *q = filt + 4 * (size_t)i;
                    test(q[0], q[1], q[2], q[3], i);
                }
                drain();
            }
        }

        if (DIAG) {
            unsigned long long pk = (unsigned long long)n_cand | ((unsigned long long)n_roots << 32);
#pragma unroll
            for (int sh = 32; sh >= 1; sh >>= 1) pk += __shfl_xor(pk, sh);
            tot_cand += pk & 0xFFFFFFFFull; tot_roots += pk >> 32;
        }
        RT_STAMP(3);
        bool finished = false;
        D3 radiance = mk(0.0, 0.0, 0.0);
        if (alive) {
            bool done = false;
            D3 L = mk(0.0, 0.0, 0.0);
            const bool is_hit = hit >= 0;
            int kind = -1;
            bool front = false;
            D3 p = o, nrm = mk(0.0, 0.0, 0.0), sp = mk(0.0, 0.0, 0.0), albedo = mk(1.0, 1.0, 1.0);
            double param = 0.0, inv_param = 0.0, r0_front = 0.0, r0_back = 0.0;
            uint32_t w_first = 0u, w_second = 0u;
            if (is_hit) {
                const double *mrec = mat + kMatStride * (size_t)hit;
                const double4 g = *reinterpret_cast<const double4 *>(geo + 4 * (size_t)hit);
                const double2 mA = *reinterpret_cast<const double2 *>(mrec);
                const double2 mB = *reinterpret_cast<const double2 *>(mrec + 2);
                const double2 mC = *reinterpret_cast<const double2 *>(mrec + 4);
                const double2 mD_ = *reinterpret_cast<const double2 *>(mrec + 6);
                const double2 mE_ = *reinterpret_cast<const double2 *>(mrec + 8);
                U4 w = philox4x32_10(pix_global, (uint32_t)s, ev, 0u, P.k0, P.k1);
                asm volatile("" : "+v"(w.x), "+v"(w.y), "+v"(w.z), "+v"(w.w));
                kind = (int)mC.y;
                param = mA.y;
                albedo = mk(mB.x, mB.y, mC.x);
                p = o + d * closest;
                const D3 outward = (p - mk(g.x, g.y, g.z)) * mA.x;
                front = dot(d, outward) < 0.0;
                nrm = front ? outward : (mk(0.0, 0.0, 0.0) - outward);
                w_first = w.x;
                if constexpr (U53) w_second = w.y;
                RT_STAMP(11);
                if constexpr (U53) {
                  if (kind != RT_KIND_DIALECTRIC) {
                    U4 b1 = philox4x32_10(pix_global, (uint32_t)s, ev + 1u, 0u, P.k0, P.k1);
                    uint32_t nblk = 2u, c0 = b1.z, c1 = b1.w;
                    double sx = u11_53(w.x, w.y), sy = u11_53(w.z, w.w), sz = u11_53(b1.x, b1.y);
                    bool ok = sx * sx + sy * sy + sz * sz < 1.0;
                    while (!ok) {
                        RT_COUNT_MAIN(6);
                        U4 b = philox4x32_10(pix_global, (uint32_t)s, ev + nblk, 0u, P.k0, P.k1);
                        nblk++;
                        sx = u11_53(c0, c1); sy = u11_53(b.x, b.y); sz = u11_53(b.z, b.w);
                        ok = sx * sx + sy * sy + sz * sz < 1.0;
                        if (!ok) {
                            b = philox4x32_10(pix_global, (uint32_t)s, ev + nblk, 0u, P.k0, P.k1);
                            b1 = philox4x32_10(pix_global, (uint32_t)s, ev + nblk + 1u, 0u, P.k0, P.k1);
                            nblk += 2u;
                            sx = u11_53(b.x, b.y); sy = u11_53(b.z, b.w); sz = u11_53(b1.x, b1.y);
                            c0 = b1.z; c1 = b1.w;
                            ok = sx * sx + sy * sy + sz * sz < 1.0;
                        }
                    }
                    ev += nblk;
                    sp = mk(sx, sy, sz);
                  } else {
                    inv_param = mD_.x; r0_front = mD_.y; r0_back = mE_.x;
                  }
                } else
                if (kind != RT_KIND_DIALECTRIC) {
                    uint32_t tx = w.x, ty = w.y, tz = w.z, nblk = 1u;
                    bool ok = unit_sphere_accepts(tx, ty, tz);
                    RT_COUNT_REDRAW_LANES(ok);
                    if (!ok) {
                        uint32_t c0 = w.w;
                        do {
                            RT_COUNT_MAIN(6);
                            U4 b = philox4x32_10(pix_global, (uint32_t)s, ev + nblk, 0u, P.k0, P.k1);
                            nblk++;
                            tx = c0; ty = b.x; tz = b.y;
                            ok = unit_sphere_accepts(tx, ty, tz);
                            if (!ok) {
                                const uint32_t c1 = b.z, c2 = b.w;
                                b = philox4x32_10(pix_global, (uint32_t)s, ev + nblk, 0u, P.k0, P.k1);
                                nblk++;
                                tx = c1; ty = c2; tz = b.x;
                                ok = unit_sphere_accepts(tx, ty, tz);
                                if (!ok) {
                                    tx = b.y; ty = b.z; tz = b.w;
                                    ok = unit_sphere_accepts(tx, ty, tz);
                                    if (!ok) {
                                        b = philox4x32_10(pix_global, (uint32_t)s, ev + nblk, 0u, P.k0, P.k1);
                                        nblk++;
                                        tx = b.x; ty = b.y; tz = b.z; c0 = b.w;
                                        ok = unit_sphere_accepts(tx, ty, tz);
                                    }
                                }
                            }
                        } while (!ok);
                    }
                    ev += nblk;
                    sp = mk(u11(tx), u11(ty), u11(tz));
                } else {
                    inv_param = mD_.x; r0_front = mD_.y; r0_back = mE_.x;
                }
            }
            RT_STAMP(12);
            D3 V = d;
            if (kind == RT_KIND_LAMBERTIAN) V = sp;
            if (kind == RT_KIND_METAL) V = reflect(d, nrm);
            const D3 uV = unit_vector(V);
            if (!is_hit) {
                const double t = 0.5 * (uV.y + 1.0);
                const D3 sky = mk(1.0, 1.0, 1.0) * (1.0 - t) + mk(0.5, 0.7, 1.0) * t;
                L = mk(s_thr[0][tid], s_thr[1][tid], s_thr[2][tid]) * sky;
                done = true;
            } else {
                D3 ndir;
                if (kind == RT_KIND_LAMBERTIAN) {
                    ndir = nrm + uV;
                    const double eps = 1e-8;
                    const bool near_zero = __builtin_fabs(ndir.x) < eps && __builtin_fabs(ndir.y) < eps && __builtin_fabs(ndir.z) < eps;
                    if (__builtin_expect(__ballot(near_zero) != 0ull, 0)) {
                        if (near_zero) ndir = nrm;
                    }
                } else if (kind == RT_KIND_METAL) {
                    ndir = uV + sp * param;
                    if (dot(ndir, nrm) <= 0.0) done = true;
                } else {
                    const double ratio = front ? inv_param : param;
                    const double cos_theta = min_1(-dot(uV, nrm));
                    const double sin_theta = __builtin_sqrt(1.0 - cos_theta * cos_theta);
                    bool do_refract = false;
                    if (ratio * sin_theta <= 1.0) {
                        const double r0 = front ? r0_front : r0_back;
                        const double x = 1.0 - cos_theta;
                        const double x2 = x * x;
                        const double refl = r0 + (1.0 - r0) * ((x2 * x2) * x);
                        ev++;
                        do_refract = refl <= (U53 ? u01_53(w_first, w_second) : u01(w_first));
                    }
                    ndir = do_refract ? refract(uV, nrm, ratio) : reflect(uV, nrm);
                }
                if (kind != RT_KIND_DIALECTRIC) {
                    s_thr[0][tid] = s_thr[0][tid] * albedo.x;
                    s_thr[1][tid] = s_thr[1][tid] * albedo.y;
                    s_thr[2][tid] = s_thr[2][tid] * albedo.z;
                }
                o = p;
                d = ndir;
                depth -= 1;
                if (depth <= 0) done = true;
            }
            if (done) {
                alive = false;
                finished = true;
                radiance = L;
            }
        }
        RT_STAMP(13);
        __builtin_amdgcn_s_setprio(1);
        {
            const uint32_t age = (blk_seq - (my_blk >> 4)) & 0x0FFFFFFFu;
            const bool direct = finished && !(P.use_ring && age < (uint32_t)kRingDepth);
            const bool ringed = finished && !direct;
            RT_LDS_RING_ADDS(ringed, my_blk);
            if (finished) {
                const unsigned long long q0 = quantize(radiance.x), q1 = quantize(radiance.y), q2 = quantize(radiance.z);
                if (ringed) {
                    unsigned long long *acc = ring_w + ((my_blk >> 4) & (uint32_t)(kRingDepth - 1)) * (kRingSlots * 3) + (my_blk & 15u) * 3u;
                    atomicAdd(acc + 0, q0); atomicAdd(acc + 1, q1); atomicAdd(acc + 2, q2);
                } else {
                    unsigned long long *px = P.fix + (size_t)pix_local * 3u;
                    atomicAdd(px + 0, q0); atomicAdd(px + 1, q1); atomicAdd(px + 2, q2);
                }
            }
            n_direct += (uint32_t)__popcll(__ballot(direct));
            unsigned long long fm = __ballot(ringed);
            if (fm != 0ull) {
                __builtin_amdgcn_wave_barrier();
                const unsigned long long m0 = __ballot(ringed && age == 0u);
                rem0 -= (uint32_t)__popcll(m0);
                if (m0 != 0ull && rem0 == 0u) flush_ring(blk_seq & (uint32_t)(kRingDepth - 1));
                fm &= ~m0;
                if constexpr (kRingDepth == 2) {
                    if (fm != 0ull) {
                        rem1 -= (uint32_t)__popcll(fm);
                        if (rem1 == 0u) flush_ring((blk_seq - 1u) & 1u);
                    }
                } else
                if (fm != 0ull) {
                    const unsigned long long m1 = __ballot(ringed && age == 1u);
                    rem1 -= (uint32_t)__popcll(m1);
                    if (m1 != 0ull && rem1 == 0u) flush_ring((blk_seq - 1u) & 3u);
                    fm &= ~m1;
                    if (fm != 0ull) {
                        const unsigned long long m2 = __ballot(ringed && age == 2u);
                        rem2 -= (uint32_t)__popcll(m2);
                        if (m2 != 0ull && rem2 == 0u) flush_ring((blk_seq - 2u) & 3u);
                        fm &= ~m2;
                        if (fm != 0ull) {
                            rem3 -= (uint32_t)__popcll(fm);
                            if (rem3 == 0u) flush_ring((blk_seq - 3u) & 3u);
                        }
                    }
                }
            }
        }
        n_samples += (uint32_t)__popcll(__ballot(finished));
        RT_STAMP(4);
    }
    if (rem0 != 0u) flush_ring(blk_seq & (uint32_t)(kRingDepth - 1));
    if (rem1 != 0u) flush_ring((blk_seq - 1u) & (uint32_t)(kRingDepth - 1));
    if constexpr (kRingDepth == 4) {
        if (rem2 != 0u) flush_ring((blk_seq - 2u) & 3u);
        if (rem3 != 0u) flush_ring((blk_seq - 3u) & 3u);
    }

    RT_DIAG_FLUSH();
    {
        const unsigned long long nc = tot_cand, nr = tot_roots;
        if (DIAG) {
            const unsigned int nl = s_live[tid >> 6][lane];
            if (nl) atomicAdd(P.stats + 16 + lane, (unsigned long long)nl);
        }
        if (lane == 0) {
            atomicAdd(P.stats + 0, (unsigned long long)n_rays);
            atomicAdd(P.stats + 1, (unsigned long long)n_samples);
            if (n_direct) atomicAdd(P.stats + 4, (unsigned long long)n_direct);
            atomicAdd(P.stats + 2, nc);
            atomicAdd(P.stats + 3, nr);
        }
    }
}

#ifndef RT_RENDER_KERNEL_ONLY
__device__ __forceinline__ double fix_to_f64(unsigned long long q)
{
    return ((double)(uint32_t)(q >> 32) * 4294967296.0 + (double)(uint32_t)q) * (1.0 / 4294967296.0);
}

__global__ void fix_to_f32_kernel(const unsigned long long *__restrict__ fix, float *__restrict__ out, long long count)
{
    long long k = (long long)blockIdx.x * blockDim.x + threadIdx.x;
    const long long stride = (long long)gridDim.x * blockDim.x;
    for (; k < count; k += stride) out[k] = (float)fix_to_f64(fix[k]);
}

__device__ __forceinline__ uint8_t as_u8(double x)
{
    if (!(x == x)) return 0;
    if (x <= 0.0) return 0;
    if (x >= 255.0) return 255;
    return (uint8_t)x;
}
__device__ __forceinline__ double clamp_r(double x, double lo, double hi)
{
    if (x < lo) return lo;
    if (x > hi) return hi;
    return x;
}
__global__ void resolve_rgba8_kernel(const unsigned long long *__restrict__ fix, uint8_t *__restrict__ out,
                                     int width, int rows, double scale, int flip)
{
    long long k = (long long)blockIdx.x * blockDim.x + threadIdx.x;
    const long long npix = (long long)width * rows;
    const long long stride = (long long)gridDim.x * blockDim.x;
    for (; k < npix; k += stride) {
        const int r = (int)(k / width);
        const int i = (int)(k - (long long)r * width);
        const int dst = flip ? rows - 1 - r : r;
        const unsigned long long *q = fix + k * 3;
        uchar4 px;
        px.x = as_u8(256.0 * clamp_r(__builtin_sqrt(scale * fix_to_f64(q[0])), 0.0, 0.999));
        px.y = as_u8(256.0 * clamp_r(__builtin_sqrt(scale * fix_to_f64(q[1])), 0.0, 0.999));
        px.z = as_u8(256.0 * clamp_r(__builtin_sqrt(scale * fix_to_f64(q[2])), 0.0, 0.999));
        px.w = 255;
        reinterpret_cast<uchar4 *>(out)[(long long)dst * width + i] = px;
    }
}

__global__ void resolve_rgba8_counts_kernel(const unsigned long long *__restrict__ fix, const uint32_t *__restrict__ count,
                                            uint8_t *__restrict__ out, int width, int rows, int flip)
{
    long long k = (long long)blockIdx.x * blockDim.x + threadIdx.x;
    const long long npix = (long long)width * rows;
    const long long stride = (long long)gridDim.x * blockDim.x;
    for (; k < npix; k += stride) {
        const int r = (int)(k / width);
        const int i = (int)(k - (long long)r * width);
        const int dst = flip ? rows - 1 - r : r;
        const unsigned long long *q = fix + k * 3;
        const double scale = 1.0 / (double)count[k];
        uchar4 px;
        px.x = as_u8(256.0 * clamp_r(__builtin_sqrt(scale * fix_to_f64(q[0])), 0.0, 0.999));
        px.y = as_u8(256.0 * clamp_r(__builtin_sqrt(scale * fix_to_f64(q[1])), 0.0, 0.999));
        px.z = as_u8(256.0 * clamp_r(__builtin_sqrt(scale * fix_to_f64(q[2])), 0.0, 0.999));
        px.w = 255;
        reinterpret_cast<uchar4 *>(out)[(long long)dst * width + i] = px;
    }
}

__host__ __device__ inline bool select_noisy(const unsigned long long *fix, const unsigned long long *half, double sc, double threshold,
                                             double dark_floor)
{
    double D = 0.0, S = 0.0;
    for (int c = 0; c < 3; ++c) {
        const long long t = (long long)(2ull * half[c] - fix[c]);
        const unsigned long long d = t < 0 ? (unsigned long long)(-t) : (unsigned long long)t;
        D = c == 0 ? (double)d : D + (double)d;
        S = c == 0 ? (double)fix[c] : S + (double)fix[c];
    }
    const double m = S * sc;
    const double err = (D * sc) / __builtin_sqrt(m > dark_floor ? m : dark_floor);
    return !(err <= threshold);
}

constexpr int kSelBlock = 256;

__global__ __launch_bounds__(kSelBlock) void select_noisy_kernel(const unsigned long long *__restrict__ fix, const unsigned long long *__restrict__ half,
                                                                 const uint32_t *__restrict__ count, uint32_t npix, uint32_t n, double sc,
                                                                 double threshold, double dark_floor, uint8_t *__restrict__ noisy)
{
    const uint32_t p = blockIdx.x * (uint32_t)kSelBlock + threadIdx.x;
    if (p >= npix) return;
    noisy[p] = (count[p] == n && select_noisy(fix + (size_t)p * 3u, half + (size_t)p * 3u, sc, threshold, dark_floor)) ? 1 : 0;
}

__global__ __launch_bounds__(kSelBlock) void select_active_kernel(const uint8_t *__restrict__ noisy, const uint32_t *__restrict__ count,
                                                                  int width, int height, uint32_t n, uint8_t *__restrict__ active,
                                                                  uint32_t *__restrict__ block_count)
{
    __shared__ uint32_t s_cnt[kSelBlock / 64];
    const uint32_t npix = (uint32_t)width * (uint32_t)height;
    const uint32_t p = blockIdx.x * (uint32_t)kSelBlock + threadIdx.x;
    bool act = false;
    if (p < npix && count[p] == n) {
        const int j = (int)(p / (uint32_t)width), i = (int)(p - (uint32_t)j * (uint32_t)width);
        const int j0 = j > 0 ? j - 1 : 0, j1 = j < height - 1 ? j + 1 : height - 1;
        const int i0 = i > 0 ? i - 1 : 0, i1 = i < width - 1 ? i + 1 : width - 1;
        for (int jj = j0; jj <= j1; ++jj)
            for (int ii = i0; ii <= i1; ++ii) act = act || noisy[(size_t)jj * (size_t)width + (size_t)ii] != 0;
    }
    if (p < npix) active[p] = act ? 1 : 0;
    const unsigned long long m = __ballot(act);
    if ((threadIdx.x & 63) == 0) s_cnt[threadIdx.x >> 6] = (uint32_t)__popcll(m);
    __syncthreads();
    if (threadIdx.x == 0) block_count[blockIdx.x] = s_cnt[0] + s_cnt[1] + s_cnt[2] + s_cnt[3];
}

__global__ __launch_bounds__(1024) void select_scan_kernel(uint32_t *__restrict__ block_count, uint32_t n_blocks, uint32_t *__restrict__ n_out)
{
    __shared__ uint32_t s_wave[16];
    __shared__ uint32_t s_carry;
    const uint32_t tid = threadIdx.x, lane = tid & 63u, wave = tid >> 6;
    if (tid == 0) s_carry = 0u;
    __syncthreads();
    for (uint32_t base = 0; base < n_blocks; base += 1024u) {
        const uint32_t k = base + tid;
        const uint32_t v = k < n_blocks ? block_count[k] : 0u;
        uint32_t x = v;
        for (int d = 1; d < 64; d <<= 1) {
            const uint32_t y = (uint32_t)__shfl_up((int)x, d);
            if (lane >= (uint32_t)d) x += y;
        }
        if (lane == 63u) s_wave[wave] = x;
        __syncthreads();
        uint32_t before = s_carry;
        for (uint32_t w = 0; w < wave; ++w) before += s_wave[w];
        if (k < n_blocks) block_count[k] = before + x - v;
        __syncthreads();
        if (tid == 1023u) s_carry = before + x;
        __syncthreads();
    }
    if (tid == 0) *n_out = s_carry;
}

__global__ __launch_bounds__(kSelBlock) void select_write_kernel(const uint8_t *__restrict__ active, const uint32_t *__restrict__ block_offset,
                                                                 uint32_t npix, uint32_t *__restrict__ list)
{
    __shared__ uint32_t s_cnt[kSelBlock / 64];
    const uint32_t p = blockIdx.x * (uint32_t)kSelBlock + threadIdx.x;
    const bool act = p < npix && active[p] != 0;
    const unsigned long long m = __ballot(act);
    if ((threadIdx.x & 63) == 0) s_cnt[threadIdx.x >> 6] = (uint32_t)__popcll(m);
    __syncthreads();
    uint32_t at = block_offset[blockIdx.x];
    for (uint32_t w = 0; w < (threadIdx.x >> 6); ++w) at += s_cnt[w];
    at += __builtin_amdgcn_mbcnt_hi((uint32_t)(m >> 32), __builtin_amdgcn_mbcnt_lo((uint32_t)m, 0u));
    if (act) list[at] = p;
}

__global__ void add_back_kernel(const uint32_t *__restrict__ list, uint32_t n_list, const unsigned long long *__restrict__ pass,
                                unsigned long long *__restrict__ fix, unsigned long long *__restrict__ half, uint32_t *__restrict__ count,
                                uint32_t step)
{
    const uint32_t k = blockIdx.x * blockDim.x + threadIdx.x;
    if (k >= n_list) return;
    const size_t g = list[k];
    for (int c = 0; c < 3; ++c) {
        const unsigned long long v = pass[(size_t)k * 3u + c];
        fix[g * 3u + c] += v;
        if (half) half[g * 3u + c] += v;
    }
    count[g] += step;
}

__global__ void fill_u32_kernel(uint32_t *__restrict__ dst, uint32_t value, uint32_t n)
{
    const uint32_t k = blockIdx.x * blockDim.x + threadIdx.x;
    if (k < n) dst[k] = value;
}

__global__ void stats_accumulate_kernel(const unsigned long long *__restrict__ stats, unsigned long long *__restrict__ total)
{
    if (threadIdx.x < 5) total[threadIdx.x] += stats[threadIdx.x];
}

__global__ void philox_kat_kernel(uint32_t c0, uint32_t c1, uint32_t c2, uint32_t c3,
                                  uint32_t k0, uint32_t k1, uint32_t *out)
{
    const U4 r = philox4x32_10(c0, c1, c2, c3, k0, k1);
    out[0] = r.x; out[1] = r.y; out[2] = r.z; out[3] = r.w;
}


__global__ __launch_bounds__(64) void tube_products_kernel(const double *o, const double *d, const uint4 *tile, float rho,
                                                         float *h_out, float *rows_out)
{
    typedef float f32x16 __attribute__((ext_vector_type(16)));
    __shared__ uint4 stage[64 * 4];
    const int lane = threadIdx.x, col = lane & 31, hh = lane >> 5;
    const TubeRay T = make_tube(mk(o[3 * lane], o[3 * lane + 1], o[3 * lane + 2]),
                                mk(d[3 * lane], d[3 * lane + 1], d[3 * lane + 2]), rho);
    for (int k = 0; k < 2; ++k) for (int i = 0; i < 3; ++i) rows_out[lane * 9 + 3 * k + i] = T.u[k][i];
    rows_out[lane * 9 + 6] = T.t[0]; rows_out[lane * 9 + 7] = T.t[1]; rows_out[lane * 9 + 8] = T.sane ? 1.0f : 0.0f;
    bf16x8 A[4];
    uint32_t w[2][8];
    tube_a_words(T, w);
    tube_stage_operands(stage, lane, w, A);
    const bf16x8 b = __builtin_bit_cast(bf16x8, tile[lane]);
    const f32x16 zero16 = {0, 0, 0, 0, 0, 0, 0, 0, 0, 0, 0, 0, 0, 0, 0, 0};
    for (int G = 0; G < 4; ++G) {
        const f32x16 acc = __builtin_amdgcn_mfma_f32_32x32x16_bf16(A[G], b, zero16, 0, 0, 0);
        for (int bb = 0; bb < 2; ++bb)
            for (int j = 0; j < 4; ++j) {
                const int ray = 16 * G + 8 * bb + 4 * hh + j;
                h_out[(ray * 32 + col) * 2 + 0] = acc[8 * bb + j];
                h_out[(ray * 32 + col) * 2 + 1] = acc[8 * bb + 4 + j];
            }
    }
}

__global__ void f64_div_sqrt_kernel(const double *a, const double *b, int n, double *q, double *r)
{
    const int k = blockIdx.x * blockDim.x + threadIdx.x;
    if (k < n) { q[k] = a[k] / b[k]; r[k] = __builtin_sqrt(a[k]); }
}

__global__ void quantize_kernel(const double *x, int n, unsigned long long *q)
{
    const int k = blockIdx.x * blockDim.x + threadIdx.x;
    if (k < n) q[k] = quantize(x[k]);
}

__global__ void unit_accept_kernel(const uint32_t *w, int n, uint32_t *acc, double *uni)
{
    const int k = blockIdx.x * blockDim.x + threadIdx.x;
    if (k < n) {
        const uint32_t x = w[3 * k], y = w[3 * k + 1], z = w[3 * k + 2];
        acc[k] = (unit_sphere_accepts(x, y, z) ? 1u : 0u) | (unit_disk_accepts(x, y) ? 2u : 0u);
        uni[4 * k] = u01(x); uni[4 * k + 1] = u11(x); uni[4 * k + 2] = u11(y); uni[4 * k + 3] = u11(z);
    }
}

#endif

}

#if defined(RTIOW_CROSSCHECK_MODES) && !defined(RT_RENDER_KERNEL_ONLY)
#include "xcheck/rt_xcheck_kernels.hpp"
#endif
```

Before: 8301.

## Skip self-intersection tests against the sphere a ray just left

After a bounce off a non-dielectric sphere, if the outgoing direction points far enough outward (a bound derived from float error, scene reach and t_min), the kernel records that sphere's slot in LDS and clears its bit in the candidate tile mask, so the next bounce never tests it. This removes one redundant ray-sphere intersection per bounce on the small-grid tube path. Per-sphere radius and slot are packed into a spare material field, and a host-side threshold is computed per launch. The threshold is what keeps the drop bit-exact, so a mistake in it could change which hit is found. A new counting build is added to check the drop.

```diff
diff --git a/__graft_entry__.py b/__graft_entry__.py
--- a/__graft_entry__.py
+++ b/__graft_entry__.py
@@ -15,11 +15,13 @@
 ]
 
 
-def build_hip_library(crosscheck=False):
-    out = os.path.join(ROOT, "tools", "librtiow_hip_xcheck.so") if crosscheck else os.path.join(ROOT, "rtiow_amd", "librtiow_hip.so")
-    srcs = [os.path.join(ROOT, "rtiow_amd", "csrc", name) for name in ("rt_api.hip", "rt_frames.hip")]
+def build_hip_library(crosscheck=False, count_own=False):
+    out = (os.path.join(ROOT, "tools", "librtiow_hip_xcheck.so") if crosscheck else
+           os.path.join(ROOT, "tools", "lib_counts_own.so") if count_own else os.path.join(ROOT, "rtiow_amd", "librtiow_hip.so"))
+    srcs = [os.path.join(ROOT, "rtiow_amd", "csrc", name) for name in ("rt_api.hip", "rt_frames.hip", "rt_own.hip")]
     import bench
     cmd = ["hipcc", *HIPCC_FLAGS, *(["-DRTIOW_CROSSCHECK_MODES"] if crosscheck else []),
+           *(["-DRT_BLOCK_COUNTS", "-DRT_COUNT_OWN"] if count_own else []),
            f'-DRT_SOURCE_SHA="{bench.kernel_source_sha()}"',
            "-I", os.path.join(ROOT, "include"), "-I", os.path.join(ROOT, "rtiow_amd", "csrc"), "-o", out, *srcs]
     subprocess.run(cmd, check=True, cwd=ROOT)
@@ -42,6 +44,7 @@
 def build() -> None:
     build_hip_library()
     build_hip_library(crosscheck=True)
+    build_hip_library(count_own=True)
     build_host_cli()
     subprocess.run(["make", "-s", "-C", os.path.join(ROOT, "oracle"), "liboracle.so"], check=True)
     import rtiow_amd
diff --git a/rtiow_amd/csrc/rt_api.hip b/rtiow_amd/csrc/rt_api.hip
--- a/rtiow_amd/csrc/rt_api.hip
+++ b/rtiow_amd/csrc/rt_api.hip
@@ -6,6 +6,7 @@
 #include <cstdio>
 #include <cstdlib>
 #include <cstring>
+#include <limits>
 #include <vector>
 
 #include "rt_host.hpp"
@@ -203,6 +204,39 @@
     kp.scene_scale = ctx->scene_scale;
     kp.n_always = ctx->n_always;
     for (int e = 0; e < 8; ++e) kp.always_idx[e] = ctx->always_idx[e];
+}
+
+double rt_host::camera_reach(const rt_camera *cams, int n)
+{
+    double reach = 0.0;
+    for (int k = 0; k < n; ++k) {
+        const rt_camera &c = cams[k];
+        auto len = [](const double v[3]) { return std::sqrt(v[0] * v[0] + v[1] * v[1] + v[2] * v[2]); };
+        const double r = len(c.origin) + std::fabs(c.lens_radius) * (len(c.u) + len(c.v));
+        if (!(r <= reach)) reach = r;
+    }
+    return reach;
+}
+
+float rt_host::own_sphere_threshold(const rt_context *ctx, double cam_reach, double t_min)
+{
+    constexpr double kOwnK = 48.0;
+    const float off = std::numeric_limits<float>::infinity();
+    const char *env = getenv("RTIOW_OWN_DROP");
+    if (env && env[0] == '0') return off;
+    if (ctx->scan_mode != 5 || !(cam_reach >= 0.0)) return off;
+    const double rho = cam_reach > ctx->own_reach ? cam_reach : ctx->own_reach;
+    if (!(rho >= 1e-100 && rho <= 1e100) || !(t_min >= 1e-200 && t_min <= 1e200)) return off;
+    const double D = 2.0 * rho * (1.0 + 0x1p-19);
+    const double E = kOwnK * 0x1p-53 * D * D;
+    if (!(ctx->own_rmin * ctx->own_rmin >= 4.0 * E)) return off;
+    double g = 2.05 * E / t_min;
+    if (g < 1e-14 * rho) g = 1e-14 * rho;
+    if (g < 1e-30) g = 1e-30;
+    g *= 1.01;
+    float gf = (float)g;
+    if ((double)gf < g) gf = std::nextafterf(gf, off);
+    return gf;
 }
 
 int rt_host::next_launch_slot(rt_context *ctx, hipStream_t stream, rt::KParams &kp)
@@ -536,6 +570,28 @@
             }
             tube_tile(col, ctx->tube_rho, &btube[t * 64], &rtube[t * 32]);
         }
+        ctx->own_reach = 0.0; ctx->own_rmin = std::numeric_limits<double>::infinity();
+        for (int i = 0; i < n; ++i) {
+            const rt_sphere &s = spheres[i];
+            const double reach = std::sqrt(s.center[0] * s.center[0] + s.center[1] * s.center[1] + s.center[2] * s.center[2]) + std::fabs(s.radius);
+            if (reach > ctx->own_reach) ctx->own_reach = reach;
+        }
+        for (size_t slot = 0; slot < slot_of.size(); ++slot) {
+            const int i = slot_of[slot];
+            if (i < 0) continue;
+            const rt_sphere &s = spheres[i];
+            float f = 0.0f;
+            if (s.radius > 0.0 && s.kind != RT_DIALECTRIC && (s.kind != RT_METAL || (s.param >= 0.0 && s.param <= 1.0))) {
+                f = (float)s.radius;
+                if ((double)f > s.radius) f = std::nextafterf(f, 0.0f);
+                if (!(f >= std::numeric_limits<float>::min()) || slot + 1 > 0xFFFFu) f = 0.0f;
+            }
+            uint32_t fb; memcpy(&fb, &f, 4);
+            fb &= 0xFFFF0000u;
+            if (fb != 0u && s.radius < ctx->own_rmin) ctx->own_rmin = s.radius;
+            const unsigned long long rec = fb != 0u ? (unsigned long long)((uint32_t)(slot + 1) | fb) : 0ull;
+            memcpy(&mat[(size_t)rt::kMatStride * i + 9], &rec, 8);
+        }
         if (!rc) rc = upload_table(&ctx->d_btube, btube.data(), btube.size());
         if (!rc) rc = upload_table(&ctx->d_geo_slot, geo_slot.data(), geo_slot.size());
         if (!rc) rc = upload_table(&ctx->d_slot_orig, slot_orig.data(), slot_orig.size());
@@ -636,6 +692,7 @@
     kp.use_ring = use_ring ? 1 : 0;
     kp.block_items = item_block;
     set_scene_params(ctx, kp);
+    kp.own_g = own_sphere_threshold(ctx, camera_reach(cam, 1), p->t_min);
     kp.fix = (unsigned long long *)d_fix;
     rc = next_launch_slot(ctx, stream, kp);
     if (rc) return rc;
@@ -667,6 +724,7 @@
         if (diag || (mode != 0 && mode != 5))
             return fail(RT_ERR_INVALID_ARGUMENT, "RT_FLAG_UNIFORM53 runs with scan mode 5 (the default) or RT_FLAG_NO_FILTER, without RT_FLAG_DIAG_STATS");
         if (mode == 0) rc = launch_render<0, false, false, true>(ctx, kp, stream, &grid);
+        else if (small_grid && std::isfinite(kp.own_g)) rc = launch_render_own(ctx, kp, stream, &grid, large_blocks ? rt::kItemBlockLarge : rt::kItemBlock, true);
         else if (small_grid) rc = large_blocks ? launch_render<5, false, true, true, rt::kItemBlockLarge>(ctx, kp, stream, &grid)
                                               : launch_render<5, false, true, true>(ctx, kp, stream, &grid);
         else rc = large_blocks ? launch_render<5, false, false, true, rt::kItemBlockLarge>(ctx, kp, stream, &grid)
@@ -692,7 +750,8 @@
 #endif
     case 10:
         if (small_grid) {
-            rc = large_blocks ? launch_render<5, false, true, false, rt::kItemBlockLarge>(ctx, kp, stream, &grid)
+            rc = std::isfinite(kp.own_g) ? launch_render_own(ctx, kp, stream, &grid, large_blocks ? rt::kItemBlockLarge : rt::kItemBlock, false)
+               : large_blocks ? launch_render<5, false, true, false, rt::kItemBlockLarge>(ctx, kp, stream, &grid)
                               : launch_render<5, false, true>(ctx, kp, stream, &grid);
             ctx->last.kernel_variant = 1;
         } else rc = large_blocks ? launch_render<5, false, false, false, rt::kItemBlockLarge>(ctx, kp, stream, &grid)
@@ -897,6 +956,7 @@
     kp.use_ring = use_ring ? 1 : 0;
     kp.block_items = item_block;
     set_scene_params(ctx, kp);
+    kp.own_g = own_sphere_threshold(ctx, camera_reach(cam, 1), p->t_min);
     kp.fix = (unsigned long long *)d_fix;
     kp.pix_list = d_pixels;
     rc = next_launch_slot(ctx, stream, kp);
@@ -921,7 +981,8 @@
     const bool small_grid = ctx->grid_dim > 0 && ctx->n_global + ctx->grid_dim * ctx->grid_dim <= 64;
     ctx->last.scan_mode = 5;
     ctx->last.kernel_variant = 8 | (small_grid ? 1 : 0);
-    rc = small_grid ? launch_render<5, false, true, false, rt::kItemBlockList>(ctx, kp, stream, &grid)
+    rc = small_grid && std::isfinite(kp.own_g) ? launch_render_own(ctx, kp, stream, &grid, rt::kItemBlockList, false) :
+         small_grid ? launch_render<5, false, true, false, rt::kItemBlockList>(ctx, kp, stream, &grid)
                     : launch_render<5, false, false, false, rt::kItemBlockList>(ctx, kp, stream, &grid);
     if (rc) return rc;
     ctx->launched = true;
diff --git a/rtiow_amd/csrc/rt_diag.hpp b/rtiow_amd/csrc/rt_diag.hpp
--- a/rtiow_amd/csrc/rt_diag.hpp
+++ b/rtiow_amd/csrc/rt_diag.hpp
@@ -13,10 +13,15 @@
 #define RT_STAMP(k) RT_DIAG_NOTHING
 #define RT_COUNT(k) RT_DIAG_NOTHING
 #define RT_COUNT_N(k, n) RT_DIAG_NOTHING
+#define RT_COUNT_KEEP(k) RT_DIAG_NOTHING
 #define RT_COUNT_MAIN(k) RT_DIAG_NOTHING
 #define RT_COUNT_ROWS_TRIP(k) RT_DIAG_NOTHING
 #define RT_COUNT_ENUM_TRIP(m) RT_DIAG_NOTHING
 #define RT_COUNT_REDRAW_LANES(ok) RT_DIAG_NOTHING
+#define RT_OWN_TRACKED 0
+#define RT_OWN_DECLARE() RT_DIAG_NOTHING
+#define RT_OWN_TRACK(goes_on, code, dropped) RT_DIAG_NOTHING
+#define RT_OWN_COUNT_PAIRS(seg0, nwords, listv) RT_DIAG_NOTHING
 #define RT_LDS(site, BYTES, ATOMIC, LOAD64, ptr, active) RT_DIAG_NOTHING
 #define RT_LDS_N(site, n, BYTES, ATOMIC, LOAD64, byte_addr, active) RT_DIAG_NOTHING
 #define RT_LDS_QUEUE_READS(take, entry) RT_DIAG_NOTHING
@@ -55,12 +60,42 @@
 #define RT_COUNT(k) do { if ((int)(tid & 63) == (int)__builtin_ctzll(__ballot(true))) s_cnt[tid >> 6][k] += 1u; } while (0)
 #define RT_COUNT_N(k, n) do { if ((int)(tid & 63) == (int)__builtin_ctzll(__ballot(true))) s_cnt[tid >> 6][k] += (unsigned)(n); } while (0)
 #define RT_DIAG_FLUSH() do { if (lane == 0) for (int k_ = 0; k_ < 8; ++k_) atomicAdd(P.stats + 8 + k_, (unsigned long long)s_cnt[tid >> 6][k_]); } while (0)
+#undef RT_COUNT_KEEP
+#if defined(RT_COUNT_OWN)
+#define RT_COUNT_KEEP(k) RT_DIAG_NOTHING
+#else
+#define RT_COUNT_KEEP(k) RT_COUNT(k)
+#endif
 #if defined(RT_COUNT_ROWS)
 #undef RT_COUNT_ROWS_TRIP
 #define RT_COUNT_ROWS_TRIP(k) RT_COUNT(k)
 #elif defined(RT_COUNT_ENUM)
 #undef RT_COUNT_ENUM_TRIP
 #define RT_COUNT_ENUM_TRIP(m) do { RT_COUNT(1); RT_COUNT_N(6, __popcll(m)); } while (0)
+#elif defined(RT_COUNT_OWN)
+#undef RT_OWN_TRACKED
+#undef RT_OWN_DECLARE
+#undef RT_OWN_TRACK
+#undef RT_OWN_COUNT_PAIRS
+#define RT_OWN_TRACKED 1
+#define RT_OWN_DECLARE() uint32_t own_any = 0u
+#define RT_OWN_TRACK(goes_on, code, dropped) do { own_any = (goes_on) ? (code) : 0u; } while (0)
+#define RT_OWN_COUNT_PAIRS(seg0, nwords, listv) do { if constexpr (OWN) { \
+        bool set_ = false; \
+        for (int w_ = 0; w_ < (nwords); ++w_) { \
+            const int tile_ = !SMALLGRID && list_all ? (seg0) + w_ : (__builtin_amdgcn_readlane((listv), w_) & 0x0FFFFFFF); \
+            if (alive && own_any != 0u && tile_ == (int)((own_any - 1u) >> 5) && ((bits_w[w_ * 64 + lane] >> ((own_any - 1u) & 31u)) & 1u)) set_ = true; } \
+        bool acc_ = false; \
+        if (set_) {                                  \
+            const double4 g_ = *reinterpret_cast<const double4 *>(P.geo_slot + 4 * (size_t)(own_any - 1u)); \
+            const D3 oc_ = o - mk(g_.x, g_.y, g_.z); \
+            const double hb_ = dot(oc_, d), c_ = length_squared(oc_) - g_.w, disc_ = hb_ * hb_ - a * c_; \
+            if (!(disc_ < 0.0)) { const double sq_ = __builtin_sqrt(disc_); double r_ = (-hb_ - sq_) / a; \
+                if (r_ < t_min) r_ = (-hb_ + sq_) / a; \
+                acc_ = !(r_ < t_min); } } \
+        const unsigned n1_ = (unsigned)__popcll(__ballot(set_ && own == own_any)), n6_ = (unsigned)__popcll(__ballot(set_ && !acc_)), \
+                       n4_ = (unsigned)__popcll(__ballot(set_ && own == own_any && acc_)); \
+        RT_COUNT_N(1, n1_); RT_COUNT_N(6, n6_); RT_COUNT_N(4, n4_); } } while (0)
 #elif defined(RT_COUNT_REDRAW)
 #undef RT_COUNT_REDRAW_LANES
 #define RT_COUNT_REDRAW_LANES(ok) do { const unsigned n1_ = (unsigned)__popcll(__ballot(true)), n6_ = (unsigned)__popcll(__ballot(!(ok))); \
diff --git a/rtiow_amd/csrc/rt_frames.hip b/rtiow_amd/csrc/rt_frames.hip
--- a/rtiow_amd/csrc/rt_frames.hip
+++ b/rtiow_amd/csrc/rt_frames.hip
@@ -89,6 +89,7 @@
     kp.use_ring = use_ring ? 1 : 0;
     kp.block_items = item_block;
     set_scene_params(ctx, kp);
+    kp.own_g = own_sphere_threshold(ctx, ctx->frames_cam_reach, p->t_min);
     kp.fix = (unsigned long long *)d_fix;
     kp.cams = reinterpret_cast<const rt::KCamera *>(d_cams);
     kp.frame_items = frame_items;
@@ -119,7 +120,8 @@
     const bool small_grid = ctx->grid_dim > 0 && ctx->n_global + ctx->grid_dim * ctx->grid_dim <= 64;
     ctx->last.scan_mode = 5;
     ctx->last.kernel_variant = 16 | (small_grid ? 1 : 0);
-    rc = small_grid ? launch_render<5, false, true, false, rt::kItemBlockFrames>(ctx, kp, stream, &grid)
+    rc = small_grid && kp.own_g < 3.0e38f ? launch_render_own(ctx, kp, stream, &grid, rt::kItemBlockFrames, false) :
+         small_grid ? launch_render<5, false, true, false, rt::kItemBlockFrames>(ctx, kp, stream, &grid)
                     : launch_render<5, false, false, false, rt::kItemBlockFrames>(ctx, kp, stream, &grid);
     if (rc) return rc;
     ctx->launched = true;
@@ -144,7 +146,9 @@
     RT_HIP(hipMemcpyAsync(ctx->d_stage_cams, cams, (size_t)n_frames * sizeof(rt_camera), hipMemcpyHostToDevice, ctx->own_stream));
     rt_params q = *p;
     q.flags &= ~RT_FLAG_ACCUMULATE;
+    ctx->frames_cam_reach = camera_reach(cams, n_frames);
     rc = rt_render_frames_device(ctx, (const rt_camera *)ctx->d_stage_cams, n_frames, sample_stride, &q, ctx->d_stage_fix, ctx->own_stream);
+    ctx->frames_cam_reach = -1.0;
     if (rc) return rc;
     RT_HIP(hipMemcpyAsync(out_fix, ctx->d_stage_fix, count * sizeof(uint64_t), hipMemcpyDeviceToHost, ctx->own_stream));
     RT_HIP(hipStreamSynchronize(ctx->own_stream));
@@ -173,7 +177,9 @@
     RT_HIP(hipMemcpyAsync(ctx->d_stage_cams, cams, (size_t)n_frames * sizeof(rt_camera), hipMemcpyHostToDevice, ctx->own_stream));
     rt_params q = *p;
     q.flags &= ~RT_FLAG_ACCUMULATE;
+    ctx->frames_cam_reach = camera_reach(cams, n_frames);
     rc = rt_render_frames_device(ctx, (const rt_camera *)ctx->d_stage_cams, n_frames, sample_stride, &q, ctx->d_stage_fix, ctx->own_stream);
+    ctx->frames_cam_reach = -1.0;
     if (rc) return rc;
     if (!flip && (long long)n_frames * p->height <= 0x7fffffffLL) {
         rc = rt_resolve_rgba8_device(ctx, ctx->d_stage_fix, p->width, n_frames * p->height, (int64_t)p->spp, 0, ctx->d_stage_rgba, ctx->own_stream);
diff --git a/rtiow_amd/csrc/rt_host.hpp b/rtiow_amd/csrc/rt_host.hpp
--- a/rtiow_amd/csrc/rt_host.hpp
+++ b/rtiow_amd/csrc/rt_host.hpp
@@ -33,6 +33,8 @@
     int grid_dim = 0;
     float grid[8] = {};
     float scene_scale = 0.0f;
+    double own_reach = 0.0, own_rmin = 0.0;
+    double frames_cam_reach = -1.0;
 #ifdef RTIOW_CROSSCHECK_MODES
     XcheckScene x;
 #endif
@@ -70,6 +72,8 @@
 int validate_params(const rt_params *p);
 int ensure(void **ptr, size_t *have, size_t need);
 void set_scene_params(const rt_context *ctx, rt::KParams &kp);
+double camera_reach(const rt_camera *cams, int n);
+float own_sphere_threshold(const rt_context *ctx, double cam_reach, double t_min);
 int next_launch_slot(rt_context *ctx, hipStream_t stream, rt::KParams &kp);
 
 template <int MODE, bool DIAG, bool SMALLGRID = false, bool U53 = false, int ITEMS = rt::kItemBlock>
@@ -93,4 +97,6 @@
     return RT_OK;
 }
 
+int launch_render_own(rt_context *ctx, const rt::KParams &kp, hipStream_t stream, int *grid_out, int items, bool u53);
+
 }
diff --git a/rtiow_amd/csrc/rt_kernels.hpp b/rtiow_amd/csrc/rt_kernels.hpp
--- a/rtiow_amd/csrc/rt_kernels.hpp
+++ b/rtiow_amd/csrc/rt_kernels.hpp
@@ -45,6 +45,7 @@
     const uint32_t *slot_orig;
     float grid[8];
     int32_t grid_dim;
+    float own_g;
     unsigned long long grid_rows;
     int32_t n_global;
     int32_t n_tiles;
@@ -70,6 +71,7 @@
 constexpr int kScanUnroll = 8;
 constexpr int kItemBlock = 256;
 constexpr int kItemBlockLarge = 1024;
+constexpr int kItemsOwn = 1;
 constexpr int kItemBlockList = -kItemBlock;
 constexpr int kItemBlockFrames = -2 * kItemBlock;
 static_assert(kItemBlockLarge + 32768 < 65536, "udiv_small: numerators x < d + kItemBlockLarge with d < 2^15 keep x * d < 2^32");
@@ -98,9 +100,10 @@
 
 typedef float f32x4 __attribute__((ext_vector_type(4)));
 
-template <int MODE, bool DIAG, bool SMALLGRID = false, bool U53 = false, int ITEMS = 256>
+template <int MODE, bool DIAG, bool SMALLGRID = false, bool U53 = false, int ITEMS_ = 256>
 __global__ __launch_bounds__(kBlock, (MODE == 5 && !DIAG) ? 4 : (MODE >= 2) ? 3 : 5) void render_kernel(const KParams P)
 {
+    constexpr int ITEMS = ITEMS_ & ~kItemsOwn;
     constexpr bool PIXLIST = ITEMS == kItemBlockList;
     constexpr bool FRAMES = ITEMS == kItemBlockFrames;
     static_assert(ITEMS > 0 || PIXLIST || FRAMES, "ITEMS: a block size, kItemBlockList or kItemBlockFrames");
@@ -113,6 +116,8 @@
     constexpr bool MATRIX = (MODE >= 2);
     constexpr bool LIFTED = (MODE == 4);
     constexpr bool TUBE = (MODE == 5);
+    constexpr bool OWN = (ITEMS_ & kItemsOwn) != 0;
+    static_assert(!OWN || (TUBE && !DIAG && SMALLGRID), "the own-sphere drop: small-grid kernels of scan mode 5 without DIAG");
     constexpr bool RAYOP = (MODE == 2 || MODE == 3);
     __shared__ float s_rayop[RAYOP ? kBlock / 64 : 1][RAYOP ? 8 : 1][RAYOP ? kRowPad : 1];
     constexpr int kSeg = TUBE ? kSegTilesTube : kSegTiles;
@@ -130,6 +135,7 @@
     __shared__ unsigned int s_rpix[kBlock / 64][kRingDepth];
     __shared__ unsigned int s_live[DIAG ? kBlock / 64 : 1][DIAG ? 64 : 1];
     __shared__ double s_thr[3][kBlock];
+    __shared__ uint16_t s_own[OWN ? kBlock : 1];
 
     const int tid = threadIdx.x;
     const int lane = tid & 63;
@@ -160,6 +166,8 @@
     D3 o = mk(0, 0, 0), d = mk(0, 0, 1);
     int depth = 0;
     uint32_t ev = 0;
+    if constexpr (OWN) s_own[tid] = 0;
+    RT_OWN_DECLARE();
     uint32_t n_rays = 0, n_samples = 0, n_direct = 0;
     unsigned long long tot_cand = 0, tot_roots = 0;
     uint32_t blk_next = 0, blk_end = 0, blk_seq = 0xFFFFFFFFu, blk_pix0 = 0, blk_s0 = 0, blk_rr0 = 0, blk_i0 = 0;
@@ -493,9 +501,20 @@
                 RT_STAMP(2);
             };
             bool list_all = true;
-            auto enumerate = [&](int seg0, int nwords_tube = 0) {
+            auto enumerate = [&](int seg0, int nwords_tube = 0, int listv_tube = 0) {
                 unsigned summary = 0u, word = 0u;
                 if constexpr (TUBE) {
+                    const uint32_t own = OWN ? (uint32_t)s_own[tid] : 0u;
+                    RT_OWN_COUNT_PAIRS(seg0, nwords_tube, listv_tube);
+                    if constexpr (OWN) {
+                        const int own_tile = (int)((own - 1u) >> 5);
+                        int own_w = -1;
+                        for (int w = 0; w < nwords_tube; ++w) {
+                            const int tile_w = !SMALLGRID && list_all ? seg0 + w : (__builtin_amdgcn_readlane(listv_tube, w) & 0x0FFFFFFF);
+                            own_w = tile_w == own_tile ? w : own_w;
+                        }
+                        if (own_w >= 0) atomicAnd(&bits_w[own_w * 64 + lane], ~(1u << ((own - 1u) & 31u)));
+                    }
                     for (int w = 0; w < nwords_tube; ++w) summary |= min(bits_w[w * 64 + lane], 1u) << w;
                     if (!alive) summary = 0u;
                 } else {
@@ -605,7 +624,7 @@
 #pragma unroll
                         for (int bb = 0; bb < 2; ++bb) {
                             if (kh[bb] != 0ull) {
-                                RT_COUNT(4);
+                                RT_COUNT_KEEP(4);
 #pragma unroll
                                 for (int j = 0; j < 4; ++j) {
                                     RT_LDS(0, 4, true, false, &row[16 * G + 8 * bb + j],
@@ -787,7 +806,7 @@
                     __builtin_amdgcn_wave_barrier();
                     RT_STAMP(6);
                     __builtin_amdgcn_s_setprio(2);
-                    enumerate(t0, nwords);
+                    enumerate(t0, nwords, listv);
                 }
                 __builtin_amdgcn_s_setprio(1);
                 finish_pool();
@@ -853,6 +872,7 @@
             D3 p = o, nrm = mk(0.0, 0.0, 0.0), sp = mk(0.0, 0.0, 0.0), albedo = mk(1.0, 1.0, 1.0);
             double param = 0.0, inv_param = 0.0, r0_front = 0.0, r0_back = 0.0;
             uint32_t w_first = 0u, w_second = 0u;
+            uint32_t own_rec = 0u, own_next = 0u;
             if (is_hit) {
                 const double *mrec = mat + kMatStride * (size_t)hit;
                 const double4 g = *reinterpret_cast<const double4 *>(geo + 4 * (size_t)hit);
@@ -865,6 +885,9 @@
                 asm volatile("" : "+v"(w.x), "+v"(w.y), "+v"(w.z), "+v"(w.w));
                 kind = (int)mC.y;
                 param = mA.y;
+                if constexpr (OWN || RT_OWN_TRACKED) {
+                    own_rec = (uint32_t)__double_as_longlong(mE_.y);
+                }
                 albedo = mk(mB.x, mB.y, mC.x);
                 p = o + d * closest;
                 const D3 outward = (p - mk(g.x, g.y, g.z)) * mA.x;
@@ -958,7 +981,7 @@
                     }
                 } else if (kind == RT_KIND_METAL) {
                     ndir = uV + sp * param;
-                    if (dot(ndir, nrm) <= 0.0) done = true;
+                    if constexpr (!(OWN || RT_OWN_TRACKED)) { if (dot(ndir, nrm) <= 0.0) done = true; }
                 } else {
                     const double ratio = front ? inv_param : param;
                     const double cos_theta = min_1(-dot(uV, nrm));
@@ -974,7 +997,12 @@
                     }
                     ndir = do_refract ? refract(uV, nrm, ratio) : reflect(uV, nrm);
                 }
+                double m_out = 0.0;
                 if (kind != RT_KIND_DIALECTRIC) {
+                    if constexpr (OWN || RT_OWN_TRACKED) {
+                        m_out = dot(ndir, nrm);
+                        if (kind == RT_KIND_METAL && m_out <= 0.0) done = true;
+                    }
                     s_thr[0][tid] = s_thr[0][tid] * albedo.x;
                     s_thr[1][tid] = s_thr[1][tid] * albedo.y;
                     s_thr[2][tid] = s_thr[2][tid] * albedo.z;
@@ -983,7 +1011,10 @@
                 d = ndir;
                 depth -= 1;
                 if (depth <= 0) done = true;
-            }
+                if constexpr (OWN) own_next = (!done && front && (float)m_out * __uint_as_float(own_rec & 0xFFFF0000u) > P.own_g) ? (own_rec & 0xFFFFu) : 0u;
+                RT_OWN_TRACK(!done, own_rec & 0xFFFFu, own_next);
+            }
+            if constexpr (OWN) s_own[tid] = (uint16_t)own_next;
             if (done) {
                 alive = false;
                 finished = true;
diff --git a/rtiow_amd/csrc/rt_own.hip b/rtiow_amd/csrc/rt_own.hip
--- /dev/null
+++ b/rtiow_amd/csrc/rt_own.hip
@@ -0,0 +1,18 @@
+#include <hip/hip_runtime.h>
+
+#define RT_RENDER_KERNEL_ONLY
+#include "rt_host.hpp"
+
+int rt_host::launch_render_own(rt_context *ctx, const rt::KParams &kp, hipStream_t stream, int *grid_out, int items, bool u53)
+{
+    if (u53) {
+        if (items == rt::kItemBlock) return launch_render<5, false, true, true, rt::kItemBlock | rt::kItemsOwn>(ctx, kp, stream, grid_out);
+        if (items == rt::kItemBlockLarge) return launch_render<5, false, true, true, rt::kItemBlockLarge | rt::kItemsOwn>(ctx, kp, stream, grid_out);
+    } else {
+        if (items == rt::kItemBlock) return launch_render<5, false, true, false, rt::kItemBlock | rt::kItemsOwn>(ctx, kp, stream, grid_out);
+        if (items == rt::kItemBlockLarge) return launch_render<5, false, true, false, rt::kItemBlockLarge | rt::kItemsOwn>(ctx, kp, stream, grid_out);
+        if (items == rt::kItemBlockList) return launch_render<5, false, true, false, rt::kItemBlockList | rt::kItemsOwn>(ctx, kp, stream, grid_out);
+        if (items == rt::kItemBlockFrames) return launch_render<5, false, true, false, rt::kItemBlockFrames | rt::kItemsOwn>(ctx, kp, stream, grid_out);
+    }
+    return fail(RT_ERR_INVALID_ARGUMENT, "launch_render_own: no such instantiation (items %d, u53 %d)", items, (int)u53);
+}
```

New measurement: 8303, median of 3. About the same (+0.0%).
